# DotBlossom/LLM-driven_content-based-feature_recommendation_system

Measured on AMD Instinct MI355X. Metric: SimCSE train-step pairs/sec at d=128, batch 8192, higher is better.
Workload: dtype fp32+bf16x3+f16

## Files before the change

### include/recsys_amd.h

```cpp
#ifndef RECSYS_AMD_H
#define RECSYS_AMD_H

#include <stddef.h>
#include <stdint.h>

#ifdef __cplusplus
extern "C" {
#endif

const char* rsx_last_error(void);
int rsx_abi_version(void);
const char* rsx_target_arch(void);
const char* rsx_build_hash(void);

int rsx_seq_embed_fwd(const float* base, const int64_t* const* ids, const float* const* tables, int ntab,
                      const float* gate, const float* pos, const int64_t* tok_pos, const float* ln_w,
                      const float* ln_b, float eps, int64_t T, int64_t L, int64_t D, float p_drop, uint64_t seed,
                      float* out, float* mean, float* rstd, void* stream);

int64_t rsx_seq_embed_bwd_workspace_floats(int64_t T, int64_t L, int64_t D);
int rsx_seq_embed_bwd(const float* base, const int64_t* const* ids, const float* const* tables,
                      const int64_t* table_rows, const int64_t* padding_idx, int ntab, const float* gate,
                      const float* pos, const int64_t* tok_pos, const float* ln_w, const float* mean,
                      const float* rstd, float eps, int64_t T, int64_t L, int64_t D, float p_drop, uint64_t seed,
                      const float* dout, float* dbase, float* const* dtables, float* dgate, float* dpos,
                      float* dln_w, float* dln_b, float* workspace, int64_t ws_floats, void* stream);

int rsx_mha_fwd(const float* qkv, const uint8_t* key_pad, const int* seg_off, int64_t B, int64_t L, int64_t H,
                int64_t Dh, int causal, float p_drop, uint64_t seed, float* out, float* lse, void* stream);
int rsx_mha_bwd(const float* qkv, const uint8_t* key_pad, const int* seg_off, const float* out, const float* lse,
                const float* dout, int64_t B, int64_t L, int64_t H, int64_t Dh, int causal, float p_drop,
                uint64_t seed, float* dqkv, void* stream);
int rsx_mha_fwd_x3(const float* qkv, const uint8_t* key_pad, const int* seg_off, int64_t B, int64_t L, int64_t H,
                   int64_t Dh, int causal, float p_drop, uint64_t seed, float* out, float* lse, void* stream);
int rsx_mha_bwd_x3(const float* qkv, const uint8_t* key_pad, const int* seg_off, const float* out, const float* lse,
                   const float* dout, int64_t B, int64_t L, int64_t H, int64_t Dh, int causal, float p_drop,
                   uint64_t seed, float* dqkv, void* stream);
int rsx_mha_qkv_fwd_x3(const float* x, const float* w, const float* bias, const uint8_t* key_pad, const int* seg_off,
                       int64_t B, int64_t L, int64_t H, int causal, float p_drop, uint64_t seed, float* qkv,
                       float* out, float* lse, void* stream);

int64_t rsx_nce_workspace_floats(int64_t N, int64_t M, int nsplit_fwd, int nsplit_bwd);
int rsx_nce_fwd(const float* A, const float* B, const float* bias, const int* k1a, const int* k1b, const int* k2a,
                const int* k2b, int64_t N, int64_t M, int64_t lda, int64_t ldb, int64_t diag_offset, float tau,
                int flags, int nsplit, float* ws, float* out2, void* stream);
int rsx_nce_bwd(const float* A, const float* B, const float* bias, const int* k1a, const int* k1b, const int* k2a,
                const int* k2b, int64_t N, int64_t M, int64_t lda, int64_t ldb, int64_t diag_offset, float tau,
                int flags, int nsplit_fwd, int nsplit, const float* gout, float* ws, float* dA, float* dB,
                int accumulate, void* stream);

int64_t rsx_nce_x3_workspace_floats(int64_t N, int64_t M);
int rsx_nce_fwd_x3(const float* A, const float* B, const float* bias, const int* k1a, const int* k1b,
                   const int* k2a, const int* k2b, int64_t N, int64_t M, int64_t lda, int64_t ldb,
                   int64_t diag_offset, float tau, int flags, float* ws, float* out2, void* stream);
int rsx_nce_bwd_x3(const float* A, const float* B, const float* bias, const int* k1a, const int* k1b,
                   const int* k2a, const int* k2b, int64_t N, int64_t M, int64_t lda, int64_t ldb,
                   int64_t diag_offset, float tau, int flags, const float* gout, float* ws, float* dA, float* dB,
                   int accumulate, void* stream);

int64_t rsx_nce_fused_workspace_floats(int64_t N, int64_t M);
int64_t rsx_nce_view_ints(int64_t N, int64_t M);
int rsx_nce_view_fill(int64_t N, int64_t M, int64_t diag_offset, int* view, void* stream);
int rsx_nce_view_fill_host(int64_t N, int64_t M, int64_t diag_offset, int* view);
int rsx_nce_fwd_grad(const float* A, const float* B, const float* bias, const int* k1a, const int* k1b, int64_t N,
                     int64_t M, int64_t lda, int64_t ldb, int64_t diag_offset, float tau, int flags,
                     const int* view, float* ws, float* out2, float* ga, void* stream);
int rsx_nce_bwd_cols(const float* A, const float* B, const float* bias, const int* k1a, const int* k1b, int64_t N,
                     int64_t M, int64_t lda, int64_t ldb, int64_t diag_offset, float tau, int flags,
                     const int* view, const float* gout, float* ws, float* dB, void* stream);

int rsx_nce_emphasis_fwd(const float* A, const float* B, const float* bias, const int* k1a, const int* k1b,
                         const int64_t* top, int64_t N, int64_t M, int64_t K, int64_t lda, int64_t ldb,
                         int64_t diag_offset, float tau, float margin, int precision, int nsplit_fwd, float* ws,
                         float* out2, void* stream);
int rsx_nce_emphasis_bwd(const float* A, const float* B, const float* bias, const int* k1a, const int* k1b,
// ... 118 lines not shown
int rsx_deepfm_train_head(const float* h2, int64_t H, const float* wo, const float* lin, const float* bias,
                          const float* y, int64_t R, int mean, float* logit, float* g, float* dh2, void* ws,
                          int64_t ws_bytes, double* loss, float* dbias, float* dwo, void* stream);
int rsx_relu_bwd(float* dx, const float* h, int64_t n, void* stream);
int rsx_deepfm_train_contrib(const float* emb, const float* g, const float* dE, int64_t ldE, const int* inv,
                             int64_t R, int F, int E, float* gV, float* gW, void* stream);
int64_t rsx_deepfm_train_sparse_workspace_bytes(int64_t n);
int rsx_deepfm_train_sparse_adam(const int64_t* keys_sorted, const int* head_cum, const int* seg_start,
                                 const int* nseg, int64_t n, int F, int E, const int64_t* vocab, const float* gV,
                                 const float* gW, float* const* V, float* const* W, float* const* mV,
                                 float* const* vV, float* const* mW, float* const* vW, double lr, double beta1,
                                 double beta2, double eps, int64_t step, void* ws, int64_t ws_bytes, float* out_dV,
                                 float* out_dW, void* stream);

int64_t rsx_binary_eval_workspace_bytes(int64_t R);
int rsx_binary_eval(const float* logit, const float* y, int64_t R, void* ws, int64_t ws_bytes, int64_t* counts,
                    double* loss_sum, int* flag, void* stream);

int64_t rsx_group_eval_workspace_bytes(int64_t R);
int rsx_group_eval(const float* logit, const float* y, const int32_t* group_id, int64_t R, int top, const double* D,
                   int64_t max_group_id, void* ws, int64_t ws_bytes, int64_t* summary, int32_t* gid, int64_t* P,
                   int64_t* N, int64_t* U2, double* dcg, int* flag, void* stream);

int rsx_reranker_seq_lens(const int64_t* uidx, const int64_t* seq_off, int64_t B, int max_len, int64_t* lens,
                          void* stream);
int rsx_reranker_batch(const int64_t* uidx, const int64_t* iidx, int64_t B, const float* u_scaled, const double* u_raw,
                       const int64_t* u_cat, const float* i_scaled, const double* i_raw, const int64_t* i_num,
                       const int64_t* seq_off, const int64_t* seq_ids, int max_len, int64_t L, float* dense,
                       int64_t* cat, int64_t* target, int64_t* seq, int64_t* mask, void* stream);

int rsx_embed3_ln(const float* word, int64_t ld_word, const float* pos, const float* type_row, const float* ln_w,
                  const float* ln_b, float eps, const int64_t* ids, const int64_t* tok_pos, int64_t T, int64_t D,
                  float* out, void* stream);

int rsx_crossnet(const float* x, int64_t ldx, int64_t B, int D, int L, const float* const* kernels,
                 const float* const* biases, const float* w_head, float* x_out, float* head_part, void* stream);
int64_t rsx_crossnet_bwd_workspace_bytes(int64_t B, int D, int L, int max_blocks);
int rsx_crossnet_bwd(const float* x, int64_t ldx, int64_t B, int D, int L, const float* const* kernels,
                     const float* const* biases, const float* w_head, const float* dhead, const float* dx_out,
                     float* const* dk, float* const* db, float* dw_head, float* dx, void* ws, int64_t ws_bytes,
                     int max_blocks, void* stream);
int64_t rsx_dcn_train_head_workspace_bytes(int64_t R);
int rsx_dcn_train_head(const float* h2, int64_t H, const float* w_d, const float* head_part, const float* bias,
                       const float* y, int64_t R, int mean, float* logit, float* g, float* dh2, void* ws,
                       int64_t ws_bytes, double* loss, float* dbias, float* dw_d, void* stream);

int rsx_gather_rows(const float* src, int64_t ld_src, const int64_t* idx, int64_t n, int64_t D, int normalize,
                    float eps, float* out, float* nrm_out, void* stream);
int rsx_scatter_rows(const float* dy, const float* y, const float* nrm, const int64_t* idx, int64_t n, int64_t D,
                     int normalize, float eps, int mode, int64_t skip_idx, float* dst, int64_t ld_dst, void* stream);
int rsx_segment_sum_rows(const float* src, int64_t ld_src, const int64_t* perm, const int64_t* seg_off,
                         const int64_t* rows, int64_t nseg, int64_t D, const float* scale, int64_t skip_row,
                         float* dst, int64_t ld_dst, int accumulate, void* stream);

int rsx_loss_combine(const float* s_main, const float* s_un, const float* s_sup, const float* cnt, float inv_n,
                     float inv_b, float lambda_sup, float lambda_cl, float* total, float* logs, void* stream);
int rsx_loss_combine_bwd(const float* g, const float* cnt, float inv_n, float inv_b, float lambda_sup,
                         float lambda_cl, float* g3, void* stream);

enum {
  RSX_SP_IDS = 0, RSX_SP_TABLES = 16, RSX_SP_GATE = 32, RSX_SP_CONT = 33, RSX_SP_WC = 34, RSX_SP_BC = 35,
  RSX_SP_WM = 36, RSX_SP_BM = 37, RSX_SP_LNW = 38, RSX_SP_LNB = 39, RSX_SP_N = 40
};
int64_t rsx_static_profile_arena_bytes(int64_t U);
int64_t rsx_static_profile_bwd_workspace_bytes(int64_t U);
int rsx_static_profile_fwd(const void* const* p, const int64_t* dims, float eps, float p_drop, uint64_t seed,
                           void* arena, int64_t arena_bytes, float* out, void* stream);
int rsx_static_profile_bwd(const void* const* p, const int64_t* dims, float p_drop, uint64_t seed, const void* arena,
                           const float* dout, float* const* grads, void* ws, int64_t ws_bytes, void* stream);

int64_t rsx_clip_adamw_workspace_bytes(int n, const int64_t* numel, const int* clip);
int rsx_clip_adamw(int n, float* const* params, float* const* grads, float* const* exp_avg, float* const* exp_avg_sq,
                   const int64_t* numel, const int* clip, const float* step, const float* const* step_dev,
                   const double* lr, const double* weight_decay, const double* beta1, const double* beta2,
                   const double* eps, float max_norm, void* ws, int64_t ws_bytes, float* norm_out, void* stream);

int rsx_hnm_mine(const float* u_norm, const float* i_norm, const int64_t* target_ids, int64_t N, int64_t D,
                 int64_t k, float hnm_threshold, float temperature, void* ws, size_t ws_bytes, int64_t* top_idx,
                 float* top_cos, int32_t* avail, void* stream);
int64_t rsx_hnm_workspace_bytes(int64_t N);
int64_t rsx_hnm_max_rows(void);

enum {
  RSX_TW_PV = 0, RSX_TW_IDS = 1, RSX_TW_TOK_POS = 7, RSX_TW_TOK_PAD = 8, RSX_TW_SEG32 = 9, RSX_TW_SEG64 = 10,
  RSX_TW_TOK_USER = 11, RSX_TW_GATE = 12, RSX_TW_PROFILE = 13, RSX_TW_ITEMSEG = 14, RSX_TW_ITEM_PROJ = 19,
  RSX_TW_TABLES = 21, RSX_TW_POS = 27, RSX_TW_EMB_LN = 28, RSX_TW_LAYER0 = 30
};
int64_t rsx_tower_n_ptrs(int layers);
int64_t rsx_tower_arena_bytes(int64_t T, int64_t U, int layers);
int64_t rsx_tower_bwd_workspace_bytes(int64_t T, int64_t U, int64_t L, int layers, int64_t C);
int rsx_tower_fwd(const void* const* p, const int64_t* dims, const float* fargs, const uint64_t* seeds, void* arena,
                  int64_t arena_bytes, float* out, void* stream);
int rsx_tower_bwd(const void* const* p, const int64_t* dims, const float* fargs, const uint64_t* seeds,
                  const void* arena, const float* out, const float* dout, void* const* grads, void* ws,
                  int64_t ws_bytes, void* stream);

#ifdef __cplusplus
}
#endif

#endif
```

### llm-driven_content-based-feature_recommendation_system_amd/_native.py

```python
from __future__ import annotations

import ctypes
import os
import threading

import torch

_HERE = os.path.dirname(os.path.abspath(__file__))
LIB_PATH = os.environ.get("RSX_LIB_PATH") or os.path.join(_HERE, "librecsys_amd.so")

_lock = threading.Lock()
_lib = None
_checked_devices: set = set()

c_p = ctypes.c_void_p
c_i64 = ctypes.c_int64
c_i = ctypes.c_int
c_f = ctypes.c_float
c_d = ctypes.c_double
c_u64 = ctypes.c_uint64

ABI_VERSION = 9

_SIGS = {
    "rsx_last_error": (ctypes.c_char_p, []),
    "rsx_abi_version": (c_i, []),
    "rsx_target_arch": (ctypes.c_char_p, []),
    "rsx_build_hash": (ctypes.c_char_p, []),
    "rsx_seq_embed_fwd": (c_i, [c_p, c_p, c_p, c_i, c_p, c_p, c_p, c_p, c_p, c_f, c_i64, c_i64, c_i64, c_f, c_u64,
                                c_p, c_p, c_p, c_p]),
    "rsx_seq_embed_bwd_workspace_floats": (c_i64, [c_i64, c_i64, c_i64]),
    "rsx_seq_embed_bwd": (c_i, [c_p, c_p, c_p, c_p, c_p, c_i, c_p, c_p, c_p, c_p, c_p, c_p, c_f, c_i64, c_i64,
                                c_i64, c_f, c_u64, c_p, c_p, c_p, c_p, c_p, c_p, c_p, c_p, c_i64, c_p]),
    "rsx_mha_fwd": (c_i, [c_p, c_p, c_p, c_i64, c_i64, c_i64, c_i64, c_i, c_f, c_u64, c_p, c_p, c_p]),
    "rsx_mha_bwd": (c_i, [c_p, c_p, c_p, c_p, c_p, c_p, c_i64, c_i64, c_i64, c_i64, c_i, c_f, c_u64, c_p, c_p]),
    "rsx_mha_fwd_x3": (c_i, [c_p, c_p, c_p, c_i64, c_i64, c_i64, c_i64, c_i, c_f, c_u64, c_p, c_p, c_p]),
    "rsx_mha_qkv_fwd_x3": (c_i, [c_p, c_p, c_p, c_p, c_p, c_i64, c_i64, c_i64, c_i, c_f, c_u64, c_p, c_p, c_p, c_p]),
    "rsx_mha_bwd_x3": (c_i, [c_p, c_p, c_p, c_p, c_p, c_p, c_i64, c_i64, c_i64, c_i64, c_i, c_f, c_u64, c_p, c_p]),
    "rsx_nce_workspace_floats": (c_i64, [c_i64, c_i64, c_i, c_i]),
    "rsx_nce_fwd": (c_i, [c_p, c_p, c_p, c_p, c_p, c_p, c_p, c_i64, c_i64, c_i64, c_i64, c_i64, c_f, c_i, c_i, c_p,
                          c_p, c_p]),
    "rsx_nce_bwd": (c_i, [c_p, c_p, c_p, c_p, c_p, c_p, c_p, c_i64, c_i64, c_i64, c_i64, c_i64, c_f, c_i, c_i, c_i,
                          c_p, c_p, c_p, c_p, c_i, c_p]),
    "rsx_nce_x3_workspace_floats": (c_i64, [c_i64, c_i64]),
    "rsx_nce_fwd_x3": (c_i, [c_p, c_p, c_p, c_p, c_p, c_p, c_p, c_i64, c_i64, c_i64, c_i64, c_i64, c_f, c_i, c_p, c_p,
                             c_p]),
    "rsx_nce_bwd_x3": (c_i, [c_p, c_p, c_p, c_p, c_p, c_p, c_p, c_i64, c_i64, c_i64, c_i64, c_i64, c_f, c_i, c_p, c_p,
                             c_p, c_p, c_i, c_p]),
    "rsx_nce_fused_workspace_floats": (c_i64, [c_i64, c_i64]),
    "rsx_nce_view_ints": (c_i64, [c_i64, c_i64]),
    "rsx_nce_view_fill": (c_i, [c_i64, c_i64, c_i64, c_p, c_p]),
    "rsx_nce_view_fill_host": (c_i, [c_i64, c_i64, c_i64, c_p]),
    "rsx_nce_fwd_grad": (c_i, [c_p, c_p, c_p, c_p, c_p, c_i64, c_i64, c_i64, c_i64, c_i64, c_f, c_i, c_p, c_p, c_p,
                               c_p, c_p]),
    "rsx_nce_bwd_cols": (c_i, [c_p, c_p, c_p, c_p, c_p, c_i64, c_i64, c_i64, c_i64, c_i64, c_f, c_i, c_p, c_p, c_p,
                               c_p, c_p]),
    "rsx_nce_emphasis_fwd": (c_i, [c_p, c_p, c_p, c_p, c_p, c_p, c_i64, c_i64, c_i64, c_i64, c_i64, c_i64, c_f, c_f,
                                   c_i, c_i, c_p, c_p, c_p]),
    "rsx_nce_emphasis_bwd": (c_i, [c_p, c_p, c_p, c_p, c_p, c_p, c_i64, c_i64, c_i64, c_i64, c_i64, c_i64, c_f, c_f,
                                   c_i, c_i, c_p, c_p, c_p, c_p, c_p]),
    "rsx_nce_emphasis_bwd_csr": (c_i, [c_p, c_p, c_p, c_p, c_p, c_p, c_i64, c_i64, c_i64, c_i64, c_i64, c_i64, c_f,
                                       c_f, c_i, c_i, c_p, c_p, c_p, c_p, c_p, c_p, c_p, c_p]),
    "rsx_nce_grouped_workspace_floats": (c_i64, [c_i64, c_i64, c_i, c_i, c_i]),
    "rsx_nce_grouped_fwd": (c_i, [c_p, c_p, c_p, c_p, c_p, c_p, c_p, c_p, c_i64, c_i64, c_i64, c_i64, c_f, c_i, c_i,
                                  c_p, c_p, c_p]),
    "rsx_kernel_events": (c_i, [c_i]),
    "rsx_kernel_events_read": (c_i, [c_p, c_i]),
    "rsx_gather_events": (c_i, [c_i]),
    "rsx_gather_events_read": (c_i, [c_p, c_p, c_i]),
    "rsx_nce_grouped_fwd_grad": (c_i, [c_p, c_p, c_p, c_p, c_p, c_p, c_p, c_p, c_i64, c_i64, c_i64, c_i64, c_f, c_i,
                                       c_i, c_p, c_p, c_p, c_p]),
    "rsx_nce_grouped_bwd": (c_i, [c_p, c_p, c_p, c_p, c_p, c_p, c_p, c_p, c_p, c_p, c_p, c_p, c_p, c_i64, c_i64,
                                  c_i64, c_i64, c_f, c_i, c_i, c_i, c_p, c_p, c_p, c_p, c_i, c_p]),
    "rsx_deepfm_embed": (c_i, [c_p, c_i64, c_i, c_i, c_p, c_p, c_f, c_p, c_p, c_p]),
    "rsx_deepfm_fused_workspace_bytes": (c_i64, [c_i]),
    "rsx_deepfm_fused": (c_i, [c_p, c_i64, c_i, c_p, c_p, c_f, c_p, c_p, c_p, c_p, c_p, c_p, c_p, c_p, c_p]),
    "rsx_deepfm_fused_prep": (c_i, [c_i, c_p, c_p, c_p, c_p]),
    "rsx_deepfm_fused_run": (c_i, [c_p, c_i64, c_i, c_p, c_p, c_p, c_f, c_p, c_p, c_p, c_p, c_p, c_p, c_p]),
    "rsx_deepfm_pack": (c_i, [c_p, c_p, c_i64, c_p, c_p]),
    "rsx_reranker_seq_lens": (c_i, [c_p, c_p, c_i64, c_i, c_p, c_p]),
    "rsx_reranker_batch": (c_i, [c_p, c_p, c_i64, c_p, c_p, c_p, c_p, c_p, c_p, c_p, c_p, c_i, c_i64, c_p, c_p, c_p,
                                 c_p, c_p, c_p]),
    "rsx_deepfm_fused_uses_packed": (c_i, [c_i]),
    "rsx_linear_fwd": (c_i, [c_p, c_i64, c_p, c_p, c_i64, c_i64, c_i64, c_i, c_p, c_p]),
    "rsx_linear_dot_fwd": (c_i, [c_p, c_i64, c_p, c_p, c_i64, c_i64, c_i64, c_i, c_p, c_p, c_p, c_p, c_p]),
    "rsx_static_embed_fwd": (c_i, [c_p, c_p, c_p, c_p, c_i, c_p, c_i64, c_p, c_i64, c_p]),
    "rsx_static_embed_bwd_workspace_floats": (c_i64, [c_i64, c_i, c_p, c_p]),
    "rsx_static_embed_bwd": (c_i, [c_p, c_p, c_p, c_p, c_p, c_i, c_p, c_p, c_i64, c_i64, c_i64, c_p, c_p, c_i, c_p,
                                   c_i64, c_p]),
    "rsx_dropout_bwd": (c_i, [c_p, c_i64, c_i64, c_f, c_u64, c_p, c_p]),
    "rsx_ln_fwd": (c_i, [c_p, c_p, c_f, c_u64, c_p, c_p, c_f, c_i, c_i64, c_i64, c_p, c_p, c_p, c_p, c_p]),
    "rsx_ln_bwd_workspace_floats": (c_i64, [c_i64, c_i64]),
    "rsx_ln_bwd": (c_i, [c_p, c_p, c_p, c_p, c_p, c_i, c_p, c_p, c_f, c_u64, c_i64, c_i64, c_p, c_p, c_p, c_p, c_p,
                         c_i64, c_p]),
    "rsx_linear_wgrad_workspace_floats": (c_i64, [c_i64, c_i64, c_i64]),
    "rsx_linear_wgrad": (c_i, [c_p, c_i64, c_p, c_i64, c_i64, c_i64, c_i64, c_p, c_i64, c_p, c_i, c_p, c_i64, c_p]),
    "rsx_linear_wgrad_x3": (c_i, [c_p, c_i64, c_p, c_i64, c_i64, c_i64, c_i64, c_p, c_i64, c_p, c_i, c_p, c_i64, c_p]),
    "rsx_gemm_x3": (c_i, [c_p, c_i64, c_p, c_i64, c_p, c_i64, c_i, c_i, c_i, c_p, c_i64, c_f, c_u64, c_p, c_i64, c_p]),
    "rsx_gemm_x3_split_floats": (c_i64, [c_i64, c_i, c_i]),
    "rsx_gemm_x3_ws": (c_i, [c_p, c_i64, c_p, c_i64, c_p, c_i64, c_i, c_i, c_i, c_p, c_i64, c_f, c_u64, c_p, c_i64, c_p,
                             c_i64, c_p]),
    "rsx_gemm_x3_tn": (c_i, [c_p, c_i64, c_p, c_i64, c_p, c_i64, c_i, c_i, c_i, c_p, c_i64, c_f, c_u64, c_p, c_i64,
                             c_p]),
    "rsx_loss_combine": (c_i, [c_p, c_p, c_p, c_p, c_f, c_f, c_f, c_f, c_p, c_p, c_p]),
    "rsx_loss_combine_bwd": (c_i, [c_p, c_p, c_f, c_f, c_f, c_f, c_p, c_p]),
    "rsx_static_profile_arena_bytes": (c_i64, [c_i64]),
    "rsx_static_profile_bwd_workspace_bytes": (c_i64, [c_i64]),
    "rsx_static_profile_fwd": (c_i, [c_p, c_p, c_f, c_f, c_u64, c_p, c_i64, c_p, c_p]),
    "rsx_static_profile_bwd": (c_i, [c_p, c_p, c_f, c_u64, c_p, c_p, c_p, c_p, c_i64, c_p]),
    "rsx_clip_adamw_workspace_bytes": (c_i64, [c_i, c_p, c_p]),
    "rsx_clip_adamw": (c_i, [c_i, c_p, c_p, c_p, c_p, c_p, c_p, c_p, c_p, c_p, c_p, c_p, c_p, c_p, c_f, c_p, c_i64,
                             c_p, c_p]),
    "rsx_tower_n_ptrs": (c_i64, [c_i]),
    "rsx_tower_arena_bytes": (c_i64, [c_i64, c_i64, c_i]),
    "rsx_tower_bwd_workspace_bytes": (c_i64, [c_i64, c_i64, c_i64, c_i, c_i64]),
    "rsx_tower_fwd": (c_i, [c_p, c_p, c_p, c_p, c_p, c_i64, c_p, c_p]),
    "rsx_tower_bwd": (c_i, [c_p, c_p, c_p, c_p, c_p, c_p, c_p, c_p, c_p, c_i64, c_p]),
    "rsx_gemm_x3_rowadd": (c_i, [c_p, c_i64, c_p, c_i64, c_p, c_i64, c_i, c_i, c_p, c_i64, c_p, c_p, c_i64, c_p]),
    "rsx_gemm_x3_addln": (c_i, [c_p, c_i64, c_p, c_i64, c_p, c_i64, c_i, c_i, c_p, c_i64, c_f, c_u64, c_p, c_p, c_f,
                                c_p, c_i64, c_p, c_i64, c_p, c_p, c_p]),
    "rsx_topk_workspace_bytes": (c_i64, [c_i64, c_i64, c_i64]),
    "rsx_retrieve_topk": (c_i, [c_p, c_i64, c_p, c_i64, c_i64, c_i64, c_i64, c_p, c_p, c_p, c_p]),
    "rsx_topk_path": (c_i, [c_i64, c_i64, c_i64]),
    "rsx_ids_check": (c_i, [c_p, c_i64, c_i64, c_i64, c_p, c_p, c_p]),
    "rsx_step_index_workspace_bytes": (c_i64, [c_i64, c_i64, c_i64]),
    "rsx_step_index_count": (c_i, [c_p, c_p, c_p, c_i64, c_i64, c_i64, c_p, c_i64, c_p, c_p]),
    "rsx_step_index_totals": (c_i, [c_p, c_i, c_i64, c_i64, c_i64, c_p, c_i64, c_p, c_p]),
    "rsx_step_index_fill": (c_i, [c_p, c_p, c_p, c_p, c_i64, c_i64, c_i64, c_i64, c_p, c_p, c_i64, c_p, c_p]),
    "rsx_topk_corpus_bytes": (c_i64, [c_i64]),
    "rsx_topk_prepare_corpus": (c_i, [c_p, c_i64, c_i64, c_p, c_p]),
    "rsx_topk_workspace_bytes_corpus": (c_i64, [c_i64, c_i64, c_i64]),
    "rsx_retrieve_topk_corpus": (c_i, [c_p, c_i64, c_p, c_i64, c_p, c_i64, c_i64, c_i64, c_p, c_p, c_p, c_p]),
    "rsx_gather_rows": (c_i, [c_p, c_i64, c_p, c_i64, c_i64, c_i, c_f, c_p, c_p, c_p]),
    "rsx_embed3_ln": (c_i, [c_p, c_i64, c_p, c_p, c_p, c_p, c_f, c_p, c_p, c_i64, c_i64, c_p, c_p]),
    "rsx_crossnet": (c_i, [c_p, c_i64, c_i64, c_i, c_i, c_p, c_p, c_p, c_p, c_p, c_p]),
    "rsx_crossnet_bwd_workspace_bytes": (c_i64, [c_i64, c_i, c_i, c_i]),
    "rsx_crossnet_bwd": (c_i, [c_p, c_i64, c_i64, c_i, c_i, c_p, c_p, c_p, c_p, c_p, c_p, c_p, c_p, c_p, c_p, c_i64, c_i,
                               c_p]),
    "rsx_dcn_train_head_workspace_bytes": (c_i64, [c_i64]),
    "rsx_dcn_train_head": (c_i, [c_p, c_i64, c_p, c_p, c_p, c_p, c_i64, c_i, c_p, c_p, c_p, c_p, c_i64, c_p, c_p, c_p,
                                 c_p]),
    "rsx_segment_sum_rows": (c_i, [c_p, c_i64, c_p, c_p, c_p, c_i64, c_i64, c_p, c_i64, c_p, c_i64, c_i, c_p]),
    "rsx_scatter_rows": (c_i, [c_p, c_p, c_p, c_p, c_i64, c_i64, c_i, c_f, c_i, c_i64, c_p, c_i64, c_p]),
    "rsx_hnm_mine": (c_i, [c_p, c_p, c_p, c_i64, c_i64, c_i64, c_f, c_f, c_p, ctypes.c_size_t, c_p, c_p, c_p, c_p]),
    "rsx_hnm_workspace_bytes": (c_i64, [c_i64]),
    "rsx_hnm_max_rows": (c_i64, []),
    "rsx_deepfm_train_keys": (c_i, [c_p, c_i64, c_i, c_p, c_p, c_p, c_p, c_p]),
    "rsx_deepfm_train_segments": (c_i, [c_p, c_p, c_i64, c_p, c_p, c_p]),
    "rsx_deepfm_train_starts": (c_i, [c_p, c_i64, c_p, c_p, c_p]),
    "rsx_deepfm_train_head_workspace_bytes": (c_i64, [c_i64]),
    "rsx_deepfm_train_head": (c_i, [c_p, c_i64, c_p, c_p, c_p, c_p, c_i64, c_i, c_p, c_p, c_p, c_p, c_i64, c_p, c_p, c_p,
                                    c_p]),
    "rsx_relu_bwd": (c_i, [c_p, c_p, c_i64, c_p]),
    "rsx_deepfm_train_contrib": (c_i, [c_p, c_p, c_p, c_i64, c_p, c_i64, c_i, c_i, c_p, c_p, c_p]),
    "rsx_deepfm_train_sparse_workspace_bytes": (c_i64, [c_i64]),
    "rsx_deepfm_train_sparse_adam": (c_i, [c_p, c_p, c_p, c_p, c_i64, c_i, c_i, c_p, c_p, c_p, c_p, c_p, c_p, c_p,
                                           c_p, c_p, c_d, c_d, c_d, c_d, c_i64, c_p, c_i64, c_p, c_p, c_p]),
    "rsx_binary_eval_workspace_bytes": (c_i64, [c_i64]),
    "rsx_binary_eval": (c_i, [c_p, c_p, c_i64, c_p, c_i64, c_p, c_p, c_p, c_p]),
    "rsx_group_eval_workspace_bytes": (c_i64, [c_i64]),
    "rsx_group_eval": (c_i, [c_p, c_p, c_p, c_i64, c_i, c_p, c_i64, c_p, c_i64, c_p, c_p, c_p, c_p, c_p, c_p, c_p, c_p]),
}

EXPORTED_SYMBOLS = tuple(_SIGS.keys())


def load(path: str = LIB_PATH):
    global _lib
    with _lock:
        if _lib is not None:
            return _lib
        if not os.path.exists(path):
            raise RuntimeError(
                f"recsys_amd: native library not found at {path}; run __graft_entry__.build() "
                "(hipcc --offload-arch=gfx950). There is no CPU fallback.")
        lib = ctypes.CDLL(path)
        for name, (res, args) in _SIGS.items():
            fn = getattr(lib, name)
            fn.restype = res
            fn.argtypes = args
        if lib.rsx_abi_version() != ABI_VERSION:
            raise RuntimeError(f"recsys_amd: {path} has ABI {lib.rsx_abi_version()}, this binding expects "
                               f"{ABI_VERSION}; rebuild with __graft_entry__.build()")
        _lib = lib
        return lib


def lib():
    return _lib if _lib is not None else load()


def source_files() -> list:
    import glob
    here = os.path.dirname(os.path.abspath(__file__))
    csrc = os.path.join(here, "csrc")
# ... 63 lines not shown
```

### llm-driven_content-based-feature_recommendation_system_amd/csrc/rows.hip

```cpp
#include "rsx_common.h"

namespace {

template <int D>
struct RowGeo {
  static constexpr int LPR = D / 4;
  static constexpr int RPW = 64 / LPR;
};

template <int D, bool NORM>
__global__ __launch_bounds__(256) void gather_rows_k(const float* __restrict__ src, int64_t ld_src,
                                                    const int64_t* __restrict__ idx, int64_t n, float eps,
                                                    float* __restrict__ out, float* __restrict__ nrm_out) {
  constexpr int LPR = RowGeo<D>::LPR, RPW = RowGeo<D>::RPW;
  const int lane = threadIdx.x & 63, sub = lane / LPR, c = lane % LPR;
  const int64_t wave_g = (int64_t)blockIdx.x * 4 + (threadIdx.x >> 6);
  const int64_t nw = (int64_t)gridDim.x * 4;
  for (int64_t r0 = wave_g * RPW; r0 < n; r0 += nw * RPW) {
    const int64_t r = r0 + sub;
    const bool ok = r < n;
    float4 x = make_float4(0.f, 0.f, 0.f, 0.f);
    if (ok) {
      const int64_t s = idx ? idx[r] : r;
      x = reinterpret_cast<const float4*>(src + s * ld_src)[c];
// ... 26 lines not shown
    float4 g = make_float4(0.f, 0.f, 0.f, 0.f);
    if (ok) g = reinterpret_cast<const float4*>(dy + r * D)[c];
    if (NORM) {
      float4 yv = make_float4(0.f, 0.f, 0.f, 0.f);
      if (ok) yv = reinterpret_cast<const float4*>(y + r * D)[c];
      float dot = yv.x * g.x + yv.y * g.y + yv.z * g.z + yv.w * g.w;
      dot = rsx::wave_sum_width(dot, LPR);
      const float nv = ok ? nrm[r] : 1.0f;
      if (nv > eps) {
        g.x = (g.x - yv.x * dot) / nv; g.y = (g.y - yv.y * dot) / nv;
        g.z = (g.z - yv.z * dot) / nv; g.w = (g.w - yv.w * dot) / nv;
      } else {
        g.x = g.x / eps; g.y = g.y / eps; g.z = g.z / eps; g.w = g.w / eps;
      }
    }
    if (ATOMIC) {
      float* xr = &s_xr[threadIdx.x >> 6][sub][0];
      reinterpret_cast<float4*>(xr)[c] = g;
      __builtin_amdgcn_wave_barrier();
      float xs[4];
#pragma unroll
      for (int k = 0; k < 4; ++k) xs[k] = xr[c + LPR * k];
      __builtin_amdgcn_wave_barrier();
      if (!ok) continue;
      const int64_t d = idx ? idx[r] : r;
      if (d == skip_idx) continue;
      float* q = dst + d * ld_dst + c;
#pragma unroll
      for (int k = 0; k < 4; ++k) atomicAdd(q + LPR * k, xs[k]);
      continue;
    }
    if (!ok) continue;
    const int64_t d = idx ? idx[r] : r;
    if (d == skip_idx) continue;
    float* p = dst + d * ld_dst + 4 * c;
    if (accumulate) {
      float4 o = *reinterpret_cast<float4*>(p);
      o.x += g.x; o.y += g.y; o.z += g.z; o.w += g.w;
      *reinterpret_cast<float4*>(p) = o;
    } else {
      *reinterpret_cast<float4*>(p) = g;
    }
  }
}

unsigned grid_for(int64_t n, int D) {
  const int64_t rows_per_block = 4 * (64 / (D / 4));
  int64_t b = (n + rows_per_block - 1) / rows_per_block;
  if (b > 16384) b = 16384;
  if (b < 1) b = 1;
  return (unsigned)b;
}

template <int D>
__global__ __launch_bounds__(256) void segsum_rows_k(const float* __restrict__ src, int64_t ld_src,
                                                    const int64_t* __restrict__ perm,
                                                    const int64_t* __restrict__ seg,
                                                    const int64_t* __restrict__ rows, int64_t nseg,
                                                    const float* __restrict__ scale, int64_t skip,
                                                    float* __restrict__ dst, int64_t ld_dst, int accumulate) {
  constexpr int LPR = RowGeo<D>::LPR, RPW = RowGeo<D>::RPW;
  const int lane = threadIdx.x & 63, sub = lane / LPR, c = lane % LPR;
  const int64_t wave_g = (int64_t)blockIdx.x * 4 + (threadIdx.x >> 6);
  const int64_t nw = (int64_t)gridDim.x * 4;
  const float sc = scale ? scale[0] : 1.0f;
  for (int64_t u0 = wave_g * RPW; u0 < nseg; u0 += nw * RPW) {
    const int64_t u = u0 + sub;
    if (u >= nseg) continue;
    const int64_t row = rows ? rows[u] : u;
    if (row == skip) continue;
    float4 acc = make_float4(0.f, 0.f, 0.f, 0.f);
    const int64_t k1 = seg[u + 1];
    int64_t k = seg[u];
    for (; k + 16 <= k1; k += 16) {
      int64_t p[16];
#pragma unroll
      for (int i = 0; i < 16; ++i) p[i] = perm ? perm[k + i] : k + i;
      float4 x[16];
#pragma unroll
      for (int i = 0; i < 16; ++i) x[i] = reinterpret_cast<const float4*>(src + p[i] * ld_src)[c];
#pragma unroll
      for (int i = 0; i < 16; ++i) {
        acc.x += x[i].x; acc.y += x[i].y; acc.z += x[i].z; acc.w += x[i].w;
      }
    }
    if (k < k1) {
      const int n = (int)(k1 - k);
      int64_t p[15];
#pragma unroll
      for (int i = 0; i < 15; ++i) p[i] = i < n ? (perm ? perm[k + i] : k + i) : 0;
      float4 x[15];
#pragma unroll
      for (int i = 0; i < 15; ++i)
        x[i] = i < n ? reinterpret_cast<const float4*>(src + p[i] * ld_src)[c] : make_float4(0.f, 0.f, 0.f, 0.f);
#pragma unroll
      for (int i = 0; i < 15; ++i)
        if (i < n) { acc.x += x[i].x; acc.y += x[i].y; acc.z += x[i].z; acc.w += x[i].w; }
    }
    float4* d = reinterpret_cast<float4*>(dst + row * ld_dst) + c;
    float4 v = make_float4(sc * acc.x, sc * acc.y, sc * acc.z, sc * acc.w);
    if (accumulate) {
      const float4 o = *d;
      v.x += o.x; v.y += o.y; v.z += o.z; v.w += o.w;
    }
    *d = v;
  }
}

__global__ __launch_bounds__(256) void ids_check_k(const int64_t* __restrict__ ids, int64_t n, int64_t lo, int64_t hi,
                                                   int64_t* __restrict__ out, int* flag) {
  bool bad = false;
  for (int64_t i = (int64_t)blockIdx.x * 256 + threadIdx.x; i < n; i += (int64_t)gridDim.x * 256) {
    const int64_t v = ids[i];
    const bool ok = v >= lo && v < hi;
    out[i] = ok ? v : 0;
    bad |= !ok;
  }
  if (__builtin_amdgcn_ballot_w64(bad) && (threadIdx.x & 63) == 0) atomicOr(flag, 1);
}

__global__ void loss_combine_k(const float* s_main, const float* s_un, const float* s_sup, const float* cnt,
                               float inv_n, float inv_b, float lsup, float lcl, float* total, float* logs) {
  if (threadIdx.x != 0) return;
  const float m = s_main ? s_main[0] * inv_n : 0.0f;
  float cl = s_un[0] * inv_b;
  if (s_sup) cl += lsup * (s_sup[0] / fmaxf(cnt[0], 1.0f));
  const float t = m + lcl * cl;
  total[0] = t;
  logs[0] = t; logs[1] = m; logs[2] = cl;
}

__global__ void loss_combine_bwd_k(const float* g, const float* cnt, float inv_n, float inv_b, float lsup, float lcl,
                                   float* g3) {
  if (threadIdx.x != 0) return;
  const float gv = g[0];
  g3[0] = gv * inv_n;
  g3[1] = gv * lcl * inv_b;
  g3[2] = cnt ? gv * lcl * lsup / fmaxf(cnt[0], 1.0f) : 0.0f;
}

}

RSX_API int rsx_loss_combine(const float* s_main, const float* s_un, const float* s_sup, const float* cnt,
                             float inv_n, float inv_b, float lambda_sup, float lambda_cl, float* total, float* logs,
                             void* stream) {
  RSX_ARG(s_un && total && logs && (!s_sup || cnt), "null tensor");
  hipLaunchKernelGGL(loss_combine_k, dim3(1), dim3(64), 0, (hipStream_t)stream, s_main, s_un, s_sup, cnt, inv_n,
                     inv_b, lambda_sup, lambda_cl, total, logs);
  RSX_LAUNCHED();
  return 0;
// ... 17 lines not shown
  hipStream_t st = (hipStream_t)stream;
  const unsigned g = grid_for(n, (int)D);
#define RSX_G(DD)                                                                                     \
  if (D == DD) {                                                                                      \
    if (normalize) hipLaunchKernelGGL((gather_rows_k<DD, true>), dim3(g), dim3(256), 0, st, src, ld_src, idx, n, eps, out, nrm_out); \
    else hipLaunchKernelGGL((gather_rows_k<DD, false>), dim3(g), dim3(256), 0, st, src, ld_src, idx, n, eps, out, nrm_out); \
  }
  RSX_G(64) RSX_G(128) RSX_G(256)
#undef RSX_G
  RSX_LAUNCHED();
  return 0;
}

RSX_API int rsx_scatter_rows(const float* dy, const float* y, const float* nrm, const int64_t* idx, int64_t n,
                             int64_t D, int normalize, float eps, int mode, int64_t skip_idx, float* dst,
                             int64_t ld_dst, void* stream) {
  RSX_ARG(dy && dst, "null tensor");
  RSX_ARG(!normalize || (y && nrm), "normalize backward needs y and norms");
  RSX_ARG(D == 64 || D == 128 || D == 256, "D must be 64, 128 or 256");
  RSX_ARG(mode >= 0 && mode <= 2, "mode must be 0,1,2");
  if (n == 0) return 0;
  hipStream_t st = (hipStream_t)stream;
  const unsigned g = grid_for(n, (int)D);
#define RSX_S(DD, NN, AA)                                                                           \
  hipLaunchKernelGGL((scatter_rows_k<DD, NN, AA>), dim3(g), dim3(256), 0, st, dy, y, nrm, idx, n, eps, dst, ld_dst, \
                     mode == 1 ? 1 : 0, skip_idx)
#define RSX_SD(DD)                                          \
  if (D == DD) {                                            \
    if (normalize) {                                        \
      if (mode == 2) RSX_S(DD, true, true); else RSX_S(DD, true, false);   \
    } else {                                                \
      if (mode == 2) RSX_S(DD, false, true); else RSX_S(DD, false, false); \
    }                                                       \
  }
  RSX_SD(64) RSX_SD(128) RSX_SD(256)
#undef RSX_SD
#undef RSX_S
  RSX_LAUNCHED();
  return 0;
}

RSX_API int rsx_segment_sum_rows(const float* src, int64_t ld_src, const int64_t* perm, const int64_t* seg_off,
                                 const int64_t* rows, int64_t nseg, int64_t D, const float* scale, int64_t skip_row,
                                 float* dst, int64_t ld_dst, int accumulate, void* stream) {
  RSX_ARG(src && seg_off && dst, "null tensor");
  RSX_ARG(D == 64 || D == 128 || D == 256, "D must be 64, 128 or 256");
  RSX_ARG(ld_src >= D && ld_dst >= D && ld_src % 4 == 0 && ld_dst % 4 == 0, "bad leading dimensions");
  if (nseg == 0) return 0;
  hipStream_t st = (hipStream_t)stream;
  const unsigned g = grid_for(nseg, (int)D);
#define RSX_SS(DD)                                                                                            \
  if (D == DD)                                                                                                \
    hipLaunchKernelGGL(segsum_rows_k<DD>, dim3(g), dim3(256), 0, st, src, ld_src, perm, seg_off, rows, nseg, \
                       scale, skip_row, dst, ld_dst, accumulate);
  RSX_SS(64) RSX_SS(128) RSX_SS(256)
#undef RSX_SS
  RSX_LAUNCHED();
  return 0;
}

RSX_API int rsx_ids_check(const int64_t* ids, int64_t n, int64_t lo, int64_t hi, int64_t* out, int* flag,
                          void* stream) {
  RSX_ARG(ids && out && flag, "null tensor");
  RSX_ARG(lo <= 0 && 0 < hi, "the replacement id 0 must lie in [lo, hi)");
  if (n == 0) return 0;
  int64_t g = (n + 255) / 256;
  if (g > 1024) g = 1024;
  hipLaunchKernelGGL(ids_check_k, dim3((unsigned)g), dim3(256), 0, (hipStream_t)stream, ids, n, lo, hi, out, flag);
  RSX_LAUNCHED();
  return 0;
}
```

### llm-driven_content-based-feature_recommendation_system_amd/csrc/rsx_errors.hip

```cpp
#include "rsx_common.h"
#include <stdarg.h>
#include <stdio.h>

namespace rsx {
static thread_local char g_err[1024] = {0};

void set_error(const char* fmt, ...) {
  va_list ap;
  va_start(ap, fmt);
  vsnprintf(g_err, sizeof(g_err), fmt, ap);
  va_end(ap);
}
}

RSX_API const char* rsx_last_error(void) { return rsx::g_err; }

RSX_API int rsx_abi_version(void) { return 9; }

RSX_API const char* rsx_target_arch(void) { return "gfx950"; }

#ifndef RSX_SRC_HASH
#define RSX_SRC_HASH "unknown"
#endif
RSX_API const char* rsx_build_hash(void) { return RSX_SRC_HASH; }
```

### llm-driven_content-based-feature_recommendation_system_amd/csrc/seq_embed.hip

```cpp
#include "rsx_common.h"
#include <mutex>
#include <utility>
#include <vector>

namespace {

constexpr int kMaxTab = 6;

struct FwdArgs {
  const float* base;
  const int64_t* ids[kMaxTab];
  const float* tab[kMaxTab];
  const float* gate;
  const float* pos;
  const int64_t* tok_pos;
  const float* ln_w;
  const float* ln_b;
  float* out;
  float* mean;
  float* rstd;
  int64_t T;
  int L;
  int ntab;
  float eps;
  rsx::Dropout drop;
};

typedef float f4v __attribute__((ext_vector_type(4)));
typedef __attribute__((address_space(1))) const f4v gf4v;
typedef __attribute__((address_space(1))) const int64_t gint64;
__device__ __forceinline__ float4 ldg4(const float* p) {
  const f4v v = *(gf4v*)(p);
  return make_float4(v.x, v.y, v.z, v.w);
}
__device__ __forceinline__ int64_t ldg8(const int64_t* p) { return *(gint64*)(p); }

template <int W>
__device__ __forceinline__ float lane_sum(float v) {
  if constexpr (W != 16 && W != 32 && W != 64) {
    return rsx::wave_sum_width(v, W);
  } else {
    if constexpr (W == 64) {
      const auto sw = __builtin_amdgcn_permlane32_swap(__float_as_uint(v), __float_as_uint(v), false, false);
      v = __uint_as_float(sw[0]) + __uint_as_float(sw[1]);
    }
    if constexpr (W >= 32) {
      const auto sw = __builtin_amdgcn_permlane16_swap(__float_as_uint(v), __float_as_uint(v), false, false);
      v = __uint_as_float(sw[0]) + __uint_as_float(sw[1]);
    }
    v += __int_as_float(__builtin_amdgcn_update_dpp(__float_as_int(v), __float_as_int(v), 0x128, 0xF, 0xF, false));
    v += __int_as_float(__builtin_amdgcn_update_dpp(__float_as_int(v), __float_as_int(v), 0x124, 0xF, 0xF, false));
    v += __int_as_float(__builtin_amdgcn_update_dpp(__float_as_int(v), __float_as_int(v), 0x122, 0xF, 0xF, false));
    v += __int_as_float(__builtin_amdgcn_update_dpp(__float_as_int(v), __float_as_int(v), 0x121, 0xF, 0xF, false));
    return v;
  }
}

__device__ __forceinline__ float4 f4_axpy_rn(float4 x, float4 e, float g) {
#pragma clang fp contract(off)
  x.x = x.x + e.x * g;
  x.y = x.y + e.y * g;
  x.z = x.z + e.z * g;
  x.w = x.w + e.w * g;
  return x;
}

__device__ __forceinline__ float4 f4_add_rn(float4 x, float4 p) {
#pragma clang fp contract(off)
  x.x = x.x + p.x;
  x.y = x.y + p.y;
  x.z = x.z + p.z;
  x.w = x.w + p.w;
  return x;
}

template <int D>
__device__ __forceinline__ float4 build_row(const FwdArgs& a, int64_t r, int c, const float* g) {
  float4 x = make_float4(0.f, 0.f, 0.f, 0.f);
  if (a.base) x = ldg4(a.base + r * D + 4 * c);
#pragma unroll
  for (int j = 0; j < kMaxTab; ++j) {
    if (j < a.ntab && g[j] != 0.0f) {
      const int64_t id = ldg8(a.ids[j] + r);
      const float4 e = ldg4(a.tab[j] + id * D + 4 * c);
      x = f4_axpy_rn(x, e, g[j]);
    }
  }
  if (a.pos) {
    const int l = a.tok_pos ? (int)ldg8(a.tok_pos + r) : (int)(r % a.L);
    x = f4_add_rn(x, ldg4(a.pos + (int64_t)l * D + 4 * c));
  }
  return x;
}

template <int D>
__device__ __forceinline__ void ln_drop_store(const FwdArgs& a, float4 x, int64_t r, bool ok, int c, float4 w,
                                              float4 bb, bool do_ln) {
  constexpr int LPR = D / 4;
  float4 y = x;
  if (do_ln) {
    float s = (x.x + x.y) + (x.z + x.w);
    s = lane_sum<LPR>(s);
    const float mu = s / (float)D;
    const float4 d = make_float4(x.x - mu, x.y - mu, x.z - mu, x.w - mu);
    float v = d.x * d.x + d.y * d.y + d.z * d.z + d.w * d.w;
    v = lane_sum<LPR>(v);
    const float rs = 1.0f / sqrtf(v / (float)D + a.eps);
    y.x = d.x * rs * w.x + bb.x;
    y.y = d.y * rs * w.y + bb.y;
    y.z = d.z * rs * w.z + bb.z;
    y.w = d.w * rs * w.w + bb.w;
    if (ok && c == 0) {
      if (a.mean) a.mean[r] = mu;
      if (a.rstd) a.rstd[r] = rs;
    }
  }
  if (ok) {
    if (a.drop.active()) {
      const uint64_t base_idx = (uint64_t)r * D + 4 * c;
      y.x = a.drop.apply(y.x, base_idx + 0);
      y.y = a.drop.apply(y.y, base_idx + 1);
      y.z = a.drop.apply(y.z, base_idx + 2);
      y.w = a.drop.apply(y.w, base_idx + 3);
    }
    reinterpret_cast<float4*>(a.out + r * D)[c] = y;
  }
}

template <int D, int U, int NL, bool FULL = false>
__device__ __forceinline__ void fwd_groups(const FwdArgs& a, const int64_t* const* ids_l, const float* const* tab_l,
                                           const float* g_l, int64_t r0, int sub, int c, float4 w, float4 bb,
                                           bool do_ln) {
  constexpr int RPW = 64 / (D / 4);
  const bool has_pos = FULL || a.pos, has_base = FULL || a.base;
  int64_t rr[U];
  int64_t id[U][NL > 0 ? NL : 1];
  int lp[U];
#pragma unroll
  for (int u = 0; u < U; ++u) {
    const int64_t r = r0 + u * RPW + sub;
    rr[u] = r < a.T ? r : a.T - 1;
#pragma unroll
    for (int k = 0; k < NL; ++k) id[u][k] = ldg8(ids_l[k] + rr[u]);
    if (FULL) lp[u] = (int)ldg8(a.tok_pos + rr[u]);
    else lp[u] = a.pos ? (a.tok_pos ? (int)a.tok_pos[rr[u]] : (int)(rr[u] % a.L)) : 0;
  }
  float4 x[U];
#pragma unroll
  for (int u = 0; u < U; ++u)
    x[u] = has_base ? ldg4(a.base + rr[u] * D + 4 * c) : make_float4(0.f, 0.f, 0.f, 0.f);
  float4 e[U][NL > 0 ? NL : 1];
#pragma unroll
  for (int k = 0; k < NL; ++k)
#pragma unroll
    for (int u = 0; u < U; ++u) e[u][k] = ldg4(tab_l[k] + id[u][k] * D + 4 * c);
  float4 pv[U];
  if (FULL) {
#pragma unroll
    for (int u = 0; u < U; ++u) pv[u] = ldg4(a.pos + (int64_t)lp[u] * D + 4 * c);
  }
#pragma unroll
  for (int k = 0; k < NL; ++k)
#pragma unroll
    for (int u = 0; u < U; ++u) x[u] = f4_axpy_rn(x[u], e[u][k], g_l[k]);
  if (has_pos) {
#pragma unroll
    for (int u = 0; u < U; ++u)
      x[u] = f4_add_rn(x[u], FULL ? pv[u] : ldg4(a.pos + (int64_t)lp[u] * D + 4 * c));
  }
#pragma unroll
  for (int u = 0; u < U; ++u) {
    const int64_t r = r0 + u * RPW + sub;
    ln_drop_store<D>(a, x[u], r, r < a.T, c, w, bb, FULL || do_ln);
  }
}

template <int D, int U>
__global__ __launch_bounds__(256) void seq_embed_fwd_k(FwdArgs a) {
  constexpr int LPR = D / 4;
  constexpr int RPW = 64 / LPR;
  const int lane = threadIdx.x & 63;
  const int sub = lane / LPR, c = lane % LPR;
  const int64_t wave_g = (int64_t)blockIdx.x * (blockDim.x >> 6) + (threadIdx.x >> 6);
  const int64_t nwaves = (int64_t)gridDim.x * (blockDim.x >> 6);
  float g[kMaxTab];
#pragma unroll
  for (int j = 0; j < kMaxTab; ++j) g[j] = (j < a.ntab) ? (a.gate ? a.gate[j] : 1.0f) : 0.0f;
  const int64_t* ids_l[2] = {nullptr, nullptr};
  const float* tab_l[2] = {nullptr, nullptr};
  float g_l[2] = {0.0f, 0.0f};
  int nl = 0;
#pragma unroll
  for (int j = 0; j < kMaxTab; ++j) {
    if (g[j] != 0.0f) {
      if (nl == 0) { ids_l[0] = a.ids[j]; tab_l[0] = a.tab[j]; g_l[0] = g[j]; }
      else if (nl == 1) { ids_l[1] = a.ids[j]; tab_l[1] = a.tab[j]; g_l[1] = g[j]; }
      ++nl;
    }
  }
  const bool do_ln = a.ln_w != nullptr;
  float4 w = make_float4(1.f, 1.f, 1.f, 1.f), bb = make_float4(0.f, 0.f, 0.f, 0.f);
  if (do_ln) {
    w = reinterpret_cast<const float4*>(a.ln_w)[c];
    bb = reinterpret_cast<const float4*>(a.ln_b)[c];
  }
  if (nl > 2) {
    for (int64_t r0 = wave_g * RPW; r0 < a.T; r0 += nwaves * RPW) {
      const int64_t r = r0 + sub;
      const bool ok = r < a.T;
      const float4 x = build_row<D>(a, ok ? r : a.T - 1, c, g);
      ln_drop_store<D>(a, x, r, ok, c, w, bb, do_ln);
    }
    return;
  }
  if (nl == 2 && a.base && a.pos && a.tok_pos && do_ln) {
    for (int64_t r0 = wave_g * (RPW * U); r0 < a.T; r0 += nwaves * (RPW * U))
      fwd_groups<D, U, 2, true>(a, ids_l, tab_l, g_l, r0, sub, c, w, bb, true);
    return;
  }
  for (int64_t r0 = wave_g * (RPW * U); r0 < a.T; r0 += nwaves * (RPW * U)) {
    if (nl == 2) fwd_groups<D, U, 2>(a, ids_l, tab_l, g_l, r0, sub, c, w, bb, do_ln);
    else if (nl == 1) fwd_groups<D, U, 1>(a, ids_l, tab_l, g_l, r0, sub, c, w, bb, do_ln);
    else fwd_groups<D, U, 0>(a, ids_l, tab_l, g_l, r0, sub, c, w, bb, do_ln);
  }
}

struct BwdArgs {
  FwdArgs f;
  const float* dout;
  float* dbase;
  float* dtab[kMaxTab];
  int64_t pad_idx[kMaxTab];
  int small_off[kMaxTab];
  int small_rows[kMaxTab];
  float* dgate;
  float* dpos;
  float* dln_w;
  float* dln_b;
  int64_t rows_per_block;
  int small_total;
  float* partials;
  int part_w;
};

struct BwdLive {
  const int64_t* ids[kMaxTab];
  const float* tab[kMaxTab];
  float* dtab[kMaxTab];
  float g[kMaxTab];
  int64_t pad[kMaxTab];
  int soff[kMaxTab];
  int j[kMaxTab];
  int n;
};

struct BwdCtx {
  float* xr;
  float* s_pos;
  float* s_small;
  int64_t r_begin, r_end;
  int wave, sub, c;
  float4 w;
  bool do_ln;
};

template <int D, int U, int NL, bool SC>
__device__ __forceinline__ void bwd_groups(const BwdArgs& a, const BwdLive& lv, const BwdCtx& cx, int64_t r00,
                                           float4& acc_w, float4& acc_b, float* acc_l) {
  constexpr int LPR = D / 4;
  constexpr int RPW = 64 / LPR;
  constexpr int NW = 4;
  constexpr int NS = NL > 0 ? NL : 1;
  const FwdArgs& f = a.f;
  const int c = cx.c;
  const bool need_e = cx.do_ln || a.dgate;
  const bool need_l = (f.pos && cx.do_ln) || a.dpos;
  int64_t rc[U];
  int lp[U];
  int64_t id[U][NS];
#pragma unroll
  for (int u = 0; u < U; ++u) {
    const int64_t ru = r00 + (u * NW + cx.wave) * RPW + cx.sub;
    rc[u] = ru < cx.r_end ? ru : cx.r_begin;
    lp[u] = need_l ? (f.tok_pos ? (int)f.tok_pos[rc[u]] : (int)(rc[u] % f.L)) : 0;
#pragma unroll
    for (int k = 0; k < NS; ++k)
      id[u][k] = (NL > 0 && (NL != kMaxTab || k < lv.n)) ? ldg8(lv.ids[k] + rc[u]) : 0;
  }
  float4 dyv[U], xv[U];
  float muv[U], rsv[U];
#pragma unroll
  for (int u = 0; u < U; ++u) {
    dyv[u] = ldg4(a.dout + rc[u] * D + 4 * c);
    xv[u] = make_float4(0.f, 0.f, 0.f, 0.f);
    muv[u] = 0.0f; rsv[u] = 0.0f;
    if (cx.do_ln) {
      if (f.base) xv[u] = ldg4(f.base + rc[u] * D + 4 * c);
      muv[u] = f.mean[rc[u]];
      rsv[u] = f.rstd[rc[u]];
    }
  }
  float4 ev[U][NS];
#pragma unroll
  for (int k = 0; k < NS; ++k)
#pragma unroll
    for (int u = 0; u < U; ++u) {
      ev[u][k] = make_float4(0.f, 0.f, 0.f, 0.f);
      if (NL > 0 && (NL != kMaxTab || k < lv.n) && need_e)
        ev[u][k] = ldg4(lv.tab[k] + id[u][k] * D + 4 * c);
    }
  if (cx.do_ln) {
#pragma unroll
    for (int k = 0; k < NS; ++k)
#pragma unroll
      for (int u = 0; u < U; ++u)
        if (NL > 0 && (NL != kMaxTab || k < lv.n)) xv[u] = f4_axpy_rn(xv[u], ev[u][k], lv.g[k]);
    if (f.pos) {
#pragma unroll
      for (int u = 0; u < U; ++u)
        xv[u] = f4_add_rn(xv[u], ldg4(f.pos + (int64_t)lp[u] * D + 4 * c));
    }
  }
#pragma unroll
  for (int u = 0; u < U; ++u) {
    const int64_t r = r00 + (u * NW + cx.wave) * RPW + cx.sub;
    if (r >= cx.r_end) continue;
    float4 dy = dyv[u];
    if (f.drop.active()) {
      const uint64_t bi = (uint64_t)r * D + 4 * c;
      dy.x = f.drop.apply(dy.x, bi + 0);
      dy.y = f.drop.apply(dy.y, bi + 1);
      dy.z = f.drop.apply(dy.z, bi + 2);
      dy.w = f.drop.apply(dy.w, bi + 3);
    }
    float4 dx = dy;
    if (cx.do_ln) {
      const float4 x = xv[u];
      const float mu = muv[u], rs = rsv[u];
      const float4 w = cx.w;
      const float4 xh = make_float4((x.x - mu) * rs, (x.y - mu) * rs, (x.z - mu) * rs, (x.w - mu) * rs);
      acc_w.x += dy.x * xh.x; acc_w.y += dy.y * xh.y; acc_w.z += dy.z * xh.z; acc_w.w += dy.w * xh.w;
      acc_b.x += dy.x; acc_b.y += dy.y; acc_b.z += dy.z; acc_b.w += dy.w;
      const float4 dh = make_float4(dy.x * w.x, dy.y * w.y, dy.z * w.z, dy.w * w.w);
      float c1 = (dh.x + dh.y) + (dh.z + dh.w);
      float c2 = dh.x * xh.x + dh.y * xh.y + dh.z * xh.z + dh.w * xh.w;
      c1 = lane_sum<LPR>(c1) / (float)D;
      c2 = lane_sum<LPR>(c2) / (float)D;
      dx.x = (dh.x - c1 - xh.x * c2) * rs;
      dx.y = (dh.y - c1 - xh.y * c2) * rs;
      dx.z = (dh.z - c1 - xh.z * c2) * rs;
// ... 390 lines not shown
    dst = a.dln_b ? a.dln_b + (j - nlds - a.D) : nullptr;
  } else if (j - nlds - 2 * a.D < a.ntab) {
    dst = a.dgate ? a.dgate + (j - nlds - 2 * a.D) : nullptr;
  }
  if (dst) *dst += v;
}

template <int D>
int launch_fwd(const FwdArgs& a, hipStream_t st) {
  constexpr int U = 2;
  const int64_t rows_per_block = 4 * (64 / (D / 4)) * U;
  int64_t blocks = (a.T + rows_per_block - 1) / rows_per_block;
  if (blocks > 16384) blocks = 16384;
  if (blocks < 1) blocks = 1;
  hipLaunchKernelGGL((seq_embed_fwd_k<D, U>), dim3((unsigned)blocks), dim3(256), 0, st, a);
  return 0;
}

template <int D>
int launch_bwd(const BwdArgs& a, hipStream_t st, bool keysum) {
  const int64_t blocks = (a.f.T + a.rows_per_block - 1) / a.rows_per_block;
  if (keysum) {
    hipLaunchKernelGGL((seq_embed_bwd_k<D, false>), dim3((unsigned)blocks), dim3(256), 0, st, a);
    return 0;
  }
  const size_t lds = (size_t)(a.f.L * D + a.small_total) * sizeof(float);
  hipLaunchKernelGGL((seq_embed_bwd_k<D>), dim3((unsigned)blocks), dim3(256), lds, st, a);
  return 0;
}

int64_t bwd_rows_per_block(int64_t T, int64_t D, int64_t target_blocks) {
  int64_t rpb = (T + target_blocks - 1) / target_blocks;
  const int64_t quantum = 2 * 4 * (64 / (D / 4));
  rpb = (rpb + quantum - 1) / quantum * quantum;
  if (rpb < quantum) rpb = quantum;
  return rpb;
}

int small_layout(const int64_t* table_rows, int ntab, int64_t D, bool has_grad_j[kMaxTab], int off[kMaxTab],
                 int rows[kMaxTab]) {
  int o = 0;
  for (int j = 0; j < kMaxTab; ++j) {
    off[j] = -1;
    rows[j] = 0;
    if (j < ntab && has_grad_j[j] && table_rows && table_rows[j] * D <= 4096 && o + table_rows[j] * D <= kSmallMax) {
      off[j] = o;
      rows[j] = (int)table_rows[j];
      o += (int)(table_rows[j] * D);
    }
  }
  return o;
}

bool fill_fwd(FwdArgs& a, const float* base, const int64_t* const* ids, const float* const* tabs, int ntab,
              const float* gate, const float* pos, const int64_t* tok_pos, const float* ln_w, const float* ln_b,
              float eps, int64_t T, int64_t L, float* out, float* mean, float* rstd, float p_drop, uint64_t seed) {
  if (ntab < 0 || ntab > kMaxTab) return false;
  a.base = base;
  for (int j = 0; j < kMaxTab; ++j) {
    a.ids[j] = (j < ntab) ? ids[j] : nullptr;
    a.tab[j] = (j < ntab) ? tabs[j] : nullptr;
  }
  a.gate = gate;
  a.pos = pos;
  a.tok_pos = tok_pos;
  a.ln_w = ln_w;
  a.ln_b = ln_b;
  a.out = out;
  a.mean = mean;
  a.rstd = rstd;
  a.T = T;
  a.L = (int)L;
  a.ntab = ntab;
  a.eps = eps;
  a.drop = rsx::make_dropout(p_drop, seed);
  return true;
}

struct GatherEvents {
  std::mutex mu;
  bool on = false;
  std::vector<std::pair<hipEvent_t, hipEvent_t>> ev;
  std::vector<int64_t> tokens;
  void clear() {
    for (auto& e : ev) {
      (void)hipEventDestroy(e.first);
      (void)hipEventDestroy(e.second);
    }
    ev.clear();
    tokens.clear();
  }
};
GatherEvents& gather_events() {
  static GatherEvents g;
  return g;
}
}

RSX_API int rsx_gather_events(int on) {
  GatherEvents& g = gather_events();
  std::lock_guard<std::mutex> lk(g.mu);
  g.clear();
  g.on = on != 0;
  return 0;
}

RSX_API int rsx_gather_events_read(float* ms, int64_t* tokens, int max_n) {
  RSX_ARG((ms != nullptr && tokens != nullptr) || max_n == 0, "null output");
  GatherEvents& g = gather_events();
  std::lock_guard<std::mutex> lk(g.mu);
  int n = 0;
  for (size_t k = 0; k < g.ev.size() && n < max_n; ++k) {
    float t = 0.0f;
    hipError_t err = hipEventSynchronize(g.ev[k].second);
    if (err == hipSuccess) err = hipEventElapsedTime(&t, g.ev[k].first, g.ev[k].second);
    if (err != hipSuccess) {
      rsx::set_error("%s: %s", __func__, hipGetErrorString(err));
      return -1;
    }
    ms[n] = t;
    tokens[n] = g.tokens[k];
    ++n;
  }
  return n;
}

RSX_API int rsx_seq_embed_fwd(const float* base, const int64_t* const* ids, const float* const* tables, int ntab,
                              const float* gate, const float* pos, const int64_t* tok_pos, const float* ln_w,
                              const float* ln_b, float eps, int64_t T, int64_t L, int64_t D, float p_drop,
                              uint64_t seed, float* out, float* mean, float* rstd, void* stream) {
  RSX_ARG(out != nullptr, "out is null");
  RSX_ARG(T >= 0 && L > 0 && L <= 64, "need T >= 0 and 0 < L <= 64");
  RSX_ARG(D == 64 || D == 128 || D == 256, "D must be 64, 128 or 256");
  RSX_ARG(ntab >= 0 && ntab <= kMaxTab, "ntab must be in [0,6]");
  RSX_ARG(ln_w == nullptr || (ln_b != nullptr), "ln_b required with ln_w");
  RSX_ARG(p_drop >= 0.0f && p_drop < 1.0f, "p_drop must be in [0,1)");
  for (int j = 0; j < ntab; ++j) RSX_ARG(ids[j] != nullptr && tables[j] != nullptr, "null table/ids");
  if (T == 0) return 0;
  FwdArgs a;
  fill_fwd(a, base, ids, tables, ntab, gate, pos, tok_pos, ln_w, ln_b, eps, T, L, out, mean, rstd, p_drop, seed);
  hipStream_t st = (hipStream_t)stream;
  GatherEvents& ge = gather_events();
  std::pair<hipEvent_t, hipEvent_t> evp{nullptr, nullptr};
  const bool timed = ge.on;
  if (timed && hipEventCreate(&evp.first) == hipSuccess && hipEventCreate(&evp.second) == hipSuccess)
    (void)hipEventRecord(evp.first, st);
  if (D == 64) launch_fwd<64>(a, st);
  else if (D == 128) launch_fwd<128>(a, st);
  else launch_fwd<256>(a, st);
  RSX_LAUNCHED();
  if (timed && evp.second) {
    (void)hipEventRecord(evp.second, st);
    std::lock_guard<std::mutex> lk(ge.mu);
    ge.ev.push_back(evp);
    ge.tokens.push_back(T);
  }
  return 0;
}

constexpr int64_t kBwdBlocksWs = 768;
constexpr int64_t kBwdBlocksAtomic = 512;
constexpr int64_t kKeyBlocksMax = 512;

RSX_API int64_t rsx_seq_embed_bwd_workspace_floats(int64_t T, int64_t L, int64_t D) {
  if (T <= 0 || D <= 0) return 0;
  const int64_t rpb = bwd_rows_per_block(T, D, kBwdBlocksWs);
  const int64_t blocks = (T + rpb - 1) / rpb;
  return blocks * (L * D + kSmallMax + 2 * D + kMaxTab) + kKeyBlocksMax * 64 * D;
}

RSX_API int rsx_seq_embed_bwd(const float* base, const int64_t* const* ids, const float* const* tables,
                              const int64_t* table_rows, const int64_t* padding_idx, int ntab, const float* gate,
                              const float* pos, const int64_t* tok_pos, const float* ln_w, const float* mean,
                              const float* rstd, float eps, int64_t T, int64_t L, int64_t D, float p_drop,
                              uint64_t seed, const float* dout, float* dbase, float* const* dtables, float* dgate,
                              float* dpos, float* dln_w, float* dln_b, float* workspace, int64_t ws_floats,
                              void* stream) {
  RSX_ARG(dout != nullptr, "dout is null");
  RSX_ARG(D == 64 || D == 128 || D == 256, "D must be 64, 128 or 256");
  RSX_ARG(ntab >= 0 && ntab <= kMaxTab, "ntab must be in [0,6]");
  RSX_ARG(ln_w == nullptr || (mean != nullptr && rstd != nullptr), "mean/rstd required with ln_w");
  RSX_ARG(p_drop >= 0.0f && p_drop < 1.0f, "p_drop must be in [0,1)");
  RSX_ARG(L > 0 && L <= 64, "need 0 < L <= 64");
  if (T == 0) return 0;
  BwdArgs a;
  fill_fwd(a.f, base, ids, tables, ntab, gate, pos, tok_pos, ln_w, nullptr, eps, T, L, nullptr,
           const_cast<float*>(mean), const_cast<float*>(rstd), p_drop, seed);
  a.dout = dout;
  a.dbase = dbase;
  bool has_grad[kMaxTab];
  for (int j = 0; j < kMaxTab; ++j) {
    a.dtab[j] = (j < ntab && dtables) ? dtables[j] : nullptr;
    a.pad_idx[j] = (j < ntab && padding_idx) ? padding_idx[j] : -1;
    has_grad[j] = a.dtab[j] != nullptr;
  }
  a.small_total = small_layout(table_rows, ntab, D, has_grad, a.small_off, a.small_rows);
  a.dgate = dgate;
  a.dpos = dpos;
  a.dln_w = dln_w;
  a.dln_b = dln_b;
  const bool use_ws = workspace != nullptr;
  if (use_ws)
    RSX_ARG(ws_floats >= rsx_seq_embed_bwd_workspace_floats(T, L, D), "workspace too small");
  a.rows_per_block = bwd_rows_per_block(T, D, use_ws ? kBwdBlocksWs : kBwdBlocksAtomic);
  const int64_t blocks = (T + a.rows_per_block - 1) / a.rows_per_block;
  a.partials = use_ws ? workspace : nullptr;
  a.part_w = (int)(L * D + a.small_total + 2 * D + kMaxTab);
  KeyArgs k{};
  bool keysum = use_ws && D == 128 && dbase != nullptr && (L * D + a.small_total) <= 64 * D &&
                getenv("RSX_SEQ_EMBED_KEYSUM") == nullptr;
  int nsm = 0;
  for (int j = 0; j < ntab && keysum; ++j) {
    if (!a.dtab[j] || a.small_off[j] < 0) continue;
    if (nsm == 2) { keysum = false; break; }
    k.ids[nsm] = ids[j];
    k.key_off[nsm] = (int)(L + a.small_off[j] / D);
    k.pad[nsm] = a.pad_idx[j];
    ++nsm;
  }
  hipStream_t st = (hipStream_t)stream;
  if (D == 64) launch_bwd<64>(a, st, false);
  else if (D == 128) launch_bwd<128>(a, st, keysum);
  else launch_bwd<256>(a, st, false);
  const int64_t ws_a = blocks * a.part_w;
  int64_t kblocks = 0;
  if (keysum) {
    const int64_t nb = 2 * rsx::cu_count() < kKeyBlocksMax ? 2 * rsx::cu_count() : kKeyBlocksMax;
    int64_t rpb = (T + nb - 1) / nb;
    rpb = (rpb + 63) / 64 * 64;
    kblocks = (T + rpb - 1) / rpb;
    k.dx = dbase;
    k.tok_pos = tok_pos;
    k.T = T;
    k.L = (int)L;
    k.do_pos = dpos != nullptr;
    k.nkeys = (int)(L + a.small_total / D);
    k.rows_per_block = rpb;
    k.partials = workspace + ws_a;
    const dim3 g((unsigned)kblocks), b(256);
// ... 38 lines not shown
```

### llm-driven_content-based-feature_recommendation_system_amd/csrc/step_index.hip

```cpp
#include "rsx_common.h"
#include <hipcub/hipcub.hpp>
#include <limits.h>

namespace {

constexpr int kSegChunk = 64;

__device__ __forceinline__ uint64_t wballot(bool p) { return __builtin_amdgcn_ballot_w64(p); }
__device__ __forceinline__ int below(uint64_t m, int lane) {
  return __popcll(m & ((lane == 0) ? 0ull : (~0ull >> (64 - lane))));
}

__device__ __forceinline__ int wave_sort_asc(int v, int lane) {
#pragma unroll
  for (int k = 2; k <= 64; k <<= 1) {
#pragma unroll
    for (int j = k >> 1; j > 0; j >>= 1) {
      const int o = __shfl_xor(v, j, 64);
      const bool asc = (lane & k) == 0, lower = (lane & j) == 0;
      v = (asc == lower) ? min(v, o) : max(v, o);
    }
  }
  return v;
}
// ... 152 lines not shown
      int t = lane < 16 ? wsum[lane] : 0;
#pragma unroll
      for (int d = 1; d < 16; d <<= 1) {
        const int y = __shfl_up(t, d, 64);
        if (lane >= d) t += y;
      }
      if (lane < 16) wsum[lane] = t;
    }
    __syncthreads();
    int e = carry + (w > 0 ? wsum[w - 1] : 0) + x - s;
#pragma unroll
    for (int k = 0; k < 4; ++k) {
      if (i0 + k < J.n) J.out[i0 + k] = e;
      e += v[k];
    }
    carry += wsum[15];
    __syncthreads();
  }
}

__global__ void si_totals_k(const int* offT, const int* offN, const int* offE, const int* colidx, const int* itemidx,
                            const int* chunkoff, const int* err, const int* tglob, int world, int64_t B, int64_t L,
                            int64_t n_items, int64_t* tot) {
  if (threadIdx.x != 0) return;
  tot[0] = offT[B];
  tot[1] = offN[B];
  tot[2] = colidx[n_items];
  tot[3] = offE[B];
  tot[4] = itemidx[n_items];
  tot[5] = chunkoff[n_items];
  int e = *err ? 1 : 0;
  tot[7] = 0;
  for (int r = 0; r < world; ++r) {
    const int v = tglob[(int64_t)r * (B * L + 1) + B * L];
    e |= (v & kSlotErr) ? 1 : 0;
    tot[8 + r] = v & ~kSlotErr;
  }
  tot[6] = e;
}

struct FillOut {
  int64_t *flat1, *user1, *pos1;
  uint8_t* pad1;
  int* seg1;
  int64_t* seg1_64;
  int64_t *valid_tok, *last_tok;
  int64_t *flat2, *user2, *pos2;
  uint8_t* pad2;
  int* seg2;
  int64_t* seg2_64;
  int64_t* tok_ids;
  int *row_col, *row_beg, *row_end, *exc_cols;
  int* last_t;
};

__global__ __launch_bounds__(256) void si_tokens_k(const uint8_t* pm, const int64_t* tgt, const int64_t* ids0,
                                                   const int64_t* ids1, const int64_t* ids2, const int64_t* ids3,
                                                   const int64_t* ids4, const int64_t* ids5, int64_t B, int L,
                                                   int64_t T, const int* offT, const int* offN, const int* offE,
                                                   const int* srt, const int* colidx, FillOut f, unsigned* ikeys,
                                                   int* ivals, unsigned* pkeys, int* pvals, int* pair_b, int* pair_n) {
  const int lane = threadIdx.x & 63;
  const int64_t b = (int64_t)blockIdx.x * 4 + (threadIdx.x >> 6);
  if (b >= B) return;
  const User u = user_sel(pm, b, L, lane);
  const int64_t o = b * L + lane;
  const int64_t t0 = offT[b];
  if (u.sel) {
    const int64_t tok = t0 + below(u.sm, lane);
    const uint8_t pd = u.valid ? 0 : 1;
    f.flat1[tok] = o;
    f.user1[tok] = b;
    f.pos1[tok] = lane;
    f.pad1[tok] = pd;
    f.flat2[tok] = o;
    f.flat2[T + tok] = B * L + o;
    f.user2[tok] = b;
    f.user2[T + tok] = B + b;
    f.pos2[tok] = lane;
    f.pos2[T + tok] = lane;
    f.pad2[tok] = pd;
    f.pad2[T + tok] = pd;
    const int64_t* src[6] = {ids0, ids1, ids2, ids3, ids4, ids5};
#pragma unroll
    for (int k = 0; k < 6; ++k) {
      const int64_t v = src[k][o];
      f.tok_ids[(2 * k) * T + tok] = v;
      f.tok_ids[(2 * k + 1) * T + tok] = v;
    }
    ikeys[tok] = (unsigned)ids0[o];
    ivals[tok] = (int)tok;
    if (u.valid) {
      const int64_t r = offN[b] + below(u.vm, lane);
      f.valid_tok[r] = tok;
      f.row_col[r] = colidx[tgt[o]];
      f.row_beg[r] = offN[b];
      f.row_end[r] = offN[b + 1];
    }
  }
  if (lane < u.cnt) {
    const int v = srt[b * L + lane];
    const int c = colidx[v];
    f.exc_cols[offN[b] + lane] = c;
    const int pv = __shfl_up(v, 1, 64);
    (void)pv;
  }
  {
    const int v = lane < u.cnt ? srt[b * L + lane] : INT_MAX;
    const int pv = __shfl_up(v, 1, 64);
    const bool ds = lane < u.cnt && (lane == 0 || v != pv);
    const uint64_t dm = wballot(ds);
    if (ds) {
      const uint64_t higher = (lane == 63) ? 0ull : (dm & (~0ull << (lane + 1)));
      const int nxt = higher ? (__ffsll((long long)higher) - 1) : u.cnt;
      const int64_t e = offE[b] + below(dm, lane);
      pkeys[e] = (unsigned)colidx[v];
      pvals[e] = (int)e;
      pair_b[e] = (int)b;
      pair_n[e] = nxt - lane;
    }
  }
  if (lane == 0) {
    f.last_tok[b] = t0 + __popcll(u.sm & ((u.last == 0) ? 0ull : (~0ull >> (64 - u.last))));
    f.last_t[b] = (int)tgt[b * L + u.last];
    f.seg1[b] = (int)t0;
    f.seg1_64[b] = t0;
    f.seg2[b] = (int)t0;
    f.seg2_64[b] = t0;
    f.seg2[B + b] = (int)(T + t0);
    f.seg2_64[B + b] = T + t0;
    if (b == B - 1) {
      f.seg1[B] = (int)T;
      f.seg1_64[B] = T;
      f.seg2[2 * B] = (int)(2 * T);
      f.seg2_64[2 * B] = 2 * T;
    }
  }
}

__global__ __launch_bounds__(256) void si_itemseg_k(const unsigned* skeys, const int* svals, int64_t T,
                                                    const int* hist_i, const int* itemoff, const int* itemidx,
                                                    const int* chunkoff, int64_t U, int64_t C, int64_t* perm,
                                                    int64_t* cb, int64_t* chunk_ids, int64_t* ch_off,
                                                    int64_t* uniq_items) {
  for (int64_t p = (int64_t)blockIdx.x * 256 + threadIdx.x; p < T; p += (int64_t)gridDim.x * 256) {
    const unsigned id = skeys[p];
    const int64_t a = itemoff[id], n = hist_i[id], w = p - a;
    const int64_t tok = svals[p];
    perm[2 * a + w] = tok;
    perm[2 * a + n + w] = T + tok;
    if (w == 0) {
      const int64_t ui = itemidx[id], c0 = chunkoff[id];
      uniq_items[ui] = id;
      ch_off[ui] = c0;
      const int64_t nch = (2 * n + kSegChunk - 1) / kSegChunk;
      for (int64_t k = 0; k < nch; ++k) {
        cb[c0 + k] = 2 * a + kSegChunk * k;
        chunk_ids[c0 + k] = c0 + k;
      }
    }
    if (p == 0) {
      ch_off[U] = C;
      cb[C] = 2 * T;
    }
  }
}

__global__ __launch_bounds__(256) void si_cols_k(const int* hist_t, const int* hist_u, const int* colidx,
                                                 const int* pairoff, int64_t n_items, int64_t* uniq, float* colcnt,
                                                 int* col_beg, int* col_end) {
  for (int64_t v = (int64_t)blockIdx.x * 256 + threadIdx.x; v < n_items; v += (int64_t)gridDim.x * 256) {
    const int h = hist_t[v];
    if (h == 0) continue;
    const int d = colidx[v];
    uniq[d] = v;
    colcnt[d] = (float)h;
    col_beg[d] = pairoff[v];
    col_end[d] = pairoff[v] + hist_u[v];
  }
}

__global__ __launch_bounds__(256) void si_pairs_k(const int* spvals, int64_t E, const int* pair_b, const int* pair_n,
                                                  const int* offN, int* exc_s, int* exc_e, int* exc_n) {
  for (int64_t q = (int64_t)blockIdx.x * 256 + threadIdx.x; q < E; q += (int64_t)gridDim.x * 256) {
    const int e = spvals[q];
    const int b = pair_b[e];
    exc_s[q] = offN[b];
    exc_e[q] = offN[b + 1];
    exc_n[q] = pair_n[e];
  }
}

__global__ __launch_bounds__(256) void si_pv_k(const float* lookup, int64_t ld, const int64_t* ids_tok, int64_t T,
                                               float* pv) {
  const int lane = threadIdx.x & 31;
  for (int64_t t = ((int64_t)blockIdx.x * 256 + threadIdx.x) >> 5; t < T; t += ((int64_t)gridDim.x * 256) >> 5) {
    const float4 v = reinterpret_cast<const float4*>(lookup + ids_tok[t] * ld)[lane];
    reinterpret_cast<float4*>(pv + t * 128)[lane] = v;
    reinterpret_cast<float4*>(pv + (T + t) * 128)[lane] = v;
  }
}

int64_t a256(int64_t x) { return (x + 255) / 256 * 256; }

struct SiLayout {
  int64_t err, Tb, Nb, Eb, offT, offN, offE, srt, hist_t, hist_u, hist_i, colidx, itemidx, itemoff, chunkoff,
      pairoff, ikeys, ivals, ikeys_o, ivals_o, pkeys, pvals, pkeys_o, pvals_o, pair_b, pair_n, temp, temp_bytes,
      total;
};

int bits_for(int64_t n) {
  int b = 1;
  while (b < 32 && ((int64_t)1 << b) < n) ++b;
  return b;
}

size_t temp_bytes(int64_t B, int64_t L, int64_t n_items) {
  size_t s = 0;
  int* ip = nullptr;
  unsigned* up = nullptr;
  (void)hipcub::DeviceRadixSort::SortPairs(nullptr, s, up, up, ip, ip, (int)(B * L), 0, 32);
  return s;
}

SiLayout si_layout(int64_t B, int64_t L, int64_t n_items) {
  SiLayout l;
  int64_t o = 0;
  auto take = [&](int64_t bytes) {
    const int64_t r = o;
    o += a256(bytes);
    return r;
  };
  const int64_t BL = B * L, ni = n_items + 1;
  l.err = take(4);
  l.Tb = take((B + 1) * 4);
  l.Nb = take((B + 1) * 4);
  l.Eb = take((B + 1) * 4);
  l.offT = take((B + 1) * 4);
  l.offN = take((B + 1) * 4);
  l.offE = take((B + 1) * 4);
  l.srt = take(BL * 4);
  l.hist_t = take(ni * 4);
  l.hist_u = take(ni * 4);
  l.hist_i = take(ni * 4);
  l.colidx = take(ni * 4);
  l.itemidx = take(ni * 4);
  l.itemoff = take(ni * 4);
  l.chunkoff = take(ni * 4);
  l.pairoff = take(ni * 4);
  l.ikeys = take(BL * 4);
  l.ivals = take(BL * 4);
  l.ikeys_o = take(BL * 4);
  l.ivals_o = take(BL * 4);
// ... 57 lines not shown
  RSX_LAUNCHED();
  hipLaunchKernelGGL(si_slot_k, dim3(1), dim3(64), 0, st, at<int>(ws, l.offN), at<int>(ws, l.err), B, L, tloc);
  RSX_LAUNCHED();
  return 0;
}

RSX_API int rsx_step_index_totals(const int* tglob, int world, int64_t B, int64_t L, int64_t n_items, void* ws,
                                  int64_t ws_bytes, int64_t* totals, void* stream) {
  RSX_ARG(tglob && ws && totals, "null tensor");
  RSX_ARG(world >= 1, "world >= 1");
  const SiLayout l = si_layout(B, L, n_items);
  RSX_ARG(ws_bytes >= l.total, "workspace too small (rsx_step_index_workspace_bytes)");
  hipStream_t st = (hipStream_t)stream;
  const int64_t blk = B * L + 1, n = blk * world;
  hipLaunchKernelGGL(si_colhist_k, dim3((unsigned)std::max<int64_t>(1, std::min<int64_t>(256, (n + 1023) / 1024))),
                     dim3(256), 0, st, tglob, n, blk, n_items,
                     at<int>(ws, l.hist_t));
  RSX_LAUNCHED();
  {
    const int ni = (int)(n_items + 1);
    ScanJobs js{};
    js.j[0] = {at<int>(ws, l.hist_t), at<int>(ws, l.colidx), ni, 1};
    js.j[1] = {at<int>(ws, l.hist_i), at<int>(ws, l.itemidx), ni, 1};
    js.j[2] = {at<int>(ws, l.hist_i), at<int>(ws, l.itemoff), ni, 0};
    js.j[3] = {at<int>(ws, l.hist_i), at<int>(ws, l.chunkoff), ni, 2};
    js.j[4] = {at<int>(ws, l.hist_u), at<int>(ws, l.pairoff), ni, 0};
    hipLaunchKernelGGL(si_scan_k, dim3(5), dim3(1024), 0, st, js);
    RSX_LAUNCHED();
  }
  hipLaunchKernelGGL(si_totals_k, dim3(1), dim3(64), 0, st, at<int>(ws, l.offT), at<int>(ws, l.offN),
                     at<int>(ws, l.offE), at<int>(ws, l.colidx), at<int>(ws, l.itemidx), at<int>(ws, l.chunkoff),
                     at<int>(ws, l.err), tglob, world, B, L, n_items, totals);
  RSX_LAUNCHED();
  return 0;
}

RSX_API int rsx_step_index_fill(const uint8_t* pm, const int64_t* tgt, const int64_t* const* seq_ids,
                                const float* lookup, int64_t ld_lookup, int64_t B, int64_t L, int64_t n_items,
                                const int64_t* sizes, void* ws, int64_t ws_bytes, void* const* out, void* stream) {
  RSX_ARG(pm && tgt && seq_ids && sizes && ws && out, "null tensor");
  const SiLayout l = si_layout(B, L, n_items);
  RSX_ARG(ws_bytes >= l.total, "workspace too small (rsx_step_index_workspace_bytes)");
  const int64_t T = sizes[0], N = sizes[1], D = sizes[2], E = sizes[3], U = sizes[4], C = sizes[5];
  RSX_ARG(T >= B && T <= B * L && N >= 0 && N <= T && D >= 0 && E >= 0 && E <= N && U >= 1 && C >= U,
          "inconsistent sizes (rsx_step_index_totals)");
  hipStream_t st = (hipStream_t)stream;
  FillOut f;
  f.flat1 = (int64_t*)out[0]; f.user1 = (int64_t*)out[1]; f.pos1 = (int64_t*)out[2]; f.pad1 = (uint8_t*)out[3];
  f.seg1 = (int*)out[4]; f.seg1_64 = (int64_t*)out[5]; f.valid_tok = (int64_t*)out[6]; f.last_tok = (int64_t*)out[7];
  f.flat2 = (int64_t*)out[8]; f.user2 = (int64_t*)out[9]; f.pos2 = (int64_t*)out[10]; f.pad2 = (uint8_t*)out[11];
  f.seg2 = (int*)out[12]; f.seg2_64 = (int64_t*)out[13]; f.tok_ids = (int64_t*)out[14];
  f.row_col = (int*)out[23]; f.row_beg = (int*)out[24]; f.row_end = (int*)out[25]; f.exc_cols = (int*)out[26];
  f.last_t = (int*)out[32];
  const unsigned gu = (unsigned)((B + 3) / 4);
  hipLaunchKernelGGL(si_tokens_k, dim3(gu), dim3(256), 0, st, pm, tgt, seq_ids[0], seq_ids[1], seq_ids[2],
                     seq_ids[3], seq_ids[4], seq_ids[5], B, (int)L, T, at<int>(ws, l.offT), at<int>(ws, l.offN),
                     at<int>(ws, l.offE), at<int>(ws, l.srt), at<int>(ws, l.colidx), f, at<unsigned>(ws, l.ikeys),
                     at<int>(ws, l.ivals), at<unsigned>(ws, l.pkeys), at<int>(ws, l.pvals), at<int>(ws, l.pair_b),
                     at<int>(ws, l.pair_n));
  RSX_LAUNCHED();
  size_t tb = (size_t)l.temp_bytes;
  void* tmp = at<void>(ws, l.temp);
  (void)hipcub::DeviceRadixSort::SortPairs(tmp, tb, at<unsigned>(ws, l.ikeys), at<unsigned>(ws, l.ikeys_o),
                                           at<int>(ws, l.ivals), at<int>(ws, l.ivals_o), (int)T, 0,
                                           bits_for(n_items), st);
  RSX_LAUNCHED();
  hipLaunchKernelGGL(si_itemseg_k, dim3(grid_for(T)), dim3(256), 0, st, at<unsigned>(ws, l.ikeys_o),
                     at<int>(ws, l.ivals_o), T, at<int>(ws, l.hist_i), at<int>(ws, l.itemoff), at<int>(ws, l.itemidx),
                     at<int>(ws, l.chunkoff), U, C, (int64_t*)out[16], (int64_t*)out[17], (int64_t*)out[18],
                     (int64_t*)out[19], (int64_t*)out[20]);
  RSX_LAUNCHED();
  if (D > 0) {
    hipLaunchKernelGGL(si_cols_k, dim3(grid_for(n_items)), dim3(256), 0, st, at<int>(ws, l.hist_t),
                       at<int>(ws, l.hist_u), at<int>(ws, l.colidx), at<int>(ws, l.pairoff), n_items,
                       (int64_t*)out[21], (float*)out[22], (int*)out[30], (int*)out[31]);
    RSX_LAUNCHED();
  }
  if (E > 0) {
    (void)hipcub::DeviceRadixSort::SortPairs(tmp, tb, at<unsigned>(ws, l.pkeys), at<unsigned>(ws, l.pkeys_o),
                                             at<int>(ws, l.pvals), at<int>(ws, l.pvals_o), (int)E, 0,
                                             bits_for(D > 1 ? D : 2), st);
    RSX_LAUNCHED();
    hipLaunchKernelGGL(si_pairs_k, dim3(grid_for(E)), dim3(256), 0, st, at<int>(ws, l.pvals_o), E,
                       at<int>(ws, l.pair_b), at<int>(ws, l.pair_n), at<int>(ws, l.offN), (int*)out[27],
                       (int*)out[28], (int*)out[29]);
    RSX_LAUNCHED();
  }
  if (lookup && out[15]) {
    RSX_ARG(ld_lookup >= 128 && ld_lookup % 4 == 0, "pretrained lookup rows must be 128 floats (stride % 4 == 0)");
    hipLaunchKernelGGL(si_pv_k, dim3(grid_for(T * 32)), dim3(256), 0, st, lookup, ld_lookup, f.tok_ids, T,
                       (float*)out[15]);
    RSX_LAUNCHED();
  }
  return 0;
}
```

### llm-driven_content-based-feature_recommendation_system_amd/csrc/tower.hip

```cpp
#include "rsx_common.h"
#include "recsys_amd.h"

#include <utility>

namespace {

constexpr int64_t kD = 128, kQKV = 384, kF = 256, kHeads = 4, kDh = 32, kMaxLayers = 8;
constexpr int kEpiBias = 0, kEpiGeluDrop = 1, kEpiDgeluDrop = 2, kActGelu = 2;

int64_t al(int64_t floats) { return (floats + 63) / 64 * 64; }

struct LayerAct {
  int64_t qkv, a, lse, xs, hs, m2, r2, gg, act, f, xn, hn, mn, rn;
};
struct Layout {
  int64_t base, x0, m0, r0, h0, mh0, rh0;
  LayerAct l[kMaxLayers];
  int64_t prof, hp, g, mo, ro, o, nrm, aR, xR, tidx, tinv, tuser, tseg, lseq, total;
};

Layout layout(int64_t T, int64_t U, int nl) {
  Layout s{};
  int64_t o = 0;
  auto take = [&](int64_t n) { const int64_t r = o; o += al(n); return r; };
  s.base = take(T * kD); s.x0 = take(T * kD); s.m0 = take(T); s.r0 = take(T);
  s.h0 = take(T * kD); s.mh0 = take(T); s.rh0 = take(T);
  for (int i = 0; i < nl; ++i) {
    LayerAct& a = s.l[i];
    a.qkv = take(T * kQKV); a.a = take(T * kD); a.lse = take(T * kHeads);
    a.xs = take(T * kD); a.hs = take(T * kD); a.m2 = take(T); a.r2 = take(T);
    a.gg = take(T * kF); a.act = take(T * kF); a.f = take(T * kD);
    a.xn = take(T * kD); a.hn = take(T * kD); a.mn = take(T); a.rn = take(T);
  }
  s.prof = take(U * kD); s.hp = take(T * kD); s.g = take(T * kD); s.mo = take(T); s.ro = take(T);
  s.o = take(T * kD); s.nrm = take(T);
  s.aR = take(T * kD); s.xR = take(T * kD); s.tidx = take(2 * T); s.tinv = take(2 * T); s.tuser = take(2 * T);
  s.tseg = take(2 * (U + 1)); s.lseq = take(kHeads * U);
  s.total = o;
  return s;
}

struct BwdLayout {
  int64_t dO, dG, dHp, dX, dXs, dH, dHs, dF, dPre, dRes, dA, dQKV, dProf, dBase, part, dAR, dXR, wsw, wsl, wse, total;
  int64_t n_wsw, n_wsl, n_wse;
};

BwdLayout bwd_layout(int64_t T, int64_t U, int64_t L, int64_t C) {
  BwdLayout s{};
  int64_t o = 0;
  auto take = [&](int64_t n) { const int64_t r = o; o += al(n); return r; };
  s.dO = take(T * kD); s.dG = take(T * kD); s.dHp = take(T * kD); s.dX = take(T * kD); s.dXs = take(T * kD);
  s.dH = take(T * kD); s.dHs = take(T * kD); s.dF = take(T * kD); s.dPre = take(T * kF); s.dRes = take(T * kD);
  s.dA = take(T * kD); s.dQKV = take(T * kQKV); s.dProf = take(U * kD); s.dBase = take(T * kD);
  s.part = take((C > 0 ? C : 1) * kD);
  s.dAR = take((T + 1) * kD); s.dXR = take((T + 1) * kD);
  int64_t w = 0;
  const int64_t nk[5][3] = {{T, kD, kD}, {T, kQKV, kD}, {T, kD, kF}, {T, kF, kD}, {U, kD, kD}};
  for (auto& q : nk) {
    const int64_t v = rsx_linear_wgrad_workspace_floats(q[0], q[1], q[2]);
    if (v > w) w = v;
  }
  s.n_wsw = w;
  s.n_wsl = rsx_ln_bwd_workspace_floats(T, kD);
  s.n_wse = rsx_seq_embed_bwd_workspace_floats(T, L, kD);
  s.wsw = take(s.n_wsw); s.wsl = take(s.n_wsl); s.wse = take(s.n_wse);
  s.total = o;
  return s;
}

int64_t n_ptrs(int nl) { return RSX_TW_LAYER0 + 12 * (int64_t)nl + 6 + 1; }

__global__ __launch_bounds__(256) void tw_tail_k(const int64_t* __restrict__ last, int64_t T1, int64_t B,
                                                 const int64_t* __restrict__ tok_user, const int64_t* __restrict__ seg64,
                                                 int64_t* __restrict__ tidx, int64_t* __restrict__ tinv,
                                                 int64_t* __restrict__ tuser, int64_t* __restrict__ tseg) {
  const int64_t T = 2 * T1, R = T1 + B, n = T > 2 * B + 1 ? T : 2 * B + 1;
  for (int64_t i = (int64_t)blockIdx.x * 256 + threadIdx.x; i < n; i += (int64_t)gridDim.x * 256) {
    if (i <= 2 * B) tseg[i] = i <= B ? seg64[i] : T1 + (i - B);
    if (i >= T) continue;
    if (i < R) {
      tidx[i] = i < T1 ? i : T1 + last[i - T1];
      tuser[i] = i < T1 ? tok_user[i] : B + (i - T1);
    }
    if (i < T1) {
      tinv[i] = i;
    } else {
      const int64_t j = tok_user[i] - B;
      tinv[i] = (i - T1 == last[j]) ? T1 + j : R;
    }
  }
}

#define TW_CALL(x)            \
  do {                        \
    const int rc_ = (x);      \
    if (rc_ != 0) return rc_; \
  } while (0)

struct View {
  const void* const* p;
  const float* f(int i) const { return static_cast<const float*>(p[i]); }
  const int64_t* i64(int i) const { return static_cast<const int64_t*>(p[i]); }
};

struct LastQ {
  const float* qkv;
  const uint8_t* kpad;
// ... 82 lines not shown
#pragma unroll
    for (int e = 0; e < kDh; e += 4) {
      const float4 x = *reinterpret_cast<const float4*>(qr + e), y = *reinterpret_cast<const float4*>(kk + e);
      const float4 g = *reinterpret_cast<const float4*>(dor + e), w = *reinterpret_cast<const float4*>(vr + e);
      d += x.x * y.x + x.y * y.y + x.z * y.z + x.w * y.w;
      dv += g.x * w.x + g.y * w.y + g.z * w.z + g.w * w.w;
    }
    p = expf(d * 0.17677669529663687f - lse);
    const uint64_t idx = ((uint64_t)q * kHeads + hd) * 64 + lane;
    dp = a.drop.apply(dv, idx);
  }
  float sdp = p * dp;
  for (int o = 32; o > 0; o >>= 1) sdp += __shfl_xor(sdp, o, 64);
  const float ds = valid ? p * (dp - sdp) * 0.17677669529663687f : 0.0f;
  __shared__ float sP[kHeads][64][kDh + 1];
#pragma unroll
  for (int e = 0; e < kDh; e += 4) {
    float4 kv = make_float4(0.f, 0.f, 0.f, 0.f);
    if (valid) kv = *reinterpret_cast<const float4*>(kk + e);
    sP[hd][lane][e] = ds * kv.x;
    sP[hd][lane][e + 1] = ds * kv.y;
    sP[hd][lane][e + 2] = ds * kv.z;
    sP[hd][lane][e + 3] = ds * kv.w;
  }
  __builtin_amdgcn_wave_barrier();
  __builtin_amdgcn_s_waitcnt(0xc07f);
  float dq_d = 0.0f;
  if (lane < kDh)
    for (int k = 0; k < len; ++k) dq_d += sP[hd][k][lane];
  if (in) {
    float* drow = a.dqkv + kr * kQKV;
    const float pd = valid ? a.drop.apply(p, ((uint64_t)q * kHeads + hd) * 64 + lane) : 0.0f;
#pragma unroll
    for (int e = 0; e < kDh; e += 4) {
      const float4 x = *reinterpret_cast<const float4*>(qr + e), g = *reinterpret_cast<const float4*>(dor + e);
      *reinterpret_cast<float4*>(drow + kD + kDh * hd + e) =
          make_float4(ds * x.x, ds * x.y, ds * x.z, ds * x.w);
      *reinterpret_cast<float4*>(drow + 2 * kD + kDh * hd + e) =
          make_float4(pd * g.x, pd * g.y, pd * g.z, pd * g.w);
    }
    if (lane != qi) {
#pragma unroll
      for (int e = 0; e < kDh; e += 4)
        *reinterpret_cast<float4*>(drow + kDh * hd + e) = make_float4(0.f, 0.f, 0.f, 0.f);
    }
  }
  if (lane < kDh) a.dqkv[q * kQKV + kDh * hd + lane] = dq_d;
}

}

RSX_API int64_t rsx_tower_n_ptrs(int layers) { return n_ptrs(layers); }

RSX_API int64_t rsx_tower_arena_bytes(int64_t T, int64_t U, int layers) {
  if (layers < 1 || layers > kMaxLayers || T < 0 || U < 0) return -1;
  return layout(T, U, layers).total * 4;
}

RSX_API int64_t rsx_tower_bwd_workspace_bytes(int64_t T, int64_t U, int64_t L, int layers, int64_t C) {
  if (layers < 1 || layers > kMaxLayers || T < 0 || U < 0) return -1;
  return bwd_layout(T, U, L, C).total * 4;
}

RSX_API int rsx_tower_fwd(const void* const* p, const int64_t* dims, const float* fargs, const uint64_t* seeds,
                          void* arena, int64_t arena_bytes, float* out, void* stream) {
  RSX_ARG(p && dims && fargs && seeds && arena && out, "null argument");
  const int64_t T = dims[0], U = dims[1], L = dims[2];
  const int nl = (int)dims[3];
  RSX_ARG(nl >= 1 && nl <= kMaxLayers, "1 <= layers <= 8");
  RSX_ARG(T > 0 && U > 0 && L > 0 && L <= 64, "need T, U > 0 and 0 < L <= 64");
  const Layout s = layout(T, U, nl);
  RSX_ARG(arena_bytes >= s.total * 4, "arena too small (rsx_tower_arena_bytes)");
  for (int64_t i = 0; i < n_ptrs(nl) - 1; ++i)
    if (i < RSX_TW_ITEMSEG || i >= RSX_TW_ITEM_PROJ) RSX_ARG(p[i] != nullptr, "null input / parameter pointer");
  const int64_t tB = dims[12], T1 = dims[13];
  const bool tail = tB > 0;
  RSX_ARG(!tail || (U == 2 * tB && T == 2 * T1 && p[n_ptrs(nl) - 1]), "tail needs U = 2B, T = 2 T1 and the last rows");
  const int64_t R = tail ? T1 + tB : T;
  const View v{p};
  float* A = static_cast<float*>(arena);
  const float pd = fargs[0];
  const int pl = RSX_TW_LAYER0 + 12 * nl;
  TW_CALL(rsx_gemm_x3(v.f(RSX_TW_PV), kD, v.f(RSX_TW_ITEM_PROJ), kD, v.f(RSX_TW_ITEM_PROJ + 1), T, kD, kD, kEpiBias,
                      nullptr, 0, 0.0f, 0, A + s.base, kD, stream));
  const int64_t* ids[6];
  const float* tabs[6];
  for (int j = 0; j < 6; ++j) {
    ids[j] = v.i64(RSX_TW_IDS + j);
    tabs[j] = v.f(RSX_TW_TABLES + j);
  }
  TW_CALL(rsx_seq_embed_fwd(A + s.base, ids, tabs, 6, v.f(RSX_TW_GATE), v.f(RSX_TW_POS), v.i64(RSX_TW_TOK_POS),
                            v.f(RSX_TW_EMB_LN), v.f(RSX_TW_EMB_LN + 1), fargs[1], T, L, kD, pd, seeds[0], A + s.x0,
                            A + s.m0, A + s.r0, stream));
  TW_CALL(rsx_ln_fwd(A + s.x0, nullptr, 0.0f, 0, v.f(RSX_TW_LAYER0), v.f(RSX_TW_LAYER0 + 1), fargs[2], 0, T, kD,
                     nullptr, A + s.h0, A + s.mh0, A + s.rh0, stream));
  const float* x = A + s.x0;
  const float* h = A + s.h0;
  const uint8_t* kp = static_cast<const uint8_t*>(p[RSX_TW_TOK_PAD]);
  const int* seg = static_cast<const int*>(p[RSX_TW_SEG32]);
  int64_t* tidx = reinterpret_cast<int64_t*>(A + s.tidx);
  int64_t* tuser = reinterpret_cast<int64_t*>(A + s.tuser);
  int64_t* tseg = reinterpret_cast<int64_t*>(A + s.tseg);
  if (tail) {
    const int64_t n = T > 2 * tB + 1 ? T : 2 * tB + 1;
    int64_t blocks = (n + 255) / 256;
    if (blocks > 4096) blocks = 4096;
    hipLaunchKernelGGL(tw_tail_k, dim3((unsigned)blocks), dim3(256), 0, (hipStream_t)stream,
                       static_cast<const int64_t*>(p[n_ptrs(nl) - 1]), T1, tB, v.i64(RSX_TW_TOK_USER),
                       v.i64(RSX_TW_SEG64), tidx, reinterpret_cast<int64_t*>(A + s.tinv), tuser, tseg);
    RSX_LAUNCHED();
  }
  for (int i = 0; i < nl; ++i) {
    const int q = RSX_TW_LAYER0 + 12 * i;
    const LayerAct& a = s.l[i];
    const uint64_t* sd = seeds + 1 + 4 * i;
    TW_CALL(rsx_gemm_x3(h, kD, v.f(q + 2), kD, v.f(q + 3), T, (int)kQKV, (int)kD, kEpiBias, nullptr, 0, 0.0f, 0,
                        A + a.qkv, kQKV, stream));
    const float* ain = A + a.a;
    const float* xin = x;
    int64_t rows = T;
    if (tail && i == nl - 1) {
      TW_CALL(rsx_mha_fwd_x3(A + a.qkv, kp, seg, tB, 64, kHeads, kDh, 1, pd, sd[0], A + s.aR, A + a.lse, stream));
      LastQ lq{};
      lq.qkv = A + a.qkv; lq.kpad = kp; lq.seg64 = v.i64(RSX_TW_SEG64); lq.last = v.i64(n_ptrs(nl) - 1);
      lq.out = A + s.aR + T1 * kD; lq.lse = A + s.lseq; lq.T1 = T1; lq.B = tB; lq.drop = rsx::make_dropout(pd, sd[0]);
      hipLaunchKernelGGL(tw_lastq_fwd_k, dim3((unsigned)tB), dim3(256), 0, (hipStream_t)stream, lq);
      RSX_LAUNCHED();
      TW_CALL(rsx_gather_rows(x, kD, tidx, R, kD, 0, 0.0f, A + s.xR, nullptr, stream));
      ain = A + s.aR;
      xin = A + s.xR;
      rows = R;
    } else {
      TW_CALL(rsx_mha_fwd_x3(A + a.qkv, kp, seg, U, 64, kHeads, kDh, 1, pd, sd[0], A + a.a, A + a.lse, stream));
    }
    TW_CALL(rsx_gemm_x3_addln(ain, kD, v.f(q + 4), kD, v.f(q + 5), rows, kD, kD, xin, kD, pd, sd[1], v.f(q + 6),
                              v.f(q + 7), fargs[3 + 2 * i], A + a.xs, kD, A + a.hs, kD, A + a.m2, A + a.r2, stream));
    TW_CALL(rsx_gemm_x3(A + a.hs, kD, v.f(q + 8), kD, v.f(q + 9), rows, (int)kF, (int)kD, kEpiGeluDrop, A + a.gg, kF,
                        pd, sd[2], A + a.act, kF, stream));
    TW_CALL(rsx_gemm_x3(A + a.act, kF, v.f(q + 10), kF, v.f(q + 11), rows, (int)kD, (int)kF, kEpiBias, nullptr, 0,
                        0.0f, 0, A + a.f, kD, stream));
    if (i + 1 < nl) {
      TW_CALL(rsx_ln_fwd(A + a.xs, A + a.f, pd, sd[3], v.f(q + 12), v.f(q + 13), fargs[2 + 2 * (i + 1)], 0, T, kD,
                         A + a.xn, A + a.hn, A + a.mn, A + a.rn, stream));
      h = A + a.hn;
    } else {
      TW_CALL(rsx_ln_fwd(A + a.xs, A + a.f, pd, sd[3], nullptr, nullptr, 0.0f, 0, rows, kD, A + a.xn, nullptr,
                         nullptr, nullptr, stream));
    }
    x = A + a.xn;
  }
  const float* w0 = v.f(pl);
  TW_CALL(rsx_gemm_x3(v.f(RSX_TW_PROFILE), kD, w0 + kD, 2 * kD, v.f(pl + 1), U, kD, kD, kEpiBias, nullptr, 0, 0.0f, 0,
                      A + s.prof, kD, stream));
  TW_CALL(rsx_gemm_x3_rowadd(x, kD, w0, 2 * kD, nullptr, R, kD, kD, A + s.prof, kD,
                             tail ? tuser : v.i64(RSX_TW_TOK_USER), A + s.hp, kD, stream));
  TW_CALL(rsx_ln_fwd(A + s.hp, nullptr, 0.0f, 0, v.f(pl + 2), v.f(pl + 3), fargs[2 + 2 * nl], kActGelu, R, kD, nullptr,
                     A + s.g, A + s.mo, A + s.ro, stream));
  TW_CALL(rsx_gemm_x3(A + s.g, kD, v.f(pl + 4), kD, v.f(pl + 5), R, kD, kD, kEpiBias, nullptr, 0, 0.0f, 0, A + s.o, kD,
                      stream));
  TW_CALL(rsx_gather_rows(A + s.o, kD, nullptr, R, kD, 1, 1e-12f, out, A + s.nrm, stream));
  return 0;
}

RSX_API int rsx_tower_bwd(const void* const* p, const int64_t* dims, const float* fargs, const uint64_t* seeds,
                          const void* arena, const float* out, const float* dout, void* const* grads, void* ws,
                          int64_t ws_bytes, void* stream) {
  RSX_ARG(p && dims && fargs && seeds && arena && out && dout && grads && ws, "null argument");
  const int64_t T = dims[0], U = dims[1], L = dims[2], C = dims[4], Uq = dims[5];
  const int nl = (int)dims[3];
  RSX_ARG(nl >= 1 && nl <= kMaxLayers, "1 <= layers <= 8");
  RSX_ARG(T > 0 && U > 0 && L > 0 && L <= 64 && C >= 0 && Uq >= 0, "bad sizes");
  const Layout s = layout(T, U, nl);
  const BwdLayout b = bwd_layout(T, U, L, C);
  RSX_ARG(ws_bytes >= b.total * 4, "workspace too small (rsx_tower_bwd_workspace_bytes)");
  const int pl = RSX_TW_LAYER0 + 12 * nl;
  for (int64_t i = RSX_TW_ITEM_PROJ; i < n_ptrs(nl) - 1; ++i) RSX_ARG(grads[i] != nullptr, "null parameter gradient");
  const int64_t tB = dims[12], T1 = dims[13];
  const bool tail = tB > 0;
  RSX_ARG(!tail || (U == 2 * tB && T == 2 * T1), "tail needs U = 2B and T = 2 T1");
  const int64_t R = tail ? T1 + tB : T;
  RSX_ARG(grads[RSX_TW_GATE] && grads[RSX_TW_PROFILE], "null gate / profile gradient");
  RSX_ARG(C == 0 || (p[RSX_TW_ITEMSEG] && p[RSX_TW_ITEMSEG + 1] && p[RSX_TW_ITEMSEG + 2] && p[RSX_TW_ITEMSEG + 3] &&
                     p[RSX_TW_ITEMSEG + 4]), "item-id gradient plan required");
  const View v{p};
  const float* A = static_cast<const float*>(arena);
  float* W = static_cast<float*>(ws);
  auto G = [&](int i) { return static_cast<float*>(grads[i]); };
  const float pd = fargs[0];
  float* wsw = W + b.wsw;
  float* wsl = W + b.wsl;
  const uint8_t* kp = static_cast<const uint8_t*>(p[RSX_TW_TOK_PAD]);
  const int* seg = static_cast<const int*>(p[RSX_TW_SEG32]);
  auto wgrad = [&](const float* dy, int64_t ldy, const float* xx, int64_t ldx, int64_t t, int64_t n, int64_t k,
                   float* dw, int64_t ldw, float* db) {
    return rsx_linear_wgrad_x3(dy, ldy, xx, ldx, t, n, k, dw, ldw, db, 0, wsw, b.n_wsw, stream);
  };
  auto tn = [&](const float* dy, int64_t ldy, const float* w, int64_t ldw, int64_t m, int n, int k, float* c,
                int64_t ldc) {
    return rsx_gemm_x3_tn(dy, ldy, w, ldw, nullptr, m, n, k, kEpiBias, nullptr, 0, 0.0f, 0, c, ldc, stream);
  };
  TW_CALL(rsx_scatter_rows(dout, out, A + s.nrm, nullptr, R, kD, 1, 1e-12f, 0, -1, W + b.dO, kD, stream));
  TW_CALL(tn(W + b.dO, kD, v.f(pl + 4), kD, R, kD, kD, W + b.dG, kD));
  TW_CALL(wgrad(W + b.dO, kD, A + s.g, kD, R, kD, kD, G(pl + 4), kD, G(pl + 5)));
  TW_CALL(rsx_ln_bwd(A + s.hp, A + s.mo, A + s.ro, v.f(pl + 2), v.f(pl + 3), kActGelu, W + b.dG, nullptr, 0.0f, 0, R,
                     kD, W + b.dHp, nullptr, G(pl + 2), G(pl + 3), wsl, b.n_wsl, stream));
  const float* w0 = v.f(pl);
  const float* xl = A + s.l[nl - 1].xn;
  const int64_t* useg = tail ? reinterpret_cast<const int64_t*>(A + s.tseg) : v.i64(RSX_TW_SEG64);
  TW_CALL(rsx_segment_sum_rows(W + b.dHp, kD, nullptr, useg, nullptr, U, kD, nullptr, -1, W + b.dProf, kD, 0, stream));
  TW_CALL(tn(W + b.dHp, kD, w0, 2 * kD, R, kD, kD, W + b.dX, kD));
  TW_CALL(tn(W + b.dProf, kD, w0 + kD, 2 * kD, U, kD, kD, G(RSX_TW_PROFILE), kD));
  TW_CALL(wgrad(W + b.dHp, kD, xl, kD, R, kD, kD, G(pl), 2 * kD, nullptr));
  TW_CALL(wgrad(W + b.dProf, kD, v.f(RSX_TW_PROFILE), kD, U, kD, kD, G(pl) + kD, 2 * kD, G(pl + 1)));
  float* dX = W + b.dX;
  float* dXs = W + b.dXs;
  float* dH = W + b.dH;
  for (int i = nl - 1; i >= 0; --i) {
    const int q = RSX_TW_LAYER0 + 12 * i;
    const LayerAct& a = s.l[i];
    const uint64_t* sd = seeds + 1 + 4 * i;
    const bool tl = tail && i == nl - 1;
    const int64_t rows = tl ? R : T;
    float* dF = W + b.dF;
    if (i == nl - 1) {
      TW_CALL(rsx_dropout_bwd(dX, rows, kD, pd, sd[3], dF, stream));
// ... 7 lines not shown
    float* dHs = W + b.dHs;
    TW_CALL(rsx_gemm_x3_tn(dF, kD, v.f(q + 10), kF, nullptr, rows, (int)kF, (int)kD, kEpiDgeluDrop,
                           const_cast<float*>(A + a.gg), kF, pd, sd[2], dPre, kF, stream));
    TW_CALL(wgrad(dF, kD, A + a.act, kF, rows, kD, kF, G(q + 10), kF, G(q + 11)));
    TW_CALL(wgrad(dPre, kF, A + a.hs, kD, rows, kF, kD, G(q + 8), kD, G(q + 9)));
    TW_CALL(tn(dPre, kF, v.f(q + 8), kD, rows, (int)kD, (int)kF, dHs, kD));
    float* dRes = W + b.dRes;
    float* dA = W + b.dA;
    float* dQKV = W + b.dQKV;
    if (tl) {
      float* dXR = W + b.dXR;
      float* dAR = W + b.dAR;
      (void)hipMemsetAsync(dXR + R * kD, 0, kD * sizeof(float), (hipStream_t)stream);
      TW_CALL(rsx_ln_bwd(A + a.xs, A + a.m2, A + a.r2, v.f(q + 6), v.f(q + 7), 0, dHs, dXs, pd, sd[1], R, kD, dXR, dRes,
                         G(q + 6), G(q + 7), wsl, b.n_wsl, stream));
      TW_CALL(tn(dRes, kD, v.f(q + 4), kD, R, kD, kD, dAR, kD));
      TW_CALL(wgrad(dRes, kD, A + s.aR, kD, R, kD, kD, G(q + 4), kD, G(q + 5)));
      const int64_t* tinv = reinterpret_cast<const int64_t*>(A + s.tinv);
      TW_CALL(rsx_gather_rows(dXR, kD, tinv, T, kD, 0, 0.0f, dX, nullptr, stream));
      TW_CALL(rsx_mha_bwd_x3(A + a.qkv, kp, seg, A + s.aR, A + a.lse, dAR, tB, 64, kHeads, kDh, 1, pd, sd[0], dQKV,
                             stream));
      LastQ lq{};
      lq.qkv = A + a.qkv; lq.kpad = kp; lq.seg64 = v.i64(RSX_TW_SEG64); lq.last = v.i64(n_ptrs(nl) - 1);
      lq.lse = const_cast<float*>(A + s.lseq); lq.dout = dAR + T1 * kD; lq.dqkv = dQKV; lq.T1 = T1; lq.B = tB;
      lq.drop = rsx::make_dropout(pd, sd[0]);
      hipLaunchKernelGGL(tw_lastq_bwd_k, dim3((unsigned)tB), dim3(256), 0, (hipStream_t)stream, lq);
      RSX_LAUNCHED();
    } else {
      TW_CALL(rsx_ln_bwd(A + a.xs, A + a.m2, A + a.r2, v.f(q + 6), v.f(q + 7), 0, dHs, dXs, pd, sd[1], T, kD, dX, dRes,
                         G(q + 6), G(q + 7), wsl, b.n_wsl, stream));
      TW_CALL(tn(dRes, kD, v.f(q + 4), kD, T, kD, kD, dA, kD));
      TW_CALL(wgrad(dRes, kD, A + a.a, kD, T, kD, kD, G(q + 4), kD, G(q + 5)));
      TW_CALL(rsx_mha_bwd_x3(A + a.qkv, kp, seg, A + a.a, A + a.lse, dA, U, 64, kHeads, kDh, 1, pd, sd[0], dQKV,
                             stream));
    }
    const float* h_in = (i == 0) ? A + s.h0 : A + s.l[i - 1].hn;
    TW_CALL(tn(dQKV, kQKV, v.f(q + 2), kD, T, (int)kD, (int)kQKV, dH, kD));
    TW_CALL(wgrad(dQKV, kQKV, h_in, kD, T, kQKV, kD, G(q + 2), kD, G(q + 3)));
  }
  float* dX0 = dXs;
  TW_CALL(rsx_ln_bwd(A + s.x0, A + s.mh0, A + s.rh0, v.f(RSX_TW_LAYER0), v.f(RSX_TW_LAYER0 + 1), 0, dH, dX, 0.0f, 0, T,
                     kD, dX0, nullptr, G(RSX_TW_LAYER0), G(RSX_TW_LAYER0 + 1), wsl, b.n_wsl, stream));
  const int64_t* ids[6];
  const float* tabs[6];
  float* dtabs[6];
  for (int j = 0; j < 6; ++j) {
    ids[j] = v.i64(RSX_TW_IDS + j);
    tabs[j] = v.f(RSX_TW_TABLES + j);
    dtabs[j] = j == 0 ? nullptr : G(RSX_TW_TABLES + j);
  }
  const int64_t rows[6] = {dims[6], dims[7], dims[8], dims[9], dims[10], dims[11]};
  const int64_t pad[6] = {0, 0, 0, 0, 0, 0};
  float* dBase = W + b.dBase;
  TW_CALL(rsx_seq_embed_bwd(A + s.base, ids, tabs, rows, pad, 6, v.f(RSX_TW_GATE), v.f(RSX_TW_POS),
                            v.i64(RSX_TW_TOK_POS), v.f(RSX_TW_EMB_LN), A + s.m0, A + s.r0, fargs[1], T, L, kD, pd,
                            seeds[0], dX0, dBase, dtabs, G(RSX_TW_GATE), G(RSX_TW_POS), G(RSX_TW_EMB_LN),
                            G(RSX_TW_EMB_LN + 1), W + b.wse, b.n_wse, stream));
  if (C > 0) {
    const int64_t* plan = v.i64(RSX_TW_ITEMSEG);
    TW_CALL(rsx_segment_sum_rows(dBase, kD, plan, v.i64(RSX_TW_ITEMSEG + 1), v.i64(RSX_TW_ITEMSEG + 2), C, kD, nullptr,
                                 -1, W + b.part, kD, 0, stream));
    TW_CALL(rsx_segment_sum_rows(W + b.part, kD, v.i64(RSX_TW_ITEMSEG + 2), v.i64(RSX_TW_ITEMSEG + 3),
                                 v.i64(RSX_TW_ITEMSEG + 4), Uq, kD, v.f(RSX_TW_GATE), 0, G(RSX_TW_TABLES), kD, 1,
                                 stream));
  }
  if (grads[RSX_TW_PV]) TW_CALL(tn(dBase, kD, v.f(RSX_TW_ITEM_PROJ), kD, T, kD, kD, G(RSX_TW_PV), kD));
  TW_CALL(wgrad(dBase, kD, v.f(RSX_TW_PV), kD, T, kD, kD, G(RSX_TW_ITEM_PROJ), kD, G(RSX_TW_ITEM_PROJ + 1)));
  return 0;
}
```

### llm-driven_content-based-feature_recommendation_system_amd/dist.py

```python
from __future__ import annotations

import contextlib
import os

import torch
import torch.distributed as dist

from . import _native as N
from . import ops


_LOCAL_ONLY = False


def world():
    if not _LOCAL_ONLY and dist.is_available() and dist.is_initialized():
        return dist.get_rank(), dist.get_world_size()
    return 0, 1


@contextlib.contextmanager
def local_only():
    global _LOCAL_ONLY
    prev, _LOCAL_ONLY = _LOCAL_ONLY, True
# ... 236 lines not shown
    for sp in specs:
        if sp is None:
            sizes.append(None)
            continue
        shape, dt = sp
        n = 1
        for d in shape:
            n *= d
        nb = n * _ELEM[dt]
        sizes.append((total, nb))
        total += (nb + 255) // 256 * 256
    buf = torch.empty(max(total, 256), device=dev, dtype=torch.uint8)
    out = []
    for sp, sz in zip(specs, sizes):
        if sp is None:
            out.append(None)
            continue
        o, nb = sz
        out.append(buf[o:o + nb].view(sp[1]).view(sp[0]))
    return out


def _prepare_step_index_device(batch, pretrained_vecs, pretrained_lookup, n_items) -> StepIndex:
    from .tower_code.v1_usertower_train import _SEQ_ID_KEYS, _STATIC_KEYS

    lib = N.lib()
    rank, ws = world()
    pm = batch["padding_mask"]
    B, L = pm.shape
    dev = pm.device
    pm8 = ops._c(pm).view(torch.uint8) if pm.dtype == torch.bool else ops._c(pm.to(torch.uint8))
    tgt = ops._c(batch["target_ids"].to(torch.int64))
    seq = [ops._c(batch[k].to(torch.int64)) for k in _SEQ_ID_KEYS]
    nb = lib.rsx_step_index_workspace_bytes(B, L, n_items)
    wsb = torch.empty(nb, device=dev, dtype=torch.uint8)
    tloc = torch.empty(B * L + 1, device=dev, dtype=torch.int32)
    N.check(lib.rsx_step_index_count(N.ptr(pm8), N.ptr(tgt), N.ptr(seq[0]), B, L, n_items, N.ptr(wsb), nb,
                                     N.ptr(tloc), N.stream()), "step_index_count")
    if ws > 1:
        tglob = torch.empty(ws, B * L + 1, device=dev, dtype=torch.int32)
        all_gather_into(list(tglob.unbind(0)), tloc, group=index_group())
    else:
        tglob = tloc
    totals = torch.empty(8 + ws, device=dev, dtype=torch.int64)
    N.check(lib.rsx_step_index_totals(N.ptr(tglob), ws, B, L, n_items, N.ptr(wsb), nb, N.ptr(totals), N.stream()),
            "step_index_totals")
    tot = totals.tolist()
    T, Nr, D, E, U, C, err = tot[:7]
    if err:
        raise IndexError(f"step index: a target / item id outside [0, {n_items})")
    i64, i32, u8, f32 = torch.int64, torch.int32, torch.uint8, torch.float32
    specs = [((T,), i64), ((T,), i64), ((T,), i64), ((T,), u8), ((B + 1,), i32), ((B + 1,), i64), ((Nr,), i64),
             ((B,), i64), ((2 * T,), i64), ((2 * T,), i64), ((2 * T,), i64), ((2 * T,), u8), ((2 * B + 1,), i32),
             ((2 * B + 1,), i64), ((6, 2 * T), i64), (((2 * T, 128), f32) if pretrained_vecs is None else None),
             ((2 * T,), i64), ((C + 1,), i64), ((C,), i64), ((U + 1,), i64), ((U,), i64), ((D,), i64), ((D,), f32),
             ((Nr,), i32), ((Nr,), i32), ((Nr,), i32), ((Nr,), i32), ((E,), i32), ((E,), i32), ((E,), i32),
             ((D,), i32), ((D,), i32), ((B,), i32)]
    out = _carve(specs, dev)
    lk = ops._c(pretrained_lookup) if pretrained_vecs is None else None
    N.check(lib.rsx_step_index_fill(N.ptr(pm8), N.ptr(tgt), N.ptr_array(seq), N.ptr(lk),
                                    lk.stride(0) if lk is not None else 0, B, L, n_items,
                                    N.i64_array([T, Nr, D, E, U, C]), N.ptr(wsb), nb, N.ptr_array(out), N.stream()),
            "step_index_fill")
    pk, pk2 = _Packed(), _Packed()
    pk.flat, pk.tok_user, pk.tok_pos, pk.tok_pad, pk.seg_off, pk.seg_off64, pk.valid_tok, pk.last_tok = out[:8]
    pk.B, pk.L = B, L
    (pk2.flat, pk2.tok_user, pk2.tok_pos, pk2.tok_pad, pk2.seg_off, pk2.seg_off64) = out[8:14]
    pk2.B, pk2.L = 2 * B, L
    pk2.item_seg = tuple(out[16:21])
    tok_ids = list(out[14].unbind(0))
    if pretrained_vecs is None:
        pv_tok = out[15]
    else:
        pv_tok = pk.take(pretrained_vecs)
        pv_tok = torch.cat([pv_tok, pv_tok])
    static = static_inputs(batch)
    ix = StepIndex()
    ix.packed = (pk, pk2, tok_ids, pv_tok, static)
    ix.B = B
    ix.counts = [int(c) for c in tot[8:8 + ws]]
    ix.n_glob = sum(ix.counts)
    ix.groups = None
    if ix.n_glob > 0:
        ix.groups = ops.TargetGroups.from_arrays(*out[21:32], n_rows=Nr)
    ix.last_t = out[32]
    ix.t_glob_last = all_gather_var(ix.last_t, [B] * ws, group=index_group() if ws > 1 else None)
    ix.wsb = wsb
    return ix


def _device_lookup_ok(pretrained_vecs, lookup, device) -> bool:
    if pretrained_vecs is not None:
        return True
    return (lookup is not None and lookup.device == device and lookup.dtype == torch.float32 and lookup.dim() == 2
            and lookup.shape[1] == 128 and lookup.stride(1) == 1 and not lookup.requires_grad)


def prepare_step_index(batch, pretrained_vecs=None, pretrained_lookup=None, n_items=None) -> StepIndex:
    from .tower_code.v1_usertower_train import pack_inputs

    if n_items is None and pretrained_lookup is not None:
        n_items = pretrained_lookup.shape[0]
    if (_DEVICE_INDEX and n_items is not None and batch["item_ids"].is_cuda
            and batch["padding_mask"].shape[1] <= 64 and _device_lookup_ok(pretrained_vecs, pretrained_lookup,
                                                                          batch["item_ids"].device)):
        return _prepare_step_index_device(batch, pretrained_vecs, pretrained_lookup, int(n_items))
    rank, ws = world()
    device = batch["item_ids"].device
    B = batch["item_ids"].shape[0]
    target_ids = batch["target_ids"]
    ix = StepIndex()
    ix.packed = pack_inputs(batch, pretrained_vecs, pretrained_lookup)
    pk = ix.packed[0]
    ix.B = B
    grp = index_group() if ws > 1 else None
    ix.counts = all_gather_counts(pk.valid_tok.numel(), device, group=grp)
    ix.n_glob = sum(ix.counts)
    ix.groups = None
    if ix.n_glob > 0:
        t_loc = target_ids.reshape(-1)[pk.flat[pk.valid_tok]]
        user_loc = pk.tok_user[pk.valid_tok] + rank * B
        t_glob = all_gather_var(t_loc, ix.counts, group=grp)
        ix.groups = ops.TargetGroups(t_loc, user_loc, t_cols=t_glob)
    ix.last_t = target_ids.reshape(-1)[pk.flat[pk.last_tok]].to(torch.int32)
    ix.t_glob_last = all_gather_var(ix.last_t, [B] * ws, group=grp)
# ... 173 lines not shown
```

### llm-driven_content-based-feature_recommendation_system_amd/ops.py

```python
from __future__ import annotations

import ctypes
import math
import os
import weakref

import torch

from . import _native as N

NCE_PLAIN = 0
NCE_MASK_ITEM = 2
NCE_MASK_ITEM_USER = 6
NCE_SUPCON = 9

_NSPLIT_FWD = 8
_NSPLIT_FWD_GROUPED = int(os.environ.get("RSX_NCE_NSPLIT_FWD", "2"))
if _NSPLIT_FWD_GROUPED not in (1, 2, 4, 8):
    raise ValueError("RSX_NCE_NSPLIT_FWD must be 1, 2, 4 or 8 (the fused forward's supported partial-slot counts)")
_NSPLIT_BWD = 8

NCE_PRECISIONS = {"fp32": 0, "bf16x3": 1, "f16": 2}
_nce_precision = os.environ.get("RSX_NCE_PRECISION", "f16")
if _nce_precision not in NCE_PRECISIONS:
# ... 51 lines not shown


def _rows2(fn, name, t):
    _f32(fn, name, t)
    if t.dim() != 2:
        raise ValueError(f"{fn}: {name} must be 2-D, got shape {tuple(t.shape)}")
    return t.shape[1]


def _ln_args(fn, x, res, weight, bias):
    _f32(fn, "x", x)
    if x.dim() < 1:
        raise ValueError(f"{fn}: x must have a last dimension")
    if res is not None:
        _f32(fn, "res", res, x)
        if res.shape != x.shape:
            raise ValueError(f"{fn}: res has shape {tuple(res.shape)}, x {tuple(x.shape)}")
    D = x.shape[-1]
    _f32_vec(fn, "weight", weight, D, x)
    _f32_vec(fn, "bias", bias, D, x)


def _tensor_key(ts):
    return tuple((t, t.data_ptr(), t._version) for t in ts)


def _key_eq(a, b) -> bool:
    if a is None or len(a) != len(b):
        return False
    for x, y in zip(a, b):
        if isinstance(x, tuple):
            if x[0] is not y[0] or x[1:] != y[1:]:
                return False
        elif x != y:
            return False
    return True


def _zeros_group(likes):
    shapes = [None if t is None else t.shape for t in likes]
    sizes = [0 if t is None else (t.numel() + 3) // 4 * 4 for t in likes]
    total = sum(sizes)
    if total == 0:
        return [None] * len(likes)
    ref = next(t for t in likes if t is not None)
    flat = torch.zeros(total, device=ref.device, dtype=torch.float32)
    out, o = [], 0
    for shp, n, t in zip(shapes, sizes, likes):
        out.append(None if t is None else flat[o:o + t.numel()].view(shp))
        o += n
    return out


class _SeqEmbed(torch.autograd.Function):
    @staticmethod
    def forward(ctx, base, gate, pos, ln_w, ln_b, ids, cfg, tok_pos, *tables):
        eps, p_drop, seed, padding_idx, L, tab0_seg = cfg
        N.ensure_device(base)
        D = base.shape[-1]
        T = base.numel() // D
        base = _c(base)
        ids = [_c(t) for t in ids]
        tables = [_c(t) for t in tables]
        out = torch.empty_like(base)
        mean = torch.empty(T, device=base.device, dtype=torch.float32)
        rstd = torch.empty_like(mean)
        gate = _c(gate)
        with timed("seq_embed_fwd"):
            rc = N.lib().rsx_seq_embed_fwd(
                N.ptr(base), N.ptr_array(ids), N.ptr_array(tables), len(tables), N.ptr(gate), N.ptr(pos),
                N.ptr(tok_pos), N.ptr(ln_w), N.ptr(ln_b), eps, T, L, D, p_drop, seed, N.ptr(out), N.ptr(mean),
                N.ptr(rstd), N.stream())
        N.check(rc, "seq_embed_fwd")
        ctx.save_for_backward(base, gate, pos, ln_w, mean, rstd, tok_pos, *ids, *tables)
        ctx.cfg = (eps, p_drop, seed, padding_idx, len(tables), T, L, D)
        ctx.tab0_seg = tab0_seg
        return out

    @staticmethod
    def backward(ctx, dout):
        eps, p_drop, seed, padding_idx, nt, T, L, D = ctx.cfg
        saved = ctx.saved_tensors
        base, gate, pos, ln_w, mean, rstd, tok_pos = saved[:7]
        ids = list(saved[7:7 + nt])
        tables = list(saved[7 + nt:7 + 2 * nt])
        dout = _c(dout)
        need = ctx.needs_input_grad
        dbase = torch.empty_like(base) if need[0] else None
        dgate, dpos, dlnw, dlnb, *dtabs = _zeros_group(
            [gate if need[1] else None, pos if need[2] else None, ln_w if need[3] else None,
             ln_w if need[4] else None] + [t if need[8 + j] else None for j, t in enumerate(tables)])
        rows = N.i64_array([t.shape[0] for t in tables])
        seg0 = ctx.tab0_seg if (nt > 0 and dtabs[0] is not None) else None
        if seg0 is not None and dbase is None:
            dbase = torch.empty_like(base)
        kern_tabs = ([None] + dtabs[1:]) if seg0 is not None else dtabs
        nws = N.lib().rsx_seq_embed_bwd_workspace_floats(T, L, D)
        ws = torch.empty(nws, device=base.device, dtype=torch.float32)
        with timed("seq_embed_bwd"):
            rc = N.lib().rsx_seq_embed_bwd(
                N.ptr(base), N.ptr_array(ids), N.ptr_array(tables), rows,
                N.i64_array(padding_idx), nt, N.ptr(gate), N.ptr(pos), N.ptr(tok_pos), N.ptr(ln_w), N.ptr(mean),
                N.ptr(rstd), eps, T, L, D, p_drop, seed, N.ptr(dout), N.ptr(dbase), N.ptr_array(kern_tabs),
                N.ptr(dgate), N.ptr(dpos), N.ptr(dlnw), N.ptr(dlnb), N.ptr(ws), nws, N.stream())
        N.check(rc, "seq_embed_bwd")
        if seg0 is not None:
            perm, cb, chunk_ids, ch_off, uniq = seg0
            part = torch.empty(chunk_ids.numel(), D, device=base.device, dtype=torch.float32)
            rc = N.lib().rsx_segment_sum_rows(N.ptr(dbase), D, N.ptr(perm), N.ptr(cb), N.ptr(chunk_ids),
                                              chunk_ids.numel(), D, None, -1, N.ptr(part), D, 0, N.stream())
            N.check(rc, "segment_sum_rows(chunks)")
            rc = N.lib().rsx_segment_sum_rows(N.ptr(part), D, N.ptr(chunk_ids), N.ptr(ch_off), N.ptr(uniq),
                                              uniq.numel(), D, N.ptr(gate), padding_idx[0], N.ptr(dtabs[0]),
                                              dtabs[0].stride(0), 1, N.stream())
            N.check(rc, "segment_sum_rows(ids)")
        if not need[0]:
            dbase = None
        return (dbase, dgate, dpos, dlnw, dlnb, None, None, None, *dtabs)


_SEG_CHUNK = 64


def sort_segments(ids):
    ids = ids.reshape(-1)
    dev = ids.device
    srt, perm = torch.sort(ids, stable=True)
    uniq, cnt = torch.unique_consecutive(srt, return_counts=True)
    seg_off = torch.zeros(uniq.numel() + 1, device=dev, dtype=torch.int64)
    seg_off[1:] = torch.cumsum(cnt, 0)
    nch = (cnt + _SEG_CHUNK - 1) // _SEG_CHUNK
    ch_off = torch.zeros(uniq.numel() + 1, device=dev, dtype=torch.int64)
    ch_off[1:] = torch.cumsum(nch, 0)
    total = int(ch_off[-1])
    ch_seg = torch.repeat_interleave(torch.arange(uniq.numel(), device=dev), nch, output_size=total)
    k = torch.arange(total, device=dev)
    cb = torch.empty(total + 1, device=dev, dtype=torch.int64)
    cb[:-1] = seg_off[ch_seg] + _SEG_CHUNK * (k - ch_off[ch_seg])
    cb[-1] = ids.numel()
    return perm, cb, k, ch_off, uniq


def seq_embed(base, ids, tables, gate, pos, ln_w, ln_b, eps=1e-5, p_drop=0.0, padding_idx=None, tok_pos=None,
              tab0_seg=None):
    if padding_idx is None:
        padding_idx = [-1] * len(tables)
    padding_idx = [(-1 if p is None else int(p)) for p in padding_idx]
    seed = next_seed() if p_drop > 0 else 0
    if tok_pos is None:
        L = base.shape[1]
        pos = pos[:L]
    else:
        L = pos.shape[0]
        tok_pos = _c(tok_pos)
    cfg = (float(eps), float(p_drop), seed, padding_idx, int(L), tab0_seg)
    return _SeqEmbed.apply(base, gate, pos, ln_w, ln_b, list(ids), cfg, tok_pos, *tables)


MHA_PRECISIONS = ("fp32", "bf16x3")
_mha_precision = os.environ.get("RSX_MHA_PRECISION", "bf16x3")
assert _mha_precision in MHA_PRECISIONS, _mha_precision


def set_mha_precision(p: str) -> None:
    global _mha_precision
    assert p in MHA_PRECISIONS, p
    _mha_precision = p


def mha_precision() -> str:
    return _mha_precision


def _mha_x3(Dh):
    return _mha_precision == "bf16x3" and Dh == 32


def _mha_x3_fwd(Dh):
    return _mha_precision == "bf16x3" and Dh in (32, 64)


class _MHA(torch.autograd.Function):
    @staticmethod
    def forward(ctx, qkv, key_pad, seg_off, H, causal, p_drop, seed, max_len=None):
        N.ensure_device(qkv)
        qkv = _c(qkv)
        D3 = qkv.shape[-1]
        T = qkv.numel() // D3
        D = D3 // 3
        Dh = D // H
        if seg_off is None:
            B, L = qkv.shape[0], qkv.shape[1]
        else:
            B, L = seg_off.numel() - 1, int(max_len) if max_len else 64
        out = torch.empty(qkv.shape[:-1] + (D,), device=qkv.device, dtype=torch.float32)
        lse = torch.empty(T, H, device=qkv.device, dtype=torch.float32)
        kp = None
        if key_pad is not None:
            kp = _c(key_pad.to(torch.uint8)) if key_pad.dtype != torch.uint8 else _c(key_pad)
        fn = N.lib().rsx_mha_fwd_x3 if _mha_x3_fwd(Dh) else N.lib().rsx_mha_fwd
        rc = fn(N.ptr(qkv), N.ptr(kp), N.ptr(seg_off), B, L, H, Dh, int(causal), p_drop, seed, N.ptr(out), N.ptr(lse),
                N.stream())
        N.check(rc, "mha_fwd")
        ctx.save_for_backward(qkv, kp, seg_off, out, lse)
        ctx.cfg = (B, L, H, Dh, int(causal), p_drop, seed)
        return out

    @staticmethod
# ... 1220 lines not shown
    p = float(p_drop) if training else 0.0
    shp = h.shape
    h2 = h.reshape(-1, shp[-1])
    if (h2.is_cuda and h2.shape[0] > 0 and _x3_ok(w1.shape[0], w1.shape[1]) and _x3_ok(w2.shape[0], w2.shape[1])
            and _x3_ok(w2.shape[1], w2.shape[0]) and _x3_ok(w1.shape[1], w1.shape[0])):
        seed = next_seed() if p > 0 else 0
        f = _FFN.apply(h2, w1, b1, w2, b2, p, seed)
        return f.reshape(*shp[:-1], w2.shape[0])
    return linear_tok(torch.nn.functional.dropout(torch.nn.functional.gelu(linear_tok(h, w1, b1)), p, training),
                      w2, b2)


_TOWER_NATIVE = os.environ.get("RSX_TOWER_NATIVE", "1") != "0"


def tower_params(model):
    ps = [model.item_proj.weight, model.item_proj.bias, model.item_id_emb.weight, model.time_emb.weight,
          model.type_emb.weight, model.color_emb.weight, model.graphic_emb.weight, model.section_emb.weight,
          model.pos_emb.weight, model.emb_ln.weight, model.emb_ln.bias]
    for layer in model.transformer_encoder.layers:
        sa = layer.self_attn
        ps += [layer.norm1.weight, layer.norm1.bias, sa.in_proj_weight, sa.in_proj_bias, sa.out_proj.weight,
               sa.out_proj.bias, layer.norm2.weight, layer.norm2.bias, layer.linear1.weight, layer.linear1.bias,
               layer.linear2.weight, layer.linear2.bias]
    op = model.output_proj
    ps += [op[0].weight, op[0].bias, op[1].weight, op[1].bias, op[3].weight, op[3].bias]
    return ps


def tower_native_ok(model, packed, pv):
    if not (_TOWER_NATIVE and _gemm_precision == "bf16x3" and _mha_precision == "bf16x3" and _ADDLN_ON):
        return None
    if getattr(packed, "item_seg", None) is None or not pv.is_cuda:
        return None
    layers = model.transformer_encoder.layers
    if model.d_model != 128 or not (1 <= len(layers) <= 8) or model.pos_emb.weight.shape[0] > 64:
        return None
    for layer in layers:
        if (layer.self_attn.num_heads != 4 or layer.linear1.out_features != 256 or not layer.norm_first
                or layer.activation_relu_or_gelu != 2):
            return None
    ps = tower_params(model)
    ok = all(p.requires_grad and p.dtype == torch.float32 and p.is_contiguous() for p in ps)
    return ps if ok else None


_ADDLN_ON = os.environ.get("RSX_LINEAR_ADDLN", "1") != "0"


class _TowerPacked(torch.autograd.Function):

    @staticmethod
    def forward(ctx, pv, gate, profile, cfg, *params):
        packed, tok_ids, p_drop, eps, nl, tail_last = cfg
        T, D = pv.shape
        U = packed.seg_off.numel() - 1
        dev = pv.device
        pv = _c(pv)
        gate = _c(gate)
        profile = _c(profile)
        perm, cb, chunk_ids, ch_off, uniq = packed.item_seg
        inputs = ([pv] + list(tok_ids) + [packed.tok_pos, packed.tok_pad, packed.seg_off, packed.seg_off64,
                                            packed.tok_user, gate, profile, perm, cb, chunk_ids, ch_off, uniq])
        tail_last = None if tail_last is None else _c(tail_last)
        ptrs = N.ptr_array(inputs + list(params) + [tail_last])
        tabs = params[2:8]
        tB = 0 if tail_last is None else tail_last.numel()
        R = T // 2 + tB if tB else T
        dims = N.i64_array([T, U, params[8].shape[0], nl, chunk_ids.numel(), uniq.numel()]
                           + [t.shape[0] for t in tabs] + [tB, T // 2])
        fargs = (ctypes.c_float * (len(eps) + 1))(p_drop, *eps)
        seeds = [next_seed() if p_drop > 0 else 0 for _ in range(1 + 4 * nl)]
        seeds_arr = (ctypes.c_uint64 * len(seeds))(*seeds)
        nbytes = N.lib().rsx_tower_arena_bytes(T, U, nl)
        arena = torch.empty(nbytes, device=dev, dtype=torch.uint8)
        out = torch.empty(R, D, device=dev, dtype=torch.float32)
        with timed("tower_fwd"):
            rc = N.lib().rsx_tower_fwd(ptrs, dims, fargs, seeds_arr, N.ptr(arena), nbytes, N.ptr(out), N.stream())
        N.check(rc, "tower_fwd")
        ctx.save_for_backward(pv, gate, profile, out, *params)
        ctx.keep = (inputs + [tail_last], arena, ptrs, dims, fargs, seeds_arr)
        ctx.shape = (T, U, params[8].shape[0], nl, chunk_ids.numel())
        return out

    @staticmethod
    def backward(ctx, dout):
        if ctx.keep is None:
            raise RuntimeError("tower_packed: a second backward through the same forward (retain_graph=True) "
                               "is not supported; run the forward again")
        pv, gate, profile, out, *params = ctx.saved_tensors
        inputs, arena, ptrs, dims, fargs, seeds_arr = ctx.keep
        T, U, L, nl, C = ctx.shape
        dev = dout.device
        dout = _c(dout)
        acc_like = [gate] + [params[i] for i in range(2, 11)]
        dgate, *acc = _zeros_group(acc_like)
        written = _empty_group([params[0], params[1]] + list(params[11:]) + [profile])
        dprofile = written[-1]
        dparams = [written[0], written[1]] + acc + written[2:-1]
        dpv = torch.empty_like(pv) if ctx.needs_input_grad[0] else None
        grads = [dpv] + [None] * 11 + [dgate, dprofile] + [None] * 5 + dparams + [None]
        nws = N.lib().rsx_tower_bwd_workspace_bytes(T, U, L, nl, C)
        ws = torch.empty(nws, device=dev, dtype=torch.uint8)
        with timed("tower_bwd"):
            rc = N.lib().rsx_tower_bwd(ptrs, dims, fargs, seeds_arr, N.ptr(arena), N.ptr(out), N.ptr(dout),
                                       N.ptr_array(grads), N.ptr(ws), nws, N.stream())
        N.check(rc, "tower_bwd")
        ctx.keep = None
        return (dpv, dgate, dprofile, None) + tuple(dparams)


def _empty_group(likes):
    sizes = [0 if t is None else (t.numel() + 3) // 4 * 4 for t in likes]
    if sum(sizes) == 0:
        return [None] * len(likes)
    ref = next(t for t in likes if t is not None)
    flat = torch.empty(sum(sizes), device=ref.device, dtype=torch.float32)
    out, o = [], 0
    for t, n in zip(likes, sizes):
        out.append(None if t is None else flat[o:o + t.numel()].view(t.shape))
        o += n
    return out


def tower_packed(model, packed, pv_tok, tok_ids, s_g, profile, p_drop, params=None, tail_last=None):
    layers = model.transformer_encoder.layers
    eps = [model.emb_ln.eps]
    for layer in layers:
        eps += [layer.norm1.eps, layer.norm2.eps]
    eps.append(model.output_proj[1].eps)
    cfg = (packed, [_c(t) for t in tok_ids], float(p_drop), [float(e) for e in eps], len(layers), tail_last)
    return _TowerPacked.apply(pv_tok, s_g, profile, cfg, *(params if params is not None else tower_params(model)))


@torch.no_grad()
def bert_embed_packed(embeddings, ids, tok_pos):
    word = embeddings.word_embeddings.weight
    ids = _index("bert_embed_packed", "ids", ids, word)
    tok_pos = _index("bert_embed_packed", "tok_pos", tok_pos, word, ids.numel())
    N.ensure_device(ids)
    D = word.shape[1]
    T = ids.numel()
    out = torch.empty(T, D, device=ids.device, dtype=torch.float32)
    ln = embeddings.LayerNorm
    rc = N.lib().rsx_embed3_ln(N.ptr(word), word.stride(0), N.ptr(_c(embeddings.position_embeddings.weight)),
                               N.ptr(_c(embeddings.token_type_embeddings.weight[0])), N.ptr(ln.weight),
                               N.ptr(ln.bias), float(ln.eps), N.ptr(_c(ids)), N.ptr(_c(tok_pos)), T, D, N.ptr(out),
                               N.stream())
    N.check(rc, "embed3_ln")
    if embeddings.training and embeddings.dropout.p > 0:
        out = torch.nn.functional.dropout(out, embeddings.dropout.p, True)
    return out


class _SegmentMean(torch.autograd.Function):

    @staticmethod
    def forward(ctx, x, seg, tok_seg, inv):
        U = inv.numel()
        D = x.shape[1]
        s = torch.empty(U, D, device=x.device, dtype=torch.float32)
        rc = N.lib().rsx_segment_sum_rows(N.ptr(x), x.stride(0), None, N.ptr(seg), None, U, D, None, -1, N.ptr(s),
                                          s.stride(0), 0, N.stream())
        N.check(rc, "segment_sum_rows(mean)")
        ctx.save_for_backward(tok_seg, inv)
        return s * inv.unsqueeze(1)

    @staticmethod
    def backward(ctx, dv):
        tok_seg, inv = ctx.saved_tensors
        return gather_rows(_c(dv * inv.unsqueeze(1)), tok_seg), None, None, None


def segment_mean(x, seg, tok_seg, counts):
    _rows2("segment_mean", "x", x)
    if counts.device != x.device:
        raise RuntimeError(f"segment_mean: counts is on {counts.device}, expected {x.device}")
    seg = _index("segment_mean", "seg", seg, x, counts.numel() + 1)
    tok_seg = _index("segment_mean", "tok_seg", tok_seg, x, x.shape[0])
    N.ensure_device(x)
    inv = 1.0 / torch.clamp(counts, min=1e-9)
    return _SegmentMean.apply(_c(x), _c(seg), _c(tok_seg), inv.float())


# ... 826 lines not shown
```

### llm-driven_content-based-feature_recommendation_system_amd/tower_code/v1_refine_usertower.py

```python
from __future__ import annotations

import os

import torch
import torch.nn as nn
import torch.nn.functional as F

from .. import ops


def get_logq_probs(raw_probs, device="cpu"):
    import numpy as np
    p = np.nan_to_num(np.asarray(raw_probs, dtype=np.float64), nan=0.0) + 1e-6
    p = p / p.sum()
    full = np.zeros(len(p) + 1, dtype=np.float32)
    full[1:] = np.log(p).astype(np.float32)
    full[0] = -20.0
    return torch.tensor(full, dtype=torch.float32).to(device)


def _frame(src):
    import pandas as pd
    return src.copy() if isinstance(src, pd.DataFrame) else pd.read_parquet(src)

# ... 204 lines not shown
        return torch.triu(torch.ones(seq_len, seq_len, device=device, dtype=torch.bool), diagonal=1)

    def _encoder_stack(self, x, key_pad, p, seg_off=None):
        return encoder_stack(self.transformer_encoder.layers, x, key_pad, p, self.training, causal=True,
                             seg_off=seg_off)

    def forward(self, pretrained_vecs, item_ids, time_bucket_ids, type_ids, color_ids, graphic_ids, section_ids,
                age_bucket, price_bucket, cnt_bucket, recency_bucket, channel_ids, club_status_ids, news_freq_ids,
                fn_ids, active_ids, cont_feats, padding_mask=None, training_mode=True):
        B, seq_len = item_ids.shape
        p = self.dropout_rate if self.training else 0.0

        s_g = torch.sigmoid(self.seq_gate) * self._seq_gate_mask

        base = ops.linear_tok(pretrained_vecs, self.item_proj.weight, self.item_proj.bias)
        x = ops.seq_embed(
            base,
            [item_ids, time_bucket_ids, type_ids, color_ids, graphic_ids, section_ids],
            [self.item_id_emb.weight, self.time_emb.weight, self.type_emb.weight, self.color_emb.weight,
             self.graphic_emb.weight, self.section_emb.weight],
            s_g, self.pos_emb.weight[:seq_len], self.emb_ln.weight, self.emb_ln.bias, eps=self.emb_ln.eps,
            p_drop=p, padding_idx=[0, 0, 0, 0, 0, 0])
        output = self._encoder_stack(x, padding_mask, p)

        user_profile_vec = self._static_profile(age_bucket, price_bucket, cnt_bucket, recency_bucket, channel_ids,
                                                club_status_ids, news_freq_ids, fn_ids, active_ids, cont_feats, p)

        lin0, ln, lin3 = self.output_proj[0], self.output_proj[1], self.output_proj[3]
        D = self.d_model
        if training_mode:
            dev = output.device
            tok_user = torch.arange(B, device=dev).repeat_interleave(seq_len)
            seg = torch.arange(0, B * seq_len + 1, seq_len, device=dev)
            h = ops.profile_linear(output.reshape(B * seq_len, D), user_profile_vec, lin0.weight, lin0.bias,
                                   tok_user, seg).view(B, seq_len, -1)
        else:
            h = ops.linear_tok(torch.cat([output[:, -1, :], user_profile_vec], dim=1), lin0.weight, lin0.bias)
        h = ops.layer_norm(h, ln.weight, ln.bias, ln.eps, act=ops.ACT_GELU_ERF)
        final_vec = ops.linear_tok(h, lin3.weight, lin3.bias)
        return ops.l2_normalize(final_vec)

    def _static_profile(self, age_bucket, price_bucket, cnt_bucket, recency_bucket, channel_ids, club_status_ids,
                        news_freq_ids, fn_ids, active_ids, cont_feats, p, rows=None):
        ids = [age_bucket, price_bucket, cnt_bucket, recency_bucket, channel_ids, club_status_ids, news_freq_ids,
               fn_ids, active_ids]
        return ops.static_profile(self, ids, cont_feats, p, rows)

    def forward_packed(self, packed, pretrained_tok, tok_ids, age_bucket, price_bucket, cnt_bucket, recency_bucket,
                       channel_ids, club_status_ids, news_freq_ids, fn_ids, active_ids, cont_feats, tail_last=None):
        p = self.dropout_rate if self.training else 0.0
        s_g = torch.sigmoid(self.seq_gate) * self._seq_gate_mask
        profile = self._static_profile(age_bucket, price_bucket, cnt_bucket, recency_bucket, channel_ids,
                                       club_status_ids, news_freq_ids, fn_ids, active_ids, cont_feats, p, packed.B)
        params = ops.tower_native_ok(self, packed, pretrained_tok) if torch.is_grad_enabled() else None
        if params is not None:
            return ops.tower_packed(self, packed, pretrained_tok, tok_ids, s_g, profile, p, params, tail_last)
        base = ops.linear_tok(pretrained_tok, self.item_proj.weight, self.item_proj.bias)
        x = ops.seq_embed(
            base, tok_ids,
            [self.item_id_emb.weight, self.time_emb.weight, self.type_emb.weight, self.color_emb.weight,
             self.graphic_emb.weight, self.section_emb.weight],
            s_g, self.pos_emb.weight, self.emb_ln.weight, self.emb_ln.bias, eps=self.emb_ln.eps, p_drop=p,
            padding_idx=[0, 0, 0, 0, 0, 0], tok_pos=packed.tok_pos, tab0_seg=getattr(packed, "item_seg", None))
        x = self._encoder_stack(x, packed.tok_pad, p, seg_off=packed.seg_off)
        lin0, ln, lin3 = self.output_proj[0], self.output_proj[1], self.output_proj[3]
        D = self.d_model
        h = ops.profile_linear(x, profile, lin0.weight, lin0.bias, packed.tok_user, packed.seg_off64)
        h = ops.layer_norm(h, ln.weight, ln.bias, ln.eps, act=ops.ACT_GELU_ERF)
        out = ops.l2_normalize(ops.linear_tok(h, lin3.weight, lin3.bias))
        if tail_last is not None:
            T1 = out.shape[0] // 2
            keep = torch.cat([torch.arange(T1, device=out.device), tail_last + T1])
            out = ops.gather_rows(out, keep, unique=True)
        return out


class PackedTokens:

    def __init__(self, padding_mask: torch.Tensor):
        B, L = padding_mask.shape
        dev = padding_mask.device
        valid = ~padding_mask
        cnt = valid.sum(1)
        last = (cnt - 1).clamp(min=0)
        ar = torch.arange(B, device=dev)
        need_extra = padding_mask[ar, last]
        sel = valid.clone()
        sel[ar, last] = sel[ar, last] | need_extra
        self.flat = sel.reshape(-1).nonzero().squeeze(1)
        self.tok_user = torch.div(self.flat, L, rounding_mode="floor")
        self.tok_pos = self.flat % L
        self.tok_pad = padding_mask.reshape(-1)[self.flat].to(torch.uint8)
        seg = torch.zeros(B + 1, device=dev, dtype=torch.int64)
        seg[1:] = torch.cumsum(torch.bincount(self.tok_user, minlength=B), 0)
        self.seg_off = seg.to(torch.int32)
        self.seg_off64 = seg
        self.valid_tok = (self.tok_pad == 0).nonzero().squeeze(1)
        pad_len = L - cnt
        self.last_tok = seg[:-1] + torch.where(need_extra, torch.zeros_like(last), last - pad_len)
        self.B, self.L = B, L

    def take(self, t: torch.Tensor) -> torch.Tensor:
        return t.reshape((-1,) + tuple(t.shape[2:]))[self.flat]


def _as_keys(t):
    return t.reshape(-1).to(torch.int32)


def inbatch_corrected_logq_loss(user_emb, item_tower_emb, target_ids, user_ids, log_q_tensor, temperature=0.1,
                                lambda_logq=1.0):
    tgt = target_ids.reshape(-1)
    batch_item_emb = ops.gather_rows(item_tower_emb, tgt)
    bias = None
    if lambda_logq > 0.0:
        bias = log_q_tensor[tgt] * lambda_logq
# ... 87 lines not shown
```

Measured before the change: 555,100.

## Project pretrained item vectors once per distinct item and gather by index

Adds an ItemRows path where the pretrained token vectors are kept one row per distinct item, with a per-token index. The item projection runs on distinct rows only, and the embedding forward and backward kernels gather the projected base row through base_idx. A new segment-sum variant writes the per-item base gradient in the same pass that accumulates the item-id table gradient. This cuts projection FLOPs and memory when items repeat across sequences, at the cost of an extra indirection load per token and an ABI change across the tower arena and pointer layout.

```diff
diff --git a/include/recsys_amd.h b/include/recsys_amd.h
--- a/include/recsys_amd.h
+++ b/include/recsys_amd.h
@@ -13,14 +13,14 @@
 const char* rsx_target_arch(void);
 const char* rsx_build_hash(void);
 
-int rsx_seq_embed_fwd(const float* base, const int64_t* const* ids, const float* const* tables, int ntab,
-                      const float* gate, const float* pos, const int64_t* tok_pos, const float* ln_w,
-                      const float* ln_b, float eps, int64_t T, int64_t L, int64_t D, float p_drop, uint64_t seed,
-                      float* out, float* mean, float* rstd, void* stream);
+int rsx_seq_embed_fwd(const float* base, const int64_t* base_idx, const int64_t* const* ids,
+                      const float* const* tables, int ntab, const float* gate, const float* pos,
+                      const int64_t* tok_pos, const float* ln_w, const float* ln_b, float eps, int64_t T, int64_t L,
+                      int64_t D, float p_drop, uint64_t seed, float* out, float* mean, float* rstd, void* stream);
 
 int64_t rsx_seq_embed_bwd_workspace_floats(int64_t T, int64_t L, int64_t D);
-int rsx_seq_embed_bwd(const float* base, const int64_t* const* ids, const float* const* tables,
-                      const int64_t* table_rows, const int64_t* padding_idx, int ntab, const float* gate,
+int rsx_seq_embed_bwd(const float* base, const int64_t* base_idx, const int64_t* const* ids,
+                      const float* const* tables, const int64_t* table_rows, const int64_t* padding_idx, int ntab, const float* gate,
                       const float* pos, const int64_t* tok_pos, const float* ln_w, const float* mean,
                       const float* rstd, float eps, int64_t T, int64_t L, int64_t D, float p_drop, uint64_t seed,
                       const float* dout, float* dbase, float* const* dtables, float* dgate, float* dpos,
@@ -245,6 +245,9 @@
 int rsx_segment_sum_rows(const float* src, int64_t ld_src, const int64_t* perm, const int64_t* seg_off,
                          const int64_t* rows, int64_t nseg, int64_t D, const float* scale, int64_t skip_row,
                          float* dst, int64_t ld_dst, int accumulate, void* stream);
+int rsx_segment_sum_rows2(const float* src, int64_t ld_src, const int64_t* perm, const int64_t* seg_off,
+                          const int64_t* rows, int64_t nseg, int64_t D, const float* scale, int64_t skip_row,
+                          float* dst, int64_t ld_dst, int accumulate, float* raw, int64_t ld_raw, void* stream);
 
 int rsx_loss_combine(const float* s_main, const float* s_un, const float* s_sup, const float* cnt, float inv_n,
                      float inv_b, float lambda_sup, float lambda_cl, float* total, float* logs, void* stream);
@@ -276,11 +279,11 @@
 
 enum {
   RSX_TW_PV = 0, RSX_TW_IDS = 1, RSX_TW_TOK_POS = 7, RSX_TW_TOK_PAD = 8, RSX_TW_SEG32 = 9, RSX_TW_SEG64 = 10,
-  RSX_TW_TOK_USER = 11, RSX_TW_GATE = 12, RSX_TW_PROFILE = 13, RSX_TW_ITEMSEG = 14, RSX_TW_ITEM_PROJ = 19,
-  RSX_TW_TABLES = 21, RSX_TW_POS = 27, RSX_TW_EMB_LN = 28, RSX_TW_LAYER0 = 30
+  RSX_TW_TOK_USER = 11, RSX_TW_GATE = 12, RSX_TW_PROFILE = 13, RSX_TW_ITEMSEG = 14, RSX_TW_UIDX = 19,
+  RSX_TW_ITEM_PROJ = 20, RSX_TW_TABLES = 22, RSX_TW_POS = 28, RSX_TW_EMB_LN = 29, RSX_TW_LAYER0 = 31
 };
 int64_t rsx_tower_n_ptrs(int layers);
-int64_t rsx_tower_arena_bytes(int64_t T, int64_t U, int layers);
+int64_t rsx_tower_arena_bytes(int64_t T, int64_t U, int layers, int64_t pv_rows);
 int64_t rsx_tower_bwd_workspace_bytes(int64_t T, int64_t U, int64_t L, int layers, int64_t C);
 int rsx_tower_fwd(const void* const* p, const int64_t* dims, const float* fargs, const uint64_t* seeds, void* arena,
                   int64_t arena_bytes, float* out, void* stream);
diff --git a/llm-driven_content-based-feature_recommendation_system_amd/_native.py b/llm-driven_content-based-feature_recommendation_system_amd/_native.py
--- a/llm-driven_content-based-feature_recommendation_system_amd/_native.py
+++ b/llm-driven_content-based-feature_recommendation_system_amd/_native.py
@@ -20,17 +20,17 @@
 c_d = ctypes.c_double
 c_u64 = ctypes.c_uint64
 
-ABI_VERSION = 9
+ABI_VERSION = 10
 
 _SIGS = {
     "rsx_last_error": (ctypes.c_char_p, []),
     "rsx_abi_version": (c_i, []),
     "rsx_target_arch": (ctypes.c_char_p, []),
     "rsx_build_hash": (ctypes.c_char_p, []),
-    "rsx_seq_embed_fwd": (c_i, [c_p, c_p, c_p, c_i, c_p, c_p, c_p, c_p, c_p, c_f, c_i64, c_i64, c_i64, c_f, c_u64,
+    "rsx_seq_embed_fwd": (c_i, [c_p, c_p, c_p, c_p, c_i, c_p, c_p, c_p, c_p, c_p, c_f, c_i64, c_i64, c_i64, c_f, c_u64,
                                 c_p, c_p, c_p, c_p]),
     "rsx_seq_embed_bwd_workspace_floats": (c_i64, [c_i64, c_i64, c_i64]),
-    "rsx_seq_embed_bwd": (c_i, [c_p, c_p, c_p, c_p, c_p, c_i, c_p, c_p, c_p, c_p, c_p, c_p, c_f, c_i64, c_i64,
+    "rsx_seq_embed_bwd": (c_i, [c_p, c_p, c_p, c_p, c_p, c_p, c_i, c_p, c_p, c_p, c_p, c_p, c_p, c_f, c_i64, c_i64,
                                 c_i64, c_f, c_u64, c_p, c_p, c_p, c_p, c_p, c_p, c_p, c_p, c_i64, c_p]),
     "rsx_mha_fwd": (c_i, [c_p, c_p, c_p, c_i64, c_i64, c_i64, c_i64, c_i, c_f, c_u64, c_p, c_p, c_p]),
     "rsx_mha_bwd": (c_i, [c_p, c_p, c_p, c_p, c_p, c_p, c_i64, c_i64, c_i64, c_i64, c_i, c_f, c_u64, c_p, c_p]),
@@ -112,7 +112,7 @@
     "rsx_clip_adamw": (c_i, [c_i, c_p, c_p, c_p, c_p, c_p, c_p, c_p, c_p, c_p, c_p, c_p, c_p, c_p, c_f, c_p, c_i64,
                              c_p, c_p]),
     "rsx_tower_n_ptrs": (c_i64, [c_i]),
-    "rsx_tower_arena_bytes": (c_i64, [c_i64, c_i64, c_i]),
+    "rsx_tower_arena_bytes": (c_i64, [c_i64, c_i64, c_i, c_i64]),
     "rsx_tower_bwd_workspace_bytes": (c_i64, [c_i64, c_i64, c_i64, c_i, c_i64]),
     "rsx_tower_fwd": (c_i, [c_p, c_p, c_p, c_p, c_p, c_i64, c_p, c_p]),
     "rsx_tower_bwd": (c_i, [c_p, c_p, c_p, c_p, c_p, c_p, c_p, c_p, c_p, c_i64, c_p]),
@@ -141,6 +141,8 @@
     "rsx_dcn_train_head": (c_i, [c_p, c_i64, c_p, c_p, c_p, c_p, c_i64, c_i, c_p, c_p, c_p, c_p, c_i64, c_p, c_p, c_p,
                                  c_p]),
     "rsx_segment_sum_rows": (c_i, [c_p, c_i64, c_p, c_p, c_p, c_i64, c_i64, c_p, c_i64, c_p, c_i64, c_i, c_p]),
+    "rsx_segment_sum_rows2": (c_i, [c_p, c_i64, c_p, c_p, c_p, c_i64, c_i64, c_p, c_i64, c_p, c_i64, c_i, c_p, c_i64,
+                                    c_p]),
     "rsx_scatter_rows": (c_i, [c_p, c_p, c_p, c_p, c_i64, c_i64, c_i, c_f, c_i, c_i64, c_p, c_i64, c_p]),
     "rsx_hnm_mine": (c_i, [c_p, c_p, c_p, c_i64, c_i64, c_i64, c_f, c_f, c_p, ctypes.c_size_t, c_p, c_p, c_p, c_p]),
     "rsx_hnm_workspace_bytes": (c_i64, [c_i64]),
diff --git a/llm-driven_content-based-feature_recommendation_system_amd/csrc/rows.hip b/llm-driven_content-based-feature_recommendation_system_amd/csrc/rows.hip
--- a/llm-driven_content-based-feature_recommendation_system_amd/csrc/rows.hip
+++ b/llm-driven_content-based-feature_recommendation_system_amd/csrc/rows.hip
@@ -102,13 +102,14 @@
   return (unsigned)b;
 }
 
-template <int D>
+template <int D, bool RAW = false>
 __global__ __launch_bounds__(256) void segsum_rows_k(const float* __restrict__ src, int64_t ld_src,
                                                     const int64_t* __restrict__ perm,
                                                     const int64_t* __restrict__ seg,
                                                     const int64_t* __restrict__ rows, int64_t nseg,
                                                     const float* __restrict__ scale, int64_t skip,
-                                                    float* __restrict__ dst, int64_t ld_dst, int accumulate) {
+                                                    float* __restrict__ dst, int64_t ld_dst, int accumulate,
+                                                    float* __restrict__ raw = nullptr, int64_t ld_raw = 0) {
   constexpr int LPR = RowGeo<D>::LPR, RPW = RowGeo<D>::RPW;
   const int lane = threadIdx.x & 63, sub = lane / LPR, c = lane % LPR;
   const int64_t wave_g = (int64_t)blockIdx.x * 4 + (threadIdx.x >> 6);
@@ -118,7 +119,7 @@
     const int64_t u = u0 + sub;
     if (u >= nseg) continue;
     const int64_t row = rows ? rows[u] : u;
-    if (row == skip) continue;
+    if (!RAW && row == skip) continue;
     float4 acc = make_float4(0.f, 0.f, 0.f, 0.f);
     const int64_t k1 = seg[u + 1];
     int64_t k = seg[u];
@@ -146,6 +147,10 @@
 #pragma unroll
       for (int i = 0; i < 15; ++i)
         if (i < n) { acc.x += x[i].x; acc.y += x[i].y; acc.z += x[i].z; acc.w += x[i].w; }
+    }
+    if (RAW) {
+      reinterpret_cast<float4*>(raw + u * ld_raw)[c] = acc;
+      if (row == skip) continue;
     }
     float4* d = reinterpret_cast<float4*>(dst + row * ld_dst) + c;
     float4 v = make_float4(sc * acc.x, sc * acc.y, sc * acc.z, sc * acc.w);
@@ -269,7 +274,28 @@
 #define RSX_SS(DD)                                                                                            \
   if (D == DD)                                                                                                \
     hipLaunchKernelGGL(segsum_rows_k<DD>, dim3(g), dim3(256), 0, st, src, ld_src, perm, seg_off, rows, nseg, \
-                       scale, skip_row, dst, ld_dst, accumulate);
+                       scale, skip_row, dst, ld_dst, accumulate, (float*)nullptr, (int64_t)0);
+  RSX_SS(64) RSX_SS(128) RSX_SS(256)
+#undef RSX_SS
+  RSX_LAUNCHED();
+  return 0;
+}
+
+RSX_API int rsx_segment_sum_rows2(const float* src, int64_t ld_src, const int64_t* perm, const int64_t* seg_off,
+                                  const int64_t* rows, int64_t nseg, int64_t D, const float* scale, int64_t skip_row,
+                                  float* dst, int64_t ld_dst, int accumulate, float* raw, int64_t ld_raw,
+                                  void* stream) {
+  RSX_ARG(src && seg_off && dst && raw, "null tensor");
+  RSX_ARG(D == 64 || D == 128 || D == 256, "D must be 64, 128 or 256");
+  RSX_ARG(ld_src >= D && ld_dst >= D && ld_raw >= D && ld_src % 4 == 0 && ld_dst % 4 == 0 && ld_raw % 4 == 0,
+          "bad leading dimensions");
+  if (nseg == 0) return 0;
+  hipStream_t st = (hipStream_t)stream;
+  const unsigned g = grid_for(nseg, (int)D);
+#define RSX_SS(DD)                                                                                                  \
+  if (D == DD)                                                                                                      \
+    hipLaunchKernelGGL((segsum_rows_k<DD, true>), dim3(g), dim3(256), 0, st, src, ld_src, perm, seg_off, rows, nseg, \
+                       scale, skip_row, dst, ld_dst, accumulate, raw, ld_raw);
   RSX_SS(64) RSX_SS(128) RSX_SS(256)
 #undef RSX_SS
   RSX_LAUNCHED();
diff --git a/llm-driven_content-based-feature_recommendation_system_amd/csrc/rsx_errors.hip b/llm-driven_content-based-feature_recommendation_system_amd/csrc/rsx_errors.hip
--- a/llm-driven_content-based-feature_recommendation_system_amd/csrc/rsx_errors.hip
+++ b/llm-driven_content-based-feature_recommendation_system_amd/csrc/rsx_errors.hip
@@ -15,7 +15,7 @@
 
 RSX_API const char* rsx_last_error(void) { return rsx::g_err; }
 
-RSX_API int rsx_abi_version(void) { return 9; }
+RSX_API int rsx_abi_version(void) { return 10; }
 
 RSX_API const char* rsx_target_arch(void) { return "gfx950"; }
 
diff --git a/llm-driven_content-based-feature_recommendation_system_amd/csrc/seq_embed.hip b/llm-driven_content-based-feature_recommendation_system_amd/csrc/seq_embed.hip
--- a/llm-driven_content-based-feature_recommendation_system_amd/csrc/seq_embed.hip
+++ b/llm-driven_content-based-feature_recommendation_system_amd/csrc/seq_embed.hip
@@ -9,6 +9,7 @@
 
 struct FwdArgs {
   const float* base;
+  const int64_t* base_idx;
   const int64_t* ids[kMaxTab];
   const float* tab[kMaxTab];
   const float* gate;
@@ -77,7 +78,7 @@
 template <int D>
 __device__ __forceinline__ float4 build_row(const FwdArgs& a, int64_t r, int c, const float* g) {
   float4 x = make_float4(0.f, 0.f, 0.f, 0.f);
-  if (a.base) x = ldg4(a.base + r * D + 4 * c);
+  if (a.base) x = ldg4(a.base + (a.base_idx ? ldg8(a.base_idx + r) : r) * D + 4 * c);
 #pragma unroll
   for (int j = 0; j < kMaxTab; ++j) {
     if (j < a.ntab && g[j] != 0.0f) {
@@ -127,19 +128,21 @@
   }
 }
 
-template <int D, int U, int NL, bool FULL = false>
+template <int D, int U, int NL, bool FULL = false, bool BI = false>
 __device__ __forceinline__ void fwd_groups(const FwdArgs& a, const int64_t* const* ids_l, const float* const* tab_l,
                                            const float* g_l, int64_t r0, int sub, int c, float4 w, float4 bb,
                                            bool do_ln) {
   constexpr int RPW = 64 / (D / 4);
   const bool has_pos = FULL || a.pos, has_base = FULL || a.base;
-  int64_t rr[U];
+  int64_t rr[U], rb[U];
   int64_t id[U][NL > 0 ? NL : 1];
   int lp[U];
 #pragma unroll
   for (int u = 0; u < U; ++u) {
     const int64_t r = r0 + u * RPW + sub;
     rr[u] = r < a.T ? r : a.T - 1;
+    if (FULL) rb[u] = BI ? ldg8(a.base_idx + rr[u]) : rr[u];
+    else rb[u] = (a.base && a.base_idx) ? ldg8(a.base_idx + rr[u]) : rr[u];
 #pragma unroll
     for (int k = 0; k < NL; ++k) id[u][k] = ldg8(ids_l[k] + rr[u]);
     if (FULL) lp[u] = (int)ldg8(a.tok_pos + rr[u]);
@@ -148,7 +151,7 @@
   float4 x[U];
 #pragma unroll
   for (int u = 0; u < U; ++u)
-    x[u] = has_base ? ldg4(a.base + rr[u] * D + 4 * c) : make_float4(0.f, 0.f, 0.f, 0.f);
+    x[u] = has_base ? ldg4(a.base + rb[u] * D + 4 * c) : make_float4(0.f, 0.f, 0.f, 0.f);
   float4 e[U][NL > 0 ? NL : 1];
 #pragma unroll
   for (int k = 0; k < NL; ++k)
@@ -214,6 +217,11 @@
     return;
   }
   if (nl == 2 && a.base && a.pos && a.tok_pos && do_ln) {
+    if (a.base_idx) {
+      for (int64_t r0 = wave_g * (RPW * U); r0 < a.T; r0 += nwaves * (RPW * U))
+        fwd_groups<D, U, 2, true, true>(a, ids_l, tab_l, g_l, r0, sub, c, w, bb, true);
+      return;
+    }
     for (int64_t r0 = wave_g * (RPW * U); r0 < a.T; r0 += nwaves * (RPW * U))
       fwd_groups<D, U, 2, true>(a, ids_l, tab_l, g_l, r0, sub, c, w, bb, true);
     return;
@@ -275,13 +283,15 @@
   const int c = cx.c;
   const bool need_e = cx.do_ln || a.dgate;
   const bool need_l = (f.pos && cx.do_ln) || a.dpos;
-  int64_t rc[U];
+  int64_t rc[U], rb[U];
   int lp[U];
   int64_t id[U][NS];
+  const bool base_ix = cx.do_ln && f.base && f.base_idx;
 #pragma unroll
   for (int u = 0; u < U; ++u) {
     const int64_t ru = r00 + (u * NW + cx.wave) * RPW + cx.sub;
     rc[u] = ru < cx.r_end ? ru : cx.r_begin;
+    rb[u] = base_ix ? ldg8(f.base_idx + rc[u]) : rc[u];
     lp[u] = need_l ? (f.tok_pos ? (int)f.tok_pos[rc[u]] : (int)(rc[u] % f.L)) : 0;
 #pragma unroll
     for (int k = 0; k < NS; ++k)
@@ -295,7 +305,7 @@
     xv[u] = make_float4(0.f, 0.f, 0.f, 0.f);
     muv[u] = 0.0f; rsv[u] = 0.0f;
     if (cx.do_ln) {
-      if (f.base) xv[u] = ldg4(f.base + rc[u] * D + 4 * c);
+      if (f.base) xv[u] = ldg4(f.base + rb[u] * D + 4 * c);
       muv[u] = f.mean[rc[u]];
       rsv[u] = f.rstd[rc[u]];
     }
@@ -792,11 +802,13 @@
   return o;
 }
 
-bool fill_fwd(FwdArgs& a, const float* base, const int64_t* const* ids, const float* const* tabs, int ntab,
-              const float* gate, const float* pos, const int64_t* tok_pos, const float* ln_w, const float* ln_b,
-              float eps, int64_t T, int64_t L, float* out, float* mean, float* rstd, float p_drop, uint64_t seed) {
+bool fill_fwd(FwdArgs& a, const float* base, const int64_t* base_idx, const int64_t* const* ids,
+              const float* const* tabs, int ntab, const float* gate, const float* pos, const int64_t* tok_pos,
+              const float* ln_w, const float* ln_b, float eps, int64_t T, int64_t L, float* out, float* mean,
+              float* rstd, float p_drop, uint64_t seed) {
   if (ntab < 0 || ntab > kMaxTab) return false;
   a.base = base;
+  a.base_idx = base ? base_idx : nullptr;
   for (int j = 0; j < kMaxTab; ++j) {
     a.ids[j] = (j < ntab) ? ids[j] : nullptr;
     a.tab[j] = (j < ntab) ? tabs[j] : nullptr;
@@ -865,10 +877,11 @@
   return n;
 }
 
-RSX_API int rsx_seq_embed_fwd(const float* base, const int64_t* const* ids, const float* const* tables, int ntab,
-                              const float* gate, const float* pos, const int64_t* tok_pos, const float* ln_w,
-                              const float* ln_b, float eps, int64_t T, int64_t L, int64_t D, float p_drop,
-                              uint64_t seed, float* out, float* mean, float* rstd, void* stream) {
+RSX_API int rsx_seq_embed_fwd(const float* base, const int64_t* base_idx, const int64_t* const* ids,
+                              const float* const* tables, int ntab, const float* gate, const float* pos,
+                              const int64_t* tok_pos, const float* ln_w, const float* ln_b, float eps, int64_t T,
+                              int64_t L, int64_t D, float p_drop, uint64_t seed, float* out, float* mean,
+                              float* rstd, void* stream) {
   RSX_ARG(out != nullptr, "out is null");
   RSX_ARG(T >= 0 && L > 0 && L <= 64, "need T >= 0 and 0 < L <= 64");
   RSX_ARG(D == 64 || D == 128 || D == 256, "D must be 64, 128 or 256");
@@ -878,7 +891,8 @@
   for (int j = 0; j < ntab; ++j) RSX_ARG(ids[j] != nullptr && tables[j] != nullptr, "null table/ids");
   if (T == 0) return 0;
   FwdArgs a;
-  fill_fwd(a, base, ids, tables, ntab, gate, pos, tok_pos, ln_w, ln_b, eps, T, L, out, mean, rstd, p_drop, seed);
+  fill_fwd(a, base, base_idx, ids, tables, ntab, gate, pos, tok_pos, ln_w, ln_b, eps, T, L, out, mean, rstd, p_drop,
+           seed);
   hipStream_t st = (hipStream_t)stream;
   GatherEvents& ge = gather_events();
   std::pair<hipEvent_t, hipEvent_t> evp{nullptr, nullptr};
@@ -909,8 +923,8 @@
   return blocks * (L * D + kSmallMax + 2 * D + kMaxTab) + kKeyBlocksMax * 64 * D;
 }
 
-RSX_API int rsx_seq_embed_bwd(const float* base, const int64_t* const* ids, const float* const* tables,
-                              const int64_t* table_rows, const int64_t* padding_idx, int ntab, const float* gate,
+RSX_API int rsx_seq_embed_bwd(const float* base, const int64_t* base_idx, const int64_t* const* ids,
+                              const float* const* tables, const int64_t* table_rows, const int64_t* padding_idx, int ntab, const float* gate,
                               const float* pos, const int64_t* tok_pos, const float* ln_w, const float* mean,
                               const float* rstd, float eps, int64_t T, int64_t L, int64_t D, float p_drop,
                               uint64_t seed, const float* dout, float* dbase, float* const* dtables, float* dgate,
@@ -924,7 +938,7 @@
   RSX_ARG(L > 0 && L <= 64, "need 0 < L <= 64");
   if (T == 0) return 0;
   BwdArgs a;
-  fill_fwd(a.f, base, ids, tables, ntab, gate, pos, tok_pos, ln_w, nullptr, eps, T, L, nullptr,
+  fill_fwd(a.f, base, base_idx, ids, tables, ntab, gate, pos, tok_pos, ln_w, nullptr, eps, T, L, nullptr,
            const_cast<float*>(mean), const_cast<float*>(rstd), p_drop, seed);
   a.dout = dout;
   a.dbase = dbase;
diff --git a/llm-driven_content-based-feature_recommendation_system_amd/csrc/step_index.hip b/llm-driven_content-based-feature_recommendation_system_amd/csrc/step_index.hip
--- a/llm-driven_content-based-feature_recommendation_system_amd/csrc/step_index.hip
+++ b/llm-driven_content-based-feature_recommendation_system_amd/csrc/step_index.hip
@@ -228,13 +228,15 @@
   int64_t* tok_ids;
   int *row_col, *row_beg, *row_end, *exc_cols;
   int* last_t;
+  int64_t* tok_uidx;
 };
 
 __global__ __launch_bounds__(256) void si_tokens_k(const uint8_t* pm, const int64_t* tgt, const int64_t* ids0,
                                                    const int64_t* ids1, const int64_t* ids2, const int64_t* ids3,
                                                    const int64_t* ids4, const int64_t* ids5, int64_t B, int L,
                                                    int64_t T, const int* offT, const int* offN, const int* offE,
-                                                   const int* srt, const int* colidx, FillOut f, unsigned* ikeys,
+                                                   const int* srt, const int* colidx, const int* itemidx, FillOut f,
+                                                   unsigned* ikeys,
                                                    int* ivals, unsigned* pkeys, int* pvals, int* pair_b, int* pair_n) {
   const int lane = threadIdx.x & 63;
   const int64_t b = (int64_t)blockIdx.x * 4 + (threadIdx.x >> 6);
@@ -265,6 +267,11 @@
       f.tok_ids[(2 * k + 1) * T + tok] = v;
     }
     ikeys[tok] = (unsigned)ids0[o];
+    if (f.tok_uidx) {
+      const int64_t ui = itemidx[ids0[o]];
+      f.tok_uidx[tok] = ui;
+      f.tok_uidx[T + tok] = ui;
+    }
     ivals[tok] = (int)tok;
     if (u.valid) {
       const int64_t r = offN[b] + below(u.vm, lane);
@@ -367,14 +374,11 @@
   }
 }
 
-__global__ __launch_bounds__(256) void si_pv_k(const float* lookup, int64_t ld, const int64_t* ids_tok, int64_t T,
+__global__ __launch_bounds__(256) void si_pv_k(const float* lookup, int64_t ld, const int64_t* uniq_items, int64_t U,
                                                float* pv) {
   const int lane = threadIdx.x & 31;
-  for (int64_t t = ((int64_t)blockIdx.x * 256 + threadIdx.x) >> 5; t < T; t += ((int64_t)gridDim.x * 256) >> 5) {
-    const float4 v = reinterpret_cast<const float4*>(lookup + ids_tok[t] * ld)[lane];
-    reinterpret_cast<float4*>(pv + t * 128)[lane] = v;
-    reinterpret_cast<float4*>(pv + (T + t) * 128)[lane] = v;
-  }
+  for (int64_t u = ((int64_t)blockIdx.x * 256 + threadIdx.x) >> 5; u < U; u += ((int64_t)gridDim.x * 256) >> 5)
+    reinterpret_cast<float4*>(pv + u * 128)[lane] = reinterpret_cast<const float4*>(lookup + uniq_items[u] * ld)[lane];
 }
 
 int64_t a256(int64_t x) { return (x + 255) / 256 * 256; }
@@ -538,10 +542,12 @@
   f.seg2 = (int*)out[12]; f.seg2_64 = (int64_t*)out[13]; f.tok_ids = (int64_t*)out[14];
   f.row_col = (int*)out[23]; f.row_beg = (int*)out[24]; f.row_end = (int*)out[25]; f.exc_cols = (int*)out[26];
   f.last_t = (int*)out[32];
+  f.tok_uidx = (int64_t*)out[33];
   const unsigned gu = (unsigned)((B + 3) / 4);
   hipLaunchKernelGGL(si_tokens_k, dim3(gu), dim3(256), 0, st, pm, tgt, seq_ids[0], seq_ids[1], seq_ids[2],
                      seq_ids[3], seq_ids[4], seq_ids[5], B, (int)L, T, at<int>(ws, l.offT), at<int>(ws, l.offN),
-                     at<int>(ws, l.offE), at<int>(ws, l.srt), at<int>(ws, l.colidx), f, at<unsigned>(ws, l.ikeys),
+                     at<int>(ws, l.offE), at<int>(ws, l.srt), at<int>(ws, l.colidx), at<int>(ws, l.itemidx), f,
+                     at<unsigned>(ws, l.ikeys),
                      at<int>(ws, l.ivals), at<unsigned>(ws, l.pkeys), at<int>(ws, l.pvals), at<int>(ws, l.pair_b),
                      at<int>(ws, l.pair_n));
   RSX_LAUNCHED();
@@ -574,8 +580,8 @@
   }
   if (lookup && out[15]) {
     RSX_ARG(ld_lookup >= 128 && ld_lookup % 4 == 0, "pretrained lookup rows must be 128 floats (stride % 4 == 0)");
-    hipLaunchKernelGGL(si_pv_k, dim3(grid_for(T * 32)), dim3(256), 0, st, lookup, ld_lookup, f.tok_ids, T,
-                       (float*)out[15]);
+    hipLaunchKernelGGL(si_pv_k, dim3(grid_for(U * 32)), dim3(256), 0, st, lookup, ld_lookup,
+                       (const int64_t*)out[20], U, (float*)out[15]);
     RSX_LAUNCHED();
   }
   return 0;
diff --git a/llm-driven_content-based-feature_recommendation_system_amd/csrc/tower.hip b/llm-driven_content-based-feature_recommendation_system_amd/csrc/tower.hip
--- a/llm-driven_content-based-feature_recommendation_system_amd/csrc/tower.hip
+++ b/llm-driven_content-based-feature_recommendation_system_amd/csrc/tower.hip
@@ -19,11 +19,11 @@
   int64_t prof, hp, g, mo, ro, o, nrm, aR, xR, tidx, tinv, tuser, tseg, lseq, total;
 };
 
-Layout layout(int64_t T, int64_t U, int nl) {
+Layout layout(int64_t T, int64_t U, int nl, int64_t pv_rows) {
   Layout s{};
   int64_t o = 0;
   auto take = [&](int64_t n) { const int64_t r = o; o += al(n); return r; };
-  s.base = take(T * kD); s.x0 = take(T * kD); s.m0 = take(T); s.r0 = take(T);
+  s.base = take(pv_rows * kD); s.x0 = take(T * kD); s.m0 = take(T); s.r0 = take(T);
   s.h0 = take(T * kD); s.mh0 = take(T); s.rh0 = take(T);
   for (int i = 0; i < nl; ++i) {
     LayerAct& a = s.l[i];
@@ -41,7 +41,8 @@
 }
 
 struct BwdLayout {
-  int64_t dO, dG, dHp, dX, dXs, dH, dHs, dF, dPre, dRes, dA, dQKV, dProf, dBase, part, dAR, dXR, wsw, wsl, wse, total;
+  int64_t dO, dG, dHp, dX, dXs, dH, dHs, dF, dPre, dRes, dA, dQKV, dProf, dBase, part, dBaseU, dAR, dXR, wsw, wsl, wse,
+      total;
   int64_t n_wsw, n_wsl, n_wse;
 };
 
@@ -53,6 +54,7 @@
   s.dH = take(T * kD); s.dHs = take(T * kD); s.dF = take(T * kD); s.dPre = take(T * kF); s.dRes = take(T * kD);
   s.dA = take(T * kD); s.dQKV = take(T * kQKV); s.dProf = take(U * kD); s.dBase = take(T * kD);
   s.part = take((C > 0 ? C : 1) * kD);
+  s.dBaseU = take((C > 0 ? C : 1) * kD);
   s.dAR = take((T + 1) * kD); s.dXR = take((T + 1) * kD);
   int64_t w = 0;
   const int64_t nk[5][3] = {{T, kD, kD}, {T, kQKV, kD}, {T, kD, kF}, {T, kF, kD}, {U, kD, kD}};
@@ -241,9 +243,13 @@
 
 RSX_API int64_t rsx_tower_n_ptrs(int layers) { return n_ptrs(layers); }
 
-RSX_API int64_t rsx_tower_arena_bytes(int64_t T, int64_t U, int layers) {
-  if (layers < 1 || layers > kMaxLayers || T < 0 || U < 0) return -1;
-  return layout(T, U, layers).total * 4;
+RSX_API int64_t rsx_tower_arena_bytes(int64_t T, int64_t U, int layers, int64_t pv_rows) {
+  if (layers < 1 || layers > kMaxLayers || T < 0 || U < 0 || pv_rows < 0) return -1;
+  return layout(T, U, layers, pv_rows).total * 4;
+}
+
+namespace {
+bool per_item(const void* const* p, const int64_t* dims) { return p[RSX_TW_UIDX] != nullptr && dims[4] > 0; }
 }
 
 RSX_API int64_t rsx_tower_bwd_workspace_bytes(int64_t T, int64_t U, int64_t L, int layers, int64_t C) {
@@ -258,7 +264,10 @@
   const int nl = (int)dims[3];
   RSX_ARG(nl >= 1 && nl <= kMaxLayers, "1 <= layers <= 8");
   RSX_ARG(T > 0 && U > 0 && L > 0 && L <= 64, "need T, U > 0 and 0 < L <= 64");
-  const Layout s = layout(T, U, nl);
+  const bool uq = per_item(p, dims);
+  const int64_t Uq = dims[5];
+  RSX_ARG(!uq || Uq > 0, "per-item pretrained rows need Uq > 0");
+  const Layout s = layout(T, U, nl, uq ? Uq : T);
   RSX_ARG(arena_bytes >= s.total * 4, "arena too small (rsx_tower_arena_bytes)");
   for (int64_t i = 0; i < n_ptrs(nl) - 1; ++i)
     if (i < RSX_TW_ITEMSEG || i >= RSX_TW_ITEM_PROJ) RSX_ARG(p[i] != nullptr, "null input / parameter pointer");
@@ -270,17 +279,17 @@
   float* A = static_cast<float*>(arena);
   const float pd = fargs[0];
   const int pl = RSX_TW_LAYER0 + 12 * nl;
-  TW_CALL(rsx_gemm_x3(v.f(RSX_TW_PV), kD, v.f(RSX_TW_ITEM_PROJ), kD, v.f(RSX_TW_ITEM_PROJ + 1), T, kD, kD, kEpiBias,
-                      nullptr, 0, 0.0f, 0, A + s.base, kD, stream));
+  TW_CALL(rsx_gemm_x3(v.f(RSX_TW_PV), kD, v.f(RSX_TW_ITEM_PROJ), kD, v.f(RSX_TW_ITEM_PROJ + 1), uq ? Uq : T, kD, kD,
+                      kEpiBias, nullptr, 0, 0.0f, 0, A + s.base, kD, stream));
   const int64_t* ids[6];
   const float* tabs[6];
   for (int j = 0; j < 6; ++j) {
     ids[j] = v.i64(RSX_TW_IDS + j);
     tabs[j] = v.f(RSX_TW_TABLES + j);
   }
-  TW_CALL(rsx_seq_embed_fwd(A + s.base, ids, tabs, 6, v.f(RSX_TW_GATE), v.f(RSX_TW_POS), v.i64(RSX_TW_TOK_POS),
-                            v.f(RSX_TW_EMB_LN), v.f(RSX_TW_EMB_LN + 1), fargs[1], T, L, kD, pd, seeds[0], A + s.x0,
-                            A + s.m0, A + s.r0, stream));
+  TW_CALL(rsx_seq_embed_fwd(A + s.base, uq ? v.i64(RSX_TW_UIDX) : nullptr, ids, tabs, 6, v.f(RSX_TW_GATE),
+                            v.f(RSX_TW_POS), v.i64(RSX_TW_TOK_POS), v.f(RSX_TW_EMB_LN), v.f(RSX_TW_EMB_LN + 1), fargs[1],
+                            T, L, kD, pd, seeds[0], A + s.x0, A + s.m0, A + s.r0, stream));
   TW_CALL(rsx_ln_fwd(A + s.x0, nullptr, 0.0f, 0, v.f(RSX_TW_LAYER0), v.f(RSX_TW_LAYER0 + 1), fargs[2], 0, T, kD,
                      nullptr, A + s.h0, A + s.mh0, A + s.rh0, stream));
   const float* x = A + s.x0;
@@ -359,7 +368,10 @@
   const int nl = (int)dims[3];
   RSX_ARG(nl >= 1 && nl <= kMaxLayers, "1 <= layers <= 8");
   RSX_ARG(T > 0 && U > 0 && L > 0 && L <= 64 && C >= 0 && Uq >= 0, "bad sizes");
-  const Layout s = layout(T, U, nl);
+  const bool uq = per_item(p, dims);
+  RSX_ARG(!uq || (Uq > 0 && Uq <= C && !grads[RSX_TW_PV]),
+          "per-item pretrained rows: need 0 < Uq <= C and no pretrained-row gradient");
+  const Layout s = layout(T, U, nl, uq ? Uq : T);
   const BwdLayout b = bwd_layout(T, U, L, C);
   RSX_ARG(ws_bytes >= b.total * 4, "workspace too small (rsx_tower_bwd_workspace_bytes)");
   const int pl = RSX_TW_LAYER0 + 12 * nl;
@@ -473,17 +485,27 @@
   const int64_t rows[6] = {dims[6], dims[7], dims[8], dims[9], dims[10], dims[11]};
   const int64_t pad[6] = {0, 0, 0, 0, 0, 0};
   float* dBase = W + b.dBase;
-  TW_CALL(rsx_seq_embed_bwd(A + s.base, ids, tabs, rows, pad, 6, v.f(RSX_TW_GATE), v.f(RSX_TW_POS),
-                            v.i64(RSX_TW_TOK_POS), v.f(RSX_TW_EMB_LN), A + s.m0, A + s.r0, fargs[1], T, L, kD, pd,
+  TW_CALL(rsx_seq_embed_bwd(A + s.base, uq ? v.i64(RSX_TW_UIDX) : nullptr, ids, tabs, rows, pad, 6, v.f(RSX_TW_GATE),
+                            v.f(RSX_TW_POS), v.i64(RSX_TW_TOK_POS), v.f(RSX_TW_EMB_LN), A + s.m0, A + s.r0, fargs[1], T, L, kD, pd,
                             seeds[0], dX0, dBase, dtabs, G(RSX_TW_GATE), G(RSX_TW_POS), G(RSX_TW_EMB_LN),
                             G(RSX_TW_EMB_LN + 1), W + b.wse, b.n_wse, stream));
   if (C > 0) {
     const int64_t* plan = v.i64(RSX_TW_ITEMSEG);
     TW_CALL(rsx_segment_sum_rows(dBase, kD, plan, v.i64(RSX_TW_ITEMSEG + 1), v.i64(RSX_TW_ITEMSEG + 2), C, kD, nullptr,
                                  -1, W + b.part, kD, 0, stream));
-    TW_CALL(rsx_segment_sum_rows(W + b.part, kD, v.i64(RSX_TW_ITEMSEG + 2), v.i64(RSX_TW_ITEMSEG + 3),
-                                 v.i64(RSX_TW_ITEMSEG + 4), Uq, kD, v.f(RSX_TW_GATE), 0, G(RSX_TW_TABLES), kD, 1,
-                                 stream));
+    if (uq) {
+      TW_CALL(rsx_segment_sum_rows2(W + b.part, kD, v.i64(RSX_TW_ITEMSEG + 2), v.i64(RSX_TW_ITEMSEG + 3),
+                                    v.i64(RSX_TW_ITEMSEG + 4), Uq, kD, v.f(RSX_TW_GATE), 0, G(RSX_TW_TABLES), kD, 1,
+                                    W + b.dBaseU, kD, stream));
+    } else {
+      TW_CALL(rsx_segment_sum_rows(W + b.part, kD, v.i64(RSX_TW_ITEMSEG + 2), v.i64(RSX_TW_ITEMSEG + 3),
+                                   v.i64(RSX_TW_ITEMSEG + 4), Uq, kD, v.f(RSX_TW_GATE), 0, G(RSX_TW_TABLES), kD, 1,
+                                   stream));
+    }
+  }
+  if (uq) {
+    TW_CALL(wgrad(W + b.dBaseU, kD, v.f(RSX_TW_PV), kD, Uq, kD, kD, G(RSX_TW_ITEM_PROJ), kD, G(RSX_TW_ITEM_PROJ + 1)));
+    return 0;
   }
   if (grads[RSX_TW_PV]) TW_CALL(tn(dBase, kD, v.f(RSX_TW_ITEM_PROJ), kD, T, kD, kD, G(RSX_TW_PV), kD));
   TW_CALL(wgrad(dBase, kD, v.f(RSX_TW_PV), kD, T, kD, kD, G(RSX_TW_ITEM_PROJ), kD, G(RSX_TW_ITEM_PROJ + 1)));
diff --git a/llm-driven_content-based-feature_recommendation_system_amd/dist.py b/llm-driven_content-based-feature_recommendation_system_amd/dist.py
--- a/llm-driven_content-based-feature_recommendation_system_amd/dist.py
+++ b/llm-driven_content-based-feature_recommendation_system_amd/dist.py
@@ -312,10 +312,10 @@
     i64, i32, u8, f32 = torch.int64, torch.int32, torch.uint8, torch.float32
     specs = [((T,), i64), ((T,), i64), ((T,), i64), ((T,), u8), ((B + 1,), i32), ((B + 1,), i64), ((Nr,), i64),
              ((B,), i64), ((2 * T,), i64), ((2 * T,), i64), ((2 * T,), i64), ((2 * T,), u8), ((2 * B + 1,), i32),
-             ((2 * B + 1,), i64), ((6, 2 * T), i64), (((2 * T, 128), f32) if pretrained_vecs is None else None),
+             ((2 * B + 1,), i64), ((6, 2 * T), i64), (((U, 128), f32) if pretrained_vecs is None else None),
              ((2 * T,), i64), ((C + 1,), i64), ((C,), i64), ((U + 1,), i64), ((U,), i64), ((D,), i64), ((D,), f32),
              ((Nr,), i32), ((Nr,), i32), ((Nr,), i32), ((Nr,), i32), ((E,), i32), ((E,), i32), ((E,), i32),
-             ((D,), i32), ((D,), i32), ((B,), i32)]
+             ((D,), i32), ((D,), i32), ((B,), i32), ((2 * T,), i64)]
     out = _carve(specs, dev)
     lk = ops._c(pretrained_lookup) if pretrained_vecs is None else None
     N.check(lib.rsx_step_index_fill(N.ptr(pm8), N.ptr(tgt), N.ptr_array(seq), N.ptr(lk),
@@ -330,7 +330,7 @@
     pk2.item_seg = tuple(out[16:21])
     tok_ids = list(out[14].unbind(0))
     if pretrained_vecs is None:
-        pv_tok = out[15]
+        pv_tok = ops.ItemRows(out[15], out[33])
     else:
         pv_tok = pk.take(pretrained_vecs)
         pv_tok = torch.cat([pv_tok, pv_tok])
diff --git a/llm-driven_content-based-feature_recommendation_system_amd/ops.py b/llm-driven_content-based-feature_recommendation_system_amd/ops.py
--- a/llm-driven_content-based-feature_recommendation_system_amd/ops.py
+++ b/llm-driven_content-based-feature_recommendation_system_amd/ops.py
@@ -127,29 +127,69 @@
     return out
 
 
+class ItemRows:
+
+    requires_grad = False
+    materialized = 0
+
+    def __init__(self, rows, idx):
+        self.rows, self.idx = rows, idx
+
+    shape = property(lambda self: torch.Size((self.idx.numel(), self.rows.shape[1])))
+    dtype = property(lambda self: self.rows.dtype)
+    device = property(lambda self: self.rows.device)
+    is_cuda = property(lambda self: self.rows.is_cuda)
+
+    def materialize(self):
+        ItemRows.materialized += 1
+        return gather_rows(self.rows, self.idx)
+
+    def __len__(self):
+        return self.idx.numel()
+
+    def __getitem__(self, key):
+        return self.materialize()[key]
+
+    def __getattr__(self, name):
+        if name.startswith("__"):
+            raise AttributeError(name)
+        return getattr(self.materialize(), name)
+
+    @classmethod
+    def __torch_function__(cls, func, types, args=(), kwargs=None):
+        def tok(a):
+            return a.materialize() if isinstance(a, ItemRows) else a
+        return func(*[tok(a) for a in args], **{k: tok(v) for k, v in (kwargs or {}).items()})
+
+
 class _SeqEmbed(torch.autograd.Function):
     @staticmethod
     def forward(ctx, base, gate, pos, ln_w, ln_b, ids, cfg, tok_pos, *tables):
-        eps, p_drop, seed, padding_idx, L, tab0_seg = cfg
+        eps, p_drop, seed, padding_idx, L, tab0_seg, base_idx = cfg
         N.ensure_device(base)
         D = base.shape[-1]
-        T = base.numel() // D
         base = _c(base)
         ids = [_c(t) for t in ids]
         tables = [_c(t) for t in tables]
-        out = torch.empty_like(base)
+        if base_idx is None:
+            T = base.numel() // D
+            out = torch.empty_like(base)
+        else:
+            T = base_idx.numel()
+            out = torch.empty(T, D, device=base.device, dtype=torch.float32)
         mean = torch.empty(T, device=base.device, dtype=torch.float32)
         rstd = torch.empty_like(mean)
         gate = _c(gate)
         with timed("seq_embed_fwd"):
             rc = N.lib().rsx_seq_embed_fwd(
-                N.ptr(base), N.ptr_array(ids), N.ptr_array(tables), len(tables), N.ptr(gate), N.ptr(pos),
-                N.ptr(tok_pos), N.ptr(ln_w), N.ptr(ln_b), eps, T, L, D, p_drop, seed, N.ptr(out), N.ptr(mean),
-                N.ptr(rstd), N.stream())
+                N.ptr(base), N.ptr(base_idx), N.ptr_array(ids), N.ptr_array(tables), len(tables), N.ptr(gate),
+                N.ptr(pos), N.ptr(tok_pos), N.ptr(ln_w), N.ptr(ln_b), eps, T, L, D, p_drop, seed, N.ptr(out),
+                N.ptr(mean), N.ptr(rstd), N.stream())
         N.check(rc, "seq_embed_fwd")
         ctx.save_for_backward(base, gate, pos, ln_w, mean, rstd, tok_pos, *ids, *tables)
         ctx.cfg = (eps, p_drop, seed, padding_idx, len(tables), T, L, D)
         ctx.tab0_seg = tab0_seg
+        ctx.base_idx = base_idx
         return out
 
     @staticmethod
@@ -161,34 +201,48 @@
         tables = list(saved[7 + nt:7 + 2 * nt])
         dout = _c(dout)
         need = ctx.needs_input_grad
-        dbase = torch.empty_like(base) if need[0] else None
+        base_idx = ctx.base_idx
+        dbase = torch.empty_like(dout) if need[0] else None
         dgate, dpos, dlnw, dlnb, *dtabs = _zeros_group(
             [gate if need[1] else None, pos if need[2] else None, ln_w if need[3] else None,
              ln_w if need[4] else None] + [t if need[8 + j] else None for j, t in enumerate(tables)])
         rows = N.i64_array([t.shape[0] for t in tables])
         seg0 = ctx.tab0_seg if (nt > 0 and dtabs[0] is not None) else None
+        seg_b = ctx.tab0_seg if (base_idx is not None and need[0]) else None
         if seg0 is not None and dbase is None:
-            dbase = torch.empty_like(base)
+            dbase = torch.empty_like(dout)
         kern_tabs = ([None] + dtabs[1:]) if seg0 is not None else dtabs
         nws = N.lib().rsx_seq_embed_bwd_workspace_floats(T, L, D)
         ws = torch.empty(nws, device=base.device, dtype=torch.float32)
         with timed("seq_embed_bwd"):
             rc = N.lib().rsx_seq_embed_bwd(
-                N.ptr(base), N.ptr_array(ids), N.ptr_array(tables), rows,
+                N.ptr(base), N.ptr(base_idx), N.ptr_array(ids), N.ptr_array(tables), rows,
                 N.i64_array(padding_idx), nt, N.ptr(gate), N.ptr(pos), N.ptr(tok_pos), N.ptr(ln_w), N.ptr(mean),
                 N.ptr(rstd), eps, T, L, D, p_drop, seed, N.ptr(dout), N.ptr(dbase), N.ptr_array(kern_tabs),
                 N.ptr(dgate), N.ptr(dpos), N.ptr(dlnw), N.ptr(dlnb), N.ptr(ws), nws, N.stream())
         N.check(rc, "seq_embed_bwd")
-        if seg0 is not None:
-            perm, cb, chunk_ids, ch_off, uniq = seg0
+        if seg0 is not None or seg_b is not None:
+            perm, cb, chunk_ids, ch_off, uniq = ctx.tab0_seg
             part = torch.empty(chunk_ids.numel(), D, device=base.device, dtype=torch.float32)
             rc = N.lib().rsx_segment_sum_rows(N.ptr(dbase), D, N.ptr(perm), N.ptr(cb), N.ptr(chunk_ids),
                                               chunk_ids.numel(), D, None, -1, N.ptr(part), D, 0, N.stream())
             N.check(rc, "segment_sum_rows(chunks)")
-            rc = N.lib().rsx_segment_sum_rows(N.ptr(part), D, N.ptr(chunk_ids), N.ptr(ch_off), N.ptr(uniq),
-                                              uniq.numel(), D, N.ptr(gate), padding_idx[0], N.ptr(dtabs[0]),
-                                              dtabs[0].stride(0), 1, N.stream())
-            N.check(rc, "segment_sum_rows(ids)")
+            if seg_b is not None:
+                dbase = torch.empty_like(base)
+            if seg0 is not None and seg_b is not None:
+                rc = N.lib().rsx_segment_sum_rows2(N.ptr(part), D, N.ptr(chunk_ids), N.ptr(ch_off), N.ptr(uniq),
+                                                   uniq.numel(), D, N.ptr(gate), padding_idx[0], N.ptr(dtabs[0]),
+                                                   dtabs[0].stride(0), 1, N.ptr(dbase), D, N.stream())
+                N.check(rc, "segment_sum_rows2(ids)")
+            elif seg0 is not None:
+                rc = N.lib().rsx_segment_sum_rows(N.ptr(part), D, N.ptr(chunk_ids), N.ptr(ch_off), N.ptr(uniq),
+                                                  uniq.numel(), D, N.ptr(gate), padding_idx[0], N.ptr(dtabs[0]),
+                                                  dtabs[0].stride(0), 1, N.stream())
+                N.check(rc, "segment_sum_rows(ids)")
+            else:
+                rc = N.lib().rsx_segment_sum_rows(N.ptr(part), D, N.ptr(chunk_ids), N.ptr(ch_off), None,
+                                                  uniq.numel(), D, None, -1, N.ptr(dbase), D, 0, N.stream())
+                N.check(rc, "segment_sum_rows(base)")
         if not need[0]:
             dbase = None
         return (dbase, dgate, dpos, dlnw, dlnb, None, None, None, *dtabs)
@@ -217,7 +271,7 @@
 
 
 def seq_embed(base, ids, tables, gate, pos, ln_w, ln_b, eps=1e-5, p_drop=0.0, padding_idx=None, tok_pos=None,
-              tab0_seg=None):
+              tab0_seg=None, base_idx=None):
     if padding_idx is None:
         padding_idx = [-1] * len(tables)
     padding_idx = [(-1 if p is None else int(p)) for p in padding_idx]
@@ -228,7 +282,12 @@
     else:
         L = pos.shape[0]
         tok_pos = _c(tok_pos)
-    cfg = (float(eps), float(p_drop), seed, padding_idx, int(L), tab0_seg)
+    if base_idx is not None:
+        if tok_pos is None or tab0_seg is None or base.dim() != 2 or base.shape[0] != tab0_seg[4].numel():
+            raise RuntimeError("seq_embed: base_idx needs the packed form, tab0_seg and one base row per "
+                               "distinct ids[0] value")
+        base_idx = _c(_index("seq_embed", "base_idx", base_idx, base, ids[0].numel()))
+    cfg = (float(eps), float(p_drop), seed, padding_idx, int(L), tab0_seg, base_idx)
     return _SeqEmbed.apply(base, gate, pos, ln_w, ln_b, list(ids), cfg, tok_pos, *tables)
 
 
@@ -1555,16 +1614,18 @@
 
     @staticmethod
     def forward(ctx, pv, gate, profile, cfg, *params):
-        packed, tok_ids, p_drop, eps, nl, tail_last = cfg
-        T, D = pv.shape
+        packed, tok_ids, p_drop, eps, nl, tail_last, tok_uidx = cfg
+        T, D = tok_ids[0].numel(), pv.shape[1]
         U = packed.seg_off.numel() - 1
         dev = pv.device
         pv = _c(pv)
         gate = _c(gate)
         profile = _c(profile)
         perm, cb, chunk_ids, ch_off, uniq = packed.item_seg
+        assert pv.shape[0] == (T if tok_uidx is None else uniq.numel())
         inputs = ([pv] + list(tok_ids) + [packed.tok_pos, packed.tok_pad, packed.seg_off, packed.seg_off64,
-                                            packed.tok_user, gate, profile, perm, cb, chunk_ids, ch_off, uniq])
+                                            packed.tok_user, gate, profile, perm, cb, chunk_ids, ch_off, uniq,
+                                            tok_uidx])
         tail_last = None if tail_last is None else _c(tail_last)
         ptrs = N.ptr_array(inputs + list(params) + [tail_last])
         tabs = params[2:8]
@@ -1575,7 +1636,7 @@
         fargs = (ctypes.c_float * (len(eps) + 1))(p_drop, *eps)
         seeds = [next_seed() if p_drop > 0 else 0 for _ in range(1 + 4 * nl)]
         seeds_arr = (ctypes.c_uint64 * len(seeds))(*seeds)
-        nbytes = N.lib().rsx_tower_arena_bytes(T, U, nl)
+        nbytes = N.lib().rsx_tower_arena_bytes(T, U, nl, pv.shape[0])
         arena = torch.empty(nbytes, device=dev, dtype=torch.uint8)
         out = torch.empty(R, D, device=dev, dtype=torch.float32)
         with timed("tower_fwd"):
@@ -1602,7 +1663,7 @@
         dprofile = written[-1]
         dparams = [written[0], written[1]] + acc + written[2:-1]
         dpv = torch.empty_like(pv) if ctx.needs_input_grad[0] else None
-        grads = [dpv] + [None] * 11 + [dgate, dprofile] + [None] * 5 + dparams + [None]
+        grads = [dpv] + [None] * 11 + [dgate, dprofile] + [None] * 6 + dparams + [None]
         nws = N.lib().rsx_tower_bwd_workspace_bytes(T, U, L, nl, C)
         ws = torch.empty(nws, device=dev, dtype=torch.uint8)
         with timed("tower_bwd"):
@@ -1632,7 +1693,10 @@
     for layer in layers:
         eps += [layer.norm1.eps, layer.norm2.eps]
     eps.append(model.output_proj[1].eps)
-    cfg = (packed, [_c(t) for t in tok_ids], float(p_drop), [float(e) for e in eps], len(layers), tail_last)
+    tok_uidx = None
+    if isinstance(pv_tok, ItemRows):
+        pv_tok, tok_uidx = pv_tok.rows, _c(pv_tok.idx)
+    cfg = (packed, [_c(t) for t in tok_ids], float(p_drop), [float(e) for e in eps], len(layers), tail_last, tok_uidx)
     return _TowerPacked.apply(pv_tok, s_g, profile, cfg, *(params if params is not None else tower_params(model)))
 
 
diff --git a/llm-driven_content-based-feature_recommendation_system_amd/tower_code/v1_refine_usertower.py b/llm-driven_content-based-feature_recommendation_system_amd/tower_code/v1_refine_usertower.py
--- a/llm-driven_content-based-feature_recommendation_system_amd/tower_code/v1_refine_usertower.py
+++ b/llm-driven_content-based-feature_recommendation_system_amd/tower_code/v1_refine_usertower.py
@@ -280,16 +280,22 @@
         s_g = torch.sigmoid(self.seq_gate) * self._seq_gate_mask
         profile = self._static_profile(age_bucket, price_bucket, cnt_bucket, recency_bucket, channel_ids,
                                        club_status_ids, news_freq_ids, fn_ids, active_ids, cont_feats, p, packed.B)
+        item_seg = getattr(packed, "item_seg", None)
+        tok_uidx = None
+        if isinstance(pretrained_tok, ops.ItemRows) and item_seg is None:
+            pretrained_tok = pretrained_tok.materialize()
         params = ops.tower_native_ok(self, packed, pretrained_tok) if torch.is_grad_enabled() else None
         if params is not None:
             return ops.tower_packed(self, packed, pretrained_tok, tok_ids, s_g, profile, p, params, tail_last)
+        if isinstance(pretrained_tok, ops.ItemRows):
+            pretrained_tok, tok_uidx = pretrained_tok.rows, pretrained_tok.idx
         base = ops.linear_tok(pretrained_tok, self.item_proj.weight, self.item_proj.bias)
         x = ops.seq_embed(
             base, tok_ids,
             [self.item_id_emb.weight, self.time_emb.weight, self.type_emb.weight, self.color_emb.weight,
              self.graphic_emb.weight, self.section_emb.weight],
             s_g, self.pos_emb.weight, self.emb_ln.weight, self.emb_ln.bias, eps=self.emb_ln.eps, p_drop=p,
-            padding_idx=[0, 0, 0, 0, 0, 0], tok_pos=packed.tok_pos, tab0_seg=getattr(packed, "item_seg", None))
+            padding_idx=[0, 0, 0, 0, 0, 0], tok_pos=packed.tok_pos, tab0_seg=item_seg, base_idx=tok_uidx)
         x = self._encoder_stack(x, packed.tok_pad, p, seg_off=packed.seg_off)
         lin0, ln, lin3 = self.output_proj[0], self.output_proj[1], self.output_proj[3]
         D = self.d_model
```

After: 562,000, median of 6. 1.2% higher.
